# 30stomercury/whisper-char-alignment

Hardware: AMD Instinct MI355X
Metric: utterances/sec (whisper-medium, 10s audio, char align) at 1/2/4/8 MI355X (higher is better)
Workload: dtype f16x2 (hi + lo operand pairs on the f16 MFMA pipe: fp32-equivalent operands, fp32 accumulate)

## Files before the change

### include/wca.h

```cpp
#ifndef WCA_H_
#define WCA_H_

#include <stdint.h>

#ifdef __cplusplus
extern "C" {
#endif

typedef struct wca_engine wca_engine;

typedef enum {
  WCA_STATUS_PARTITIONED = 1,
  WCA_OK = 0,
  WCA_ERR_INVALID = -1,
  WCA_ERR_TOO_LONG = -2,
  WCA_ERR_HIP = -3,
  WCA_ERR_STATE = -4,
  WCA_ERR_NOMEM = -5
} wca_status;

typedef struct {
  int32_t n_mels;
  int32_t n_audio_ctx;
  int32_t n_audio_state;
// ... 28 lines not shown
void wca_engine_destroy(wca_engine* e);
int wca_engine_set_stream(wca_engine* e, void* hip_stream);
int wca_engine_synchronize(wca_engine* e);

int wca_load_weight(wca_engine* e, const char* name, const void* host_ptr, int dtype, const int64_t* shape, int ndim);
int wca_finalize_weights(wca_engine* e);
int wca_weights_inexact(wca_engine* e, long long* n_tensors_out, long long* n_values_out, char* first_name_out, int first_name_cap);
int wca_set_allow_rounded_weights(wca_engine* e, int on);


int wca_log_mel(wca_engine* e, const float* pcm_dev, int64_t pcm_stride, const int32_t* n_samples_host, int batch,
                float* mel_out_dev);

int wca_log_mel_long(wca_engine* e, const float* pcm_dev, int64_t n_samples, float* mel_out_dev, int64_t ld, int64_t* n_frames_out);

int wca_resample_plan(int sr_in, int32_t* L, int32_t* M, int32_t* W, int32_t* n_taps);
int wca_resample_table(int sr_in, double* table_out);
int wca_resample_16k(wca_engine* e, const float* in_dev, int channels, int64_t ld, int64_t n_in, int sr_in, float* out_dev, int64_t out_cap,
                     int64_t* n_out);

int wca_mel_window(wca_engine* e, const float* mel_long_dev, int64_t ld, int64_t n_frames, const int32_t* seek_host,
                   const int32_t* size_host, int batch, float* mel_out_dev);

int wca_quiet_cuts(wca_engine* e, const float* mel_long_dev, int64_t ld, int64_t content_frames, int n_pieces, int radius, int half_width,
                   int32_t* cuts_host, int32_t* level_host );

int wca_get_attentions(wca_engine* e, const float* mel_dev, const int64_t* tokens_dev, int batch, int n_tok,
                       const int32_t* n_tok_host, const int32_t* max_frames_host, int medfilt_width, float qk_scale,
                       float* weights_out_dev, float* logits_out_dev);

int wca_attention_weights(wca_engine* e, const float* qk_dev, int L, int H, int n, int ld, int max_frames,
                          int medfilt_width, float qk_scale, float* weights_out_dev);

int wca_median_filter(wca_engine* e, const float* in_dev, float* out_dev, int64_t rows, int F, int width);

int wca_filter_attention(wca_engine* e, const float* attns_dev, int L, int H, int n, int F, int topk, float w_colnorm,
                         float w_rownorm, float w_coverage, float* scores_host, int32_t* sel_idx_host,
                         float* sel_score_host);

int wca_force_align(wca_engine* e, const float* ws_dev, int L, int H, int n, int F, const wca_align_opts* opts,
                    float* matrix_host, int32_t* text_idx_host, int32_t* time_idx_host, int32_t* path_len_host,
                    int32_t* sel_idx_host, float* sel_score_host);

int wca_default_find_alignment(wca_engine* e, const float* ws_dev, int L, int H, int n, int F, const int32_t* heads_host,
                                int n_heads, int sot_len, float* weights_norm_out_dev, float* matrix_host,
                                int32_t* text_idx_host, int32_t* time_idx_host, int32_t* path_len_host);

int wca_dtw(wca_engine* e, const float* matrix_host, int N, int M, int32_t* text_idx_host, int32_t* time_idx_host,
            int32_t* path_len_host);

int wca_dtw_batch_dev(wca_engine* e, const float* matrix_dev, int P, int N, int M, int32_t* jump_frame_host);

int wca_dtw_open(wca_engine* e, const float* matrix_host, int N, int M, int32_t* text_idx_host, int32_t* time_idx_host,
                 int32_t* path_len_host, int32_t* end_row_host, float* score_host);

int wca_dtw_batch_dev_open(wca_engine* e, const float* matrix_dev, int P, int N, int M, const int32_t* n_rows_host,
                           const int32_t* n_cols_host, const int32_t* open_end_host, int32_t* jump_frame_host, int32_t* end_row_host,
                           float* score_host);

int wca_probe_heads(wca_engine* e, const float* ws_dev, int L, int H, int n, int F, int sot_len, float* scores_host,
                    int32_t* jump_frame_host);
int wca_probe_strict_tp(wca_engine* e, int n_heads, const int32_t* word_end_row_host, int n_hyp, const double* ref_times_host, int n_ref,
                        const uint8_t* same_word_host, double tolerance, int32_t* tp_host);

int wca_align_batch(wca_engine* e, const float* pcm_dev, int64_t pcm_stride, const int32_t* n_samples_host,
                    const int64_t* tokens_dev, int n_tok_max, const int32_t* n_tok_host,
                    const int32_t* max_frames_host, int batch, const wca_align_opts* opts, int32_t* jump_frame_host,
                    int32_t* sel_idx_host);

typedef struct {
  int32_t sample_len;
  int32_t eot;
  int32_t timestamp_begin;
  int32_t apply_timestamp_rules;
  int32_t max_initial_timestamp_index;
  int32_t no_speech;
} wca_decode_opts;

typedef struct {
  int32_t sample_len;
  int32_t eot;
  int32_t timestamp_begin;
  int32_t apply_timestamp_rules;
  int32_t max_initial_timestamp_index;
  int32_t no_speech;
  int32_t sot_index;
  int32_t prefill;
} wca_decode_opts_ex;

int wca_encode_batch(wca_engine* e, const float* mel_dev, const float* pcm_dev, int64_t pcm_stride,
                     const int32_t* n_samples_host, int batch);

int wca_greedy_decode(wca_engine* e, const float* mel_dev, const float* pcm_dev, int64_t pcm_stride,
                      const int32_t* n_samples_host, int batch, const int32_t* initial_tokens_host, int n_initial,
                      const uint8_t* suppress_mask_host, const uint8_t* blank_mask_host, const wca_decode_opts* opts,
                      int32_t* tokens_out_host, int32_t* n_tokens_host, float* sum_logprob_host,
                      float* no_speech_prob_host);
int wca_greedy_decode_ex(wca_engine* e, const float* mel_dev, const float* pcm_dev, int64_t pcm_stride,
                         const int32_t* n_samples_host, int batch, const int32_t* initial_tokens_host, int n_initial,
                         const uint8_t* suppress_mask_host, const uint8_t* blank_mask_host, const wca_decode_opts_ex* opts,
                         int32_t* tokens_out_host, int32_t* n_tokens_host, float* sum_logprob_host,
                         float* no_speech_prob_host);
int wca_greedy_decode_rows(wca_engine* e, const float* mel_dev, const float* pcm_dev, int64_t pcm_stride,
                           const int32_t* n_samples_host, int batch, const int32_t* initial_tokens_host,
                           const int32_t* n_initial_host, const int32_t* sot_index_host, const int32_t* sample_len_host,
                           const uint8_t* suppress_mask_host, const uint8_t* blank_mask_host, const wca_decode_opts* opts,
                           int32_t* tokens_out_host, int32_t* n_tokens_host, float* sum_logprob_host,
                           float* no_speech_prob_host);
int wca_detect_language(wca_engine* e, const float* mel_dev, const float* pcm_dev, int64_t pcm_stride, const int32_t* n_samples_host,
                        int batch, int sot, int lang_begin, int n_lang, int32_t* lang_token_host, float* probs_host);
int wca_last_decode_positions(wca_engine* e, int32_t* prefill_positions, int32_t* step_positions);

int wca_align_batch_enqueue(wca_engine* e, const float* pcm_dev, int64_t pcm_stride, const int32_t* n_samples_host,
                            const int64_t* tokens_dev, int n_tok_max, const int32_t* n_tok_host,
                            const int32_t* max_frames_host, int batch, const wca_align_opts* opts);
int wca_align_batch_fetch(wca_engine* e, int batch, int n_tok_max, int topk, int32_t* jump_frame_host,
                          int32_t* sel_idx_host);

int wca_align_batch_enqueue_ex(wca_engine* e, const float* pcm_dev, int64_t pcm_stride, const int32_t* n_samples_host,
                               const int64_t* tokens_dev, int n_tok_max, const int32_t* n_tok_host,
                               const int32_t* max_frames_host, int batch, const wca_align_opts* opts, int32_t vocab_end);
int wca_align_batch_fetch_ex(wca_engine* e, int batch, int n_tok_max, int topk, int32_t* jump_frame_host,
                             int32_t* sel_idx_host, float* token_logprob_host);
int wca_align_batch_enqueue_open(wca_engine* e, const float* pcm_dev, int64_t pcm_stride, const int32_t* n_samples_host,
                                 const int64_t* tokens_dev, int n_tok_max, const int32_t* n_tok_host,
                                 const int32_t* max_frames_host, int batch, const wca_align_opts* opts, int32_t vocab_end,
                                 const int32_t* open_end_host);
int wca_align_batch_fetch_open(wca_engine* e, int batch, int n_tok_max, int topk, int32_t* jump_frame_host,
                               int32_t* sel_idx_host, float* token_logprob_host, int32_t* end_row_host, float* score_host);
int wca_token_logprobs(wca_engine* e, const float* logits_dev, int rows, int ld, int vocab_end, const int64_t* targets_dev,
                       float* out_dev);

int wca_flac_info(const uint8_t* buf, int64_t nbytes, int32_t* sample_rate, int32_t* channels, int32_t* bits_per_sample,
                  int64_t* total_samples);
int wca_flac_decode(const uint8_t* buf, int64_t nbytes, float* out, int64_t capacity_per_channel, int64_t* n_decoded);

#define WCA_COMM_ID_BYTES 128
int wca_comm_unique_id(uint8_t* id_out );
int wca_comm_init(wca_engine* e, const uint8_t* id , int rank, int world);
int wca_comm_destroy(wca_engine* e);
int wca_allgather_results(wca_engine* e, const uint8_t* packed_host, int64_t n_bytes, uint8_t* gathered_host,
                          int64_t capacity_per_rank, int64_t* sizes_host );
int wca_allreduce_counters(wca_engine* e, int64_t* counters_host , int n);
int wca_collate_plan(const int64_t* sizes , const int64_t* capacities , int world, int64_t* pad_out);

int wca_test_gemm(wca_engine* e, const void* a_f16_dev, const void* w_f16_dev, const float* bias_dev, void* c_dev, int M,
                  int N, int K, int gelu, int out_mode);
int wca_test_gemm_pairs(wca_engine* e, const void* a2_f16_dev, const void* w_f16_dev, const float* bias_dev, void* c_dev, int M,
                        int N, int K, int gelu, int out_mode);
int wca_test_gemm_ln(wca_engine* e, const void* a_f16_dev, const void* w_f16_dev, const float* bias_dev, float* x_dev,
                     const float* gamma_dev, const float* beta_dev, void* xn_f16_dev, int M, int N, int K, int site);
int wca_test_gemm_plan(int M, int N, int K, int lda, int out_mode, int gelu, int a_lo, int force_tile, int site, int n_cu, int cu_limit, int flags,
                       int64_t sk_bytes, int32_t* out);
typedef struct wca_test_gemm_desc {
  const void* a;
  const void* w;
  const float* bias;
  void* c;
  const float* addend;
  const float* pos;
  int64_t a_batch_stride, c_batch_stride, a_lo, c_lo;
  int32_t M, N, K;
  int32_t lda, ldw, ldc;
  int32_t a_rows_per_batch, c_rows_per_batch;
  int32_t ld_addend, pos_period;
  int32_t gelu, out_mode, force_tile, site, cu_limit, supertile;
} wca_test_gemm_desc;
int wca_test_gemm_ex(wca_engine* e, const wca_test_gemm_desc* desc, int32_t* plan_out);
typedef struct wca_test_attn_desc {
  const void* q;
  const void* k;
  const void* v;
  void* o;
  float* cap;
  const int32_t* nk_rows;
  int64_t q_bs, k_bs, v_bs, o_bs;
  int64_t q_lo, k_lo, v_lo, o_lo;
  int64_t cap_bs, cap_hs;
  int32_t q_rs, k_rs, v_rs, o_rs;
  int32_t cap_ld, cap_cols;
  int32_t split, B, H, nq, nk, causal, variant;
} wca_test_attn_desc;
int wca_test_attention_ex(wca_engine* e, const wca_test_attn_desc* desc);
int wca_test_gemm_rows(wca_engine* e, const void* a_f16_dev, const float* x_f32_dev, const float* gamma_dev, const float* beta_dev,
                       const void* w_f16_dev, const float* bias_dev, void* c_dev, int M, int N, int K, int gelu, int out_mode, int splitk,
                       int groups, void* kv_k_f16_dev, void* kv_v_f16_dev, int T_max, int kv_t);
int wca_test_set_attn_split_drop(int mask);
int wca_test_set_switch(const char* name, int value);
int wca_test_last_scores(wca_engine* e, int batch, float* scores_host);
int wca_test_attention(wca_engine* e, const void* q_dev, const void* k_dev, const void* v_dev, void* o_dev,
                       float* cap_dev, int cap_ld, int cap_cols, int B, int H, int nq, int nk, int causal);
int wca_test_attention_split(wca_engine* e, const void* q2_dev, const void* k2_dev, const void* v2_dev, void* o2_dev,
                             float* cap_dev, int cap_ld, int cap_cols, int B, int H, int nq, int nk, int causal);
int wca_test_language_head(wca_engine* e, const float* x_dev, int B, int lang_begin, int n_lang, float* probs_dev, int32_t* lang_token_dev);
int wca_test_decode_select(wca_engine* e, const float* logits_dev, int batch, int n_vocab, int32_t* tokens_dev, int T_max,
                           int cur_len, int n_initial, const uint8_t* suppress_mask_dev, const uint8_t* blank_mask_dev,
                           const wca_decode_opts* opts, float* sum_logprob_dev, int32_t* n_done_dev);
int wca_test_decode_select_rows(wca_engine* e, const float* logits_dev, int batch, int n_vocab, int32_t* tokens_dev, int T_max,
                                const int32_t* cur_len_dev, const int32_t* n_initial_dev, const int32_t* cap_dev, int n_done_idx,
                                int n_done_len, const uint8_t* suppress_mask_dev, const uint8_t* blank_mask_dev,
                                const wca_decode_opts* opts, float* sum_logprob_dev, int32_t* n_done_dev);
int wca_test_attention_rows(wca_engine* e, const void* q_dev, const void* k_dev, const void* v_dev, void* o_dev, int B, int H, int nq,
                            int nk, const int32_t* nk_rows_dev, int causal);
int wca_test_layernorm(wca_engine* e, const float* x_dev, const float* g_dev, const float* b_dev, void* out_f16_dev,
                       int rows, int d);
int wca_test_layernorm_split(wca_engine* e, const float* x_dev, const float* g_dev, const float* b_dev, void* out2_f16_dev,
                             int rows, int d);
int wca_test_encoder(wca_engine* e, const float* mel_dev, int batch, float* xa_out_dev);

int wca_last_stage_ms(wca_engine* e, float* ms8);
enum {
  WCA_SITE_QKV = 0,
  WCA_SITE_ATTN = 1,
  WCA_SITE_OUT = 2,
  WCA_SITE_FC1 = 3,
  WCA_SITE_FC2 = 4,
  WCA_SITE_LN1 = 5,
  WCA_SITE_LN2 = 6,
  WCA_N_SITES = 7
};
int wca_last_kernel_ms(wca_engine* e, int site, int* n_launches, float* total_ms, double* flops_per_launch,
                       double* bytes_per_launch);
int wca_set_fuse_ln(wca_engine* e, int on);
enum { WCA_PRECISION_F16 = 0, WCA_PRECISION_SPLIT = 1, WCA_PRECISION_REFERENCE = 1 };
int wca_set_precision(wca_engine* e, int mode);
int wca_get_precision(wca_engine* e);
int wca_set_overlap(wca_engine* e, int on);
int wca_set_cu_partition(wca_engine* e, int phase2_cus);
int wca_set_decode_mode(wca_engine* e, int fused, int streams);
int wca_set_profiling(wca_engine* e, int on);

#ifdef __cplusplus
}
#endif
#endif
```

### whisper-char-alignment_amd/_lib.py

```python
import ctypes as C
import os

_HERE = os.path.dirname(os.path.abspath(__file__))
LIB_PATH = os.path.join(_HERE, "libwca.so")


class WcaError(RuntimeError):
    def __init__(self, code, msg):
        super().__init__("wca error %d: %s" % (code, msg))
        self.code = code


class TooLongError(WcaError):
    """n_tok > 448 or max_frames > 1500 (the skip condition of infer_ali.py:79)."""


class ModelDims(C.Structure):
    _fields_ = [(n, C.c_int32) for n in (
        "n_mels", "n_audio_ctx", "n_audio_state", "n_audio_head", "n_audio_layer",
        "n_vocab", "n_text_ctx", "n_text_state", "n_text_head", "n_text_layer")]


class AlignOpts(C.Structure):
    _fields_ = [("aggregation", C.c_int32), ("topk", C.c_int32), ("w_colnorm", C.c_float),
                ("w_rownorm", C.c_float), ("w_coverage", C.c_float), ("sot_len", C.c_int32),
                ("medfilt_width", C.c_int32), ("qk_scale", C.c_float)]


class DecodeOpts(C.Structure):
    _fields_ = [("sample_len", C.c_int32), ("eot", C.c_int32), ("timestamp_begin", C.c_int32),
                ("apply_timestamp_rules", C.c_int32), ("max_initial_timestamp_index", C.c_int32), ("no_speech", C.c_int32)]


class DecodeOptsEx(C.Structure):
    _fields_ = DecodeOpts._fields_ + [("sot_index", C.c_int32), ("prefill", C.c_int32)]


class GemmDesc(C.Structure):
    _fields_ = ([(n, C.c_void_p) for n in ("a", "w", "bias", "c", "addend", "pos")] +
                [(n, C.c_int64) for n in ("a_batch_stride", "c_batch_stride", "a_lo", "c_lo")] +
                [(n, C.c_int32) for n in ("M", "N", "K", "lda", "ldw", "ldc", "a_rows_per_batch", "c_rows_per_batch", "ld_addend", "pos_period",
                                          "gelu", "out_mode", "force_tile", "site", "cu_limit", "supertile")])


class AttnDesc(C.Structure):
    _fields_ = ([(n, C.c_void_p) for n in ("q", "k", "v", "o", "cap", "nk_rows")] +
                [(n, C.c_int64) for n in ("q_bs", "k_bs", "v_bs", "o_bs", "q_lo", "k_lo", "v_lo", "o_lo", "cap_bs", "cap_hs")] +
                [(n, C.c_int32) for n in ("q_rs", "k_rs", "v_rs", "o_rs", "cap_ld", "cap_cols", "split", "B", "H", "nq", "nk", "causal", "variant")])


ERR_TOO_LONG = -2
AGGR_MEAN, AGGR_TOPK = 0, 1
PRECISION_SITES = ("logmel", "conv", "enc_gemm", "enc_attn", "cross_kv", "dec", "capture")
SITES = {"qkv": 0, "attention": 1, "out_proj": 2, "fc1": 3, "fc2": 4, "ln1": 5, "ln2": 6}
DTYPE_F32, DTYPE_F16 = 0, 1

_vp, _i, _i64, _f = C.c_void_p, C.c_int, C.c_int64, C.c_float
_pi32 = C.POINTER(C.c_int32)
_pf = C.POINTER(C.c_float)

SIGNATURES = {
    "wca_last_error": (C.c_char_p, []),
    "wca_version": (_i, []),
    "wca_engine_create": (_i, [C.POINTER(ModelDims), _i, _i, C.POINTER(_vp)]),
    "wca_engine_create_ex": (_i, [C.POINTER(ModelDims), _i, _i, _i, C.POINTER(_vp)]),
    "wca_engine_destroy": (None, [_vp]),
    "wca_engine_set_stream": (_i, [_vp, _vp]),
    "wca_engine_synchronize": (_i, [_vp]),
    "wca_load_weight": (_i, [_vp, C.c_char_p, _vp, _i, C.POINTER(_i64), _i]),
    "wca_finalize_weights": (_i, [_vp]),
    "wca_weights_inexact": (_i, [_vp, C.POINTER(C.c_longlong), C.POINTER(C.c_longlong), C.c_char_p, _i]),
    "wca_set_allow_rounded_weights": (_i, [_vp, _i]),
    "wca_log_mel": (_i, [_vp, _vp, _i64, _pi32, _i, _vp]),
    "wca_log_mel_long": (_i, [_vp, _vp, _i64, _vp, _i64, C.POINTER(_i64)]),
    "wca_resample_plan": (_i, [_i, _pi32, _pi32, _pi32, _pi32]),
    "wca_resample_table": (_i, [_i, C.POINTER(C.c_double)]),
    "wca_resample_16k": (_i, [_vp, _vp, _i, _i64, _i64, _i, _vp, _i64, C.POINTER(_i64)]),
    "wca_mel_window": (_i, [_vp, _vp, _i64, _i64, _pi32, _pi32, _i, _vp]),
    "wca_quiet_cuts": (_i, [_vp, _vp, _i64, _i64, _i, _i, _i, _pi32, _pi32]),
    "wca_get_attentions": (_i, [_vp, _vp, _vp, _i, _i, _pi32, _pi32, _i, _f, _vp, _vp]),
    "wca_median_filter": (_i, [_vp, _vp, _vp, _i64, _i, _i]),
    "wca_filter_attention": (_i, [_vp, _vp, _i, _i, _i, _i, _i, _f, _f, _f, _pf, _pi32, _pf]),
    "wca_force_align": (_i, [_vp, _vp, _i, _i, _i, _i, C.POINTER(AlignOpts), _pf, _pi32, _pi32, _pi32, _pi32, _pf]),
    "wca_default_find_alignment": (_i, [_vp, _vp, _i, _i, _i, _i, _pi32, _i, _i, _vp, _pf, _pi32, _pi32, _pi32]),
    "wca_attention_weights": (_i, [_vp, _vp, _i, _i, _i, _i, _i, _i, _f, _vp]),
    "wca_flac_info": (_i, [_vp, _i64, _pi32, _pi32, _pi32, C.POINTER(_i64)]),
    "wca_flac_decode": (_i, [_vp, _i64, _vp, _i64, C.POINTER(_i64)]),
    "wca_dtw": (_i, [_vp, _pf, _i, _i, _pi32, _pi32, _pi32]),
    "wca_dtw_batch_dev": (_i, [_vp, _vp, _i, _i, _i, _pi32]),
    "wca_dtw_open": (_i, [_vp, _pf, _i, _i, _pi32, _pi32, _pi32, _pi32, _pf]),
    "wca_dtw_batch_dev_open": (_i, [_vp, _vp, _i, _i, _i, _pi32, _pi32, _pi32, _pi32, _pi32, _pf]),
    "wca_probe_heads": (_i, [_vp, _vp, _i, _i, _i, _i, _i, _pf, _pi32]),
    "wca_align_batch": (_i, [_vp, _vp, _i64, _pi32, _vp, _i, _pi32, _pi32, _i, C.POINTER(AlignOpts), _pi32, _pi32]),
    "wca_align_batch_enqueue": (_i, [_vp, _vp, _i64, _pi32, _vp, _i, _pi32, _pi32, _i, C.POINTER(AlignOpts)]),
    "wca_align_batch_fetch": (_i, [_vp, _i, _i, _i, _pi32, _pi32]),
    "wca_align_batch_enqueue_ex": (_i, [_vp, _vp, _i64, _pi32, _vp, _i, _pi32, _pi32, _i, C.POINTER(AlignOpts), C.c_int32]),
    "wca_align_batch_fetch_ex": (_i, [_vp, _i, _i, _i, _pi32, _pi32, _pf]),
    "wca_align_batch_enqueue_open": (_i, [_vp, _vp, _i64, _pi32, _vp, _i, _pi32, _pi32, _i, C.POINTER(AlignOpts), C.c_int32, _pi32]),
    "wca_align_batch_fetch_open": (_i, [_vp, _i, _i, _i, _pi32, _pi32, _pf, _pi32, _pf]),
    "wca_token_logprobs": (_i, [_vp, _vp, _i, _i, _i, _vp, _vp]),
    "wca_encode_batch": (_i, [_vp, _vp, _vp, _i64, _pi32, _i]),
    "wca_greedy_decode": (_i, [_vp, _vp, _vp, _i64, _pi32, _i, _pi32, _i, _vp, _vp, C.POINTER(DecodeOpts), _pi32, _pi32, _pf, _pf]),
    "wca_greedy_decode_ex": (_i, [_vp, _vp, _vp, _i64, _pi32, _i, _pi32, _i, _vp, _vp, C.POINTER(DecodeOptsEx), _pi32, _pi32, _pf, _pf]),
    "wca_greedy_decode_rows": (_i, [_vp, _vp, _vp, _i64, _pi32, _i, _pi32, _pi32, _pi32, _pi32, _vp, _vp, C.POINTER(DecodeOpts), _pi32, _pi32, _pf,
                                    _pf]),
    "wca_detect_language": (_i, [_vp, _vp, _vp, _i64, _pi32, _i, _i, _i, _i, _pi32, _pf]),
    "wca_test_language_head": (_i, [_vp, _vp, _i, _i, _i, _vp, _vp]),
    "wca_last_decode_positions": (_i, [_vp, _pi32, _pi32]),
    "wca_test_decode_select_rows": (_i, [_vp, _vp, _i, _i, _vp, _i, _vp, _vp, _vp, _i, _i, _vp, _vp, C.POINTER(DecodeOpts), _vp, _vp]),
    "wca_test_attention_rows": (_i, [_vp, _vp, _vp, _vp, _vp, _i, _i, _i, _i, _vp, _i]),
    "wca_test_decode_select": (_i, [_vp, _vp, _i, _i, _vp, _i, _i, _i, _vp, _vp, C.POINTER(DecodeOpts), _vp, _vp]),
    "wca_test_gemm": (_i, [_vp, _vp, _vp, _vp, _vp, _i, _i, _i, _i, _i]),
    "wca_test_gemm_plan": (_i, [_i, _i, _i, _i, _i, _i, _i, _i, _i, _i, _i, _i, _i64, _pi32]),
    "wca_test_gemm_ex": (_i, [_vp, C.POINTER(GemmDesc), _pi32]),
    "wca_test_attention_ex": (_i, [_vp, C.POINTER(AttnDesc)]),
    "wca_test_gemm_ln": (_i, [_vp, _vp, _vp, _vp, _vp, _vp, _vp, _vp, _i, _i, _i, _i]),
    "wca_test_set_attn_split_drop": (_i, [_i]),
    "wca_test_set_switch": (_i, [C.c_char_p, _i]),
    "wca_test_last_scores": (_i, [_vp, _i, _pf]),
    "wca_test_gemm_pairs": (_i, [_vp, _vp, _vp, _vp, _vp, _i, _i, _i, _i, _i]),
    "wca_test_attention": (_i, [_vp, _vp, _vp, _vp, _vp, _vp, _i, _i, _i, _i, _i, _i, _i]),
    "wca_test_attention_split": (_i, [_vp, _vp, _vp, _vp, _vp, _vp, _i, _i, _i, _i, _i, _i, _i]),
    "wca_test_layernorm": (_i, [_vp, _vp, _vp, _vp, _vp, _i, _i]),
    "wca_test_layernorm_split": (_i, [_vp, _vp, _vp, _vp, _vp, _i, _i]),
    "wca_test_encoder": (_i, [_vp, _vp, _i, _vp]),
    "wca_last_stage_ms": (_i, [_vp, _pf]),
    "wca_set_profiling": (_i, [_vp, _i]),
    "wca_last_kernel_ms": (_i, [_vp, _i, C.POINTER(C.c_int), _pf, C.POINTER(C.c_double), C.POINTER(C.c_double)]),
    "wca_set_overlap": (_i, [_vp, _i]),
    "wca_set_cu_partition": (_i, [_vp, _i]),
    "wca_set_fuse_ln": (_i, [_vp, _i]),
    "wca_set_precision": (_i, [_vp, _i]),
    "wca_get_precision": (_i, [_vp]),
    "wca_set_decode_mode": (_i, [_vp, _i, _i]),
    "wca_comm_unique_id": (_i, [_vp]),
    "wca_comm_init": (_i, [_vp, _vp, _i, _i]),
    "wca_comm_destroy": (_i, [_vp]),
    "wca_allgather_results": (_i, [_vp, _vp, _i64, _vp, _i64, C.POINTER(_i64)]),
    "wca_allreduce_counters": (_i, [_vp, C.POINTER(_i64), _i]),
    "wca_collate_plan": (_i, [C.POINTER(_i64), C.POINTER(_i64), _i, C.POINTER(_i64)]),
    "wca_probe_strict_tp": (_i, [_vp, _i, _vp, _i, _vp, _i, _vp, C.c_double, _vp]),
    "wca_test_gemm_rows": (_i, [_vp, _vp, _vp, _vp, _vp, _vp, _vp, _vp, _i, _i, _i, _i, _i, _i, _i, _vp, _vp, _i, _i]),
}

_lib = None


def load():
    global _lib
    if _lib is not None:
        return _lib
    if not os.path.exists(LIB_PATH):
        raise ImportError(
            "libwca.so not found at %s: build it with `python whisper-char-alignment_amd/build.py` "
            "(or __graft_entry__.build()). The alignment engine has no CPU fallback." % LIB_PATH)
    lib = C.CDLL(LIB_PATH)
    for name, (res, args) in SIGNATURES.items():
        fn = getattr(lib, name)
        fn.restype = res
        fn.argtypes = args
    _lib = lib
    return lib


def check(code):
    if code == 0:
        return
    msg = load().wca_last_error()
    msg = msg.decode("utf-8", "replace") if msg else ""
    if code == -2:
        raise TooLongError(code, msg)
    raise WcaError(code, msg)


def i32_array(values):
    arr = (C.c_int32 * len(values))(*[int(v) for v in values])
    return arr
```

### whisper-char-alignment_amd/csrc/attention_split.hip

```cpp
#include <cstdlib>

#include "attn_common.h"
#include "launch.h"

namespace wca {

namespace {

template <bool CAUSAL, bool CAPTURE>
__global__ __launch_bounds__(256, 2) void attn_split_kernel(AttnArgs a) {
  constexpr int NW = 4;
  extern __shared__ __attribute__((aligned(16))) char smem[];
  half_t* lds = reinterpret_cast<half_t*>(smem);
  const int tid = threadIdx.x;
  const int lane = tid & 63;
  const int wave = __builtin_amdgcn_readfirstlane(tid >> 6);
  const int fr = lane & 15, fg = lane >> 4;
  constexpr int QB = NW * 32;
  const int n_qt = (a.nq + QB - 1) / QB;
  const int lid = xcd_remap(blockIdx.x, n_qt * a.H * a.B);
  const int bh = lid / n_qt;
  const int b = bh / a.H, h = bh - b * a.H;
  const int q_blk = (lid - bh * n_qt) * QB;
  const int q_wave = q_blk + wave * 32;
// ... 237 lines not shown
  do {                                                                                       \
    R[0] = lds_read_tr_asm<VH>(A);                                                               \
    R[1] = lds_read_tr_asm<VH + B16>(A);                                                         \
    R[2] = lds_read_tr_asm<VL>(A);                                                               \
    R[3] = lds_read_tr_asm<VL + B16>(A);                                                         \
    R[4] = lds_read_tr_asm<VH + K2>(A);                                                          \
    R[5] = lds_read_tr_asm<VH + K2 + B16>(A);                                                    \
    R[6] = lds_read_tr_asm<VL + K2>(A);                                                          \
    R[7] = lds_read_tr_asm<VL + K2 + B16>(A);                                                    \
  } while (0)
      WCA_ISSUE_V(c_, vaddr[0] + sb);
#pragma unroll
      for (int dt = 0; dt < 4; ++dt) {
        if (dt < 3) {
          WCA_ISSUE_V(n_, vaddr[dt + 1] + sb);
          WCA_LGKM_WAIT8(8, c_[0], c_[1], c_[2], c_[3], c_[4], c_[5], c_[6], c_[7]);
        } else {
          WCA_LGKM_WAIT8(0, c_[0], c_[1], c_[2], c_[3], c_[4], c_[5], c_[6], c_[7]);
        }
#pragma unroll
        for (int k2 = 0; k2 < 2; ++k2) {
          const half8 vh = __builtin_shufflevector(c_[4 * k2], c_[4 * k2 + 1], 0, 1, 2, 3, 4, 5, 6, 7);
          const half8 vl = __builtin_shufflevector(c_[4 * k2 + 2], c_[4 * k2 + 3], 0, 1, 2, 3, 4, 5, 6, 7);
#pragma unroll
          for (int s = 0; s < 2; ++s) {
            ot[s][dt] = __builtin_amdgcn_mfma_f32_16x16x32_f16(vl, ph[s][k2], ot[s][dt], 0, 0, 0);
            ot[s][dt] = __builtin_amdgcn_mfma_f32_16x16x32_f16(vh, pl[s][k2], ot[s][dt], 0, 0, 0);
            ot[s][dt] = __builtin_amdgcn_mfma_f32_16x16x32_f16(vh, ph[s][k2], ot[s][dt], 0, 0, 0);
          }
        }
        if (dt < 3) {
#pragma unroll
          for (int i = 0; i < 8; ++i) c_[i] = n_[i];
        }
      }
#undef WCA_ISSUE_V
    }
  }

#pragma unroll
  for (int s = 0; s < 2; ++s) {
    const float l = xor32_sum(xor16_sum(l_part[s]));
    if (qrow[s] >= a.nq) continue;
    const float inv = 1.0f / l;
    half_t* op = a.O + (long)b * a.o_bs + (long)qrow[s] * a.o_rs + h * 64 + 4 * fg;
#pragma unroll
    for (int dt = 0; dt < 4; ++dt) {
      half4 oh, ol;
#pragma unroll
      for (int r = 0; r < 4; ++r) {
        const HalfPair pr = split_pair(ot[s][dt][r] * inv);
        oh[r] = pr.hi;
        ol[r] = pr.lo;
      }
      *reinterpret_cast<half4*>(op + dt * 16) = oh;
      *reinterpret_cast<half4*>(op + a.o_lo + dt * 16) = ol;
    }
  }
}



#define WCA_S_PIN8(A, B, C, D, E, F, G, H) asm volatile("" : "+v"(A), "+v"(B), "+v"(C), "+v"(D), "+v"(E), "+v"(F), "+v"(G), "+v"(H)::"memory")

template <int DROP>
__global__ __launch_bounds__(256, 2) void attn_split32_kernel(AttnArgs a) {
  constexpr int NW = 4;
  extern __shared__ __attribute__((aligned(16))) char smem[];
  half_t* lds = reinterpret_cast<half_t*>(smem);
  const int tid = threadIdx.x;
  const int lane = tid & 63;
  const int wave = __builtin_amdgcn_readfirstlane(tid >> 6);
  const int l31 = lane & 31, hh = lane >> 5;
  constexpr int QB = NW * 32;
  constexpr int TB = TILE * (int)sizeof(half_t);
  constexpr int SLOT_BYTES = 4 * TB;
  const int n_qt = (a.nq + QB - 1) / QB;
  const int lid = xcd_remap(blockIdx.x, n_qt * a.H * a.B);
  const int bh = lid / n_qt;
  const int b = bh / a.H, h = bh - b * a.H;
  const int q_wave = (lid - bh * n_qt) * QB + wave * 32;
  const int qrow = q_wave + l31;
  const float c_log2 = a.scale * LOG2E;
  half8 qh[4], ql[4];
  {
    const int qc = qrow < a.nq ? qrow : a.nq - 1;
    const half_t* qp = a.Q + (long)b * a.q_bs + (long)qc * a.q_rs + h * 64 + hh * 8;
#pragma unroll
    for (int ks = 0; ks < 4; ++ks) {
      const half8 rh = *reinterpret_cast<const half8*>(qp + ks * 16);
      const half8 rl = *reinterpret_cast<const half8*>(qp + a.q_lo + ks * 16);
#pragma unroll
      for (int j = 0; j < 8; ++j) {
        const HalfPair pr = split_pair(((float)rh[j] + (float)rl[j]) * c_log2);
        qh[ks][j] = pr.hi;
        ql[ks][j] = pr.lo;
      }
    }
  }
  const int nkt = (a.nk + KT - 1) / KT;
  const int kbytes = (int)(((long)(a.nk - 1) * a.k_rs + 64) * 2), vbytes = (int)(((long)(a.nk - 1) * a.v_rs + 64) * 2);
  const half_t* Kb = a.K + (long)b * a.k_bs + h * 64;
  const half_t* Vb = a.V + (long)b * a.v_bs + h * 64;
  const __amdgpu_buffer_rsrc_t rkh = __builtin_amdgcn_make_buffer_rsrc(const_cast<half_t*>(Kb), 0, kbytes, 0x00020000);
  const __amdgpu_buffer_rsrc_t rkl = __builtin_amdgcn_make_buffer_rsrc(const_cast<half_t*>(Kb + a.k_lo), 0, kbytes, 0x00020000);
  const __amdgpu_buffer_rsrc_t rvh = __builtin_amdgcn_make_buffer_rsrc(const_cast<half_t*>(Vb), 0, vbytes, 0x00020000);
  const __amdgpu_buffer_rsrc_t rvl = __builtin_amdgcn_make_buffer_rsrc(const_cast<half_t*>(Vb + a.v_lo), 0, vbytes, 0x00020000);
  unsigned dk[2], dv[2];
#pragma unroll
  for (int i = 0; i < 2; ++i) {
    const int r = (wave * 2 + i) * 8 + (lane >> 3);
    dk[i] = (unsigned)(r * a.k_rs * 2 + (((lane & 7) ^ ((r >> 1) & 7)) << 4));
    dv[i] = (unsigned)(r * a.v_rs * 2 + (((lane & 7) ^ ((r & 2) << 1)) << 4));
  }
  const unsigned k_tile_bytes = (unsigned)(KT * a.k_rs * 2), v_tile_bytes = (unsigned)(KT * a.v_rs * 2);
  auto stage = [&](int buf, int kt) {
    half_t* Kh = lds + buf * (4 * TILE);
#pragma unroll
    for (int i = 0; i < 2; ++i) {
      const int rbase = (wave * 2 + i) * 8;
      __builtin_amdgcn_raw_ptr_buffer_load_lds(rkh, (WCA_LDS void*)(Kh + rbase * 64), 16, (int)dk[i], (int)(kt * k_tile_bytes), 0, 0);
      __builtin_amdgcn_raw_ptr_buffer_load_lds(rkl, (WCA_LDS void*)(Kh + TILE + rbase * 64), 16, (int)dk[i], (int)(kt * k_tile_bytes), 0, 0);
      __builtin_amdgcn_raw_ptr_buffer_load_lds(rvh, (WCA_LDS void*)(Kh + 2 * TILE + rbase * 64), 16, (int)dv[i], (int)(kt * v_tile_bytes), 0, 0);
      __builtin_amdgcn_raw_ptr_buffer_load_lds(rvl, (WCA_LDS void*)(Kh + 3 * TILE + rbase * 64), 16, (int)dv[i], (int)(kt * v_tile_bytes), 0, 0);
    }
  };

  const int kswz = (l31 >> 1) & 7;
  const unsigned lds_base = lds_off(lds);
  unsigned ka[4];
#pragma unroll
  for (int ks = 0; ks < 4; ++ks) ka[ks] = lds_base + (unsigned)(l31 * 128 + 16 * ((hh ^ kswz) & 1) + 32 * (ks ^ (kswz >> 1)));
  const int vq = (lane & 15) >> 2, vp = lane & 3, vg1 = (lane >> 4) & 1;
  const int vkey0 = 4 * hh + vq;
  const int vdim0 = 16 * vg1 + 4 * vp;
  const int vsw = (vkey0 & 2) << 1;
  unsigned va[2];
#pragma unroll
  for (int db = 0; db < 2; ++db)
    va[db] = lds_base + (unsigned)(2 * TB + vkey0 * 128 + (((4 * db + (vdim0 >> 3)) ^ vsw) << 4) + 2 * (vdim0 & 7));

  f32x16 ot[2];
#pragma unroll
  for (int d = 0; d < 2; ++d)
#pragma unroll
    for (int r = 0; r < 16; ++r) ot[d][r] = 0.f;
  float m_run = -INFINITY;
  float l_run = 0.f;
  f32x16 cinit;
#pragma unroll
  for (int r = 0; r < 16; ++r) cinit[r] = 0.f;

  stage(0, 0);
  auto tile = [&](auto slot_c, int kt) {
    constexpr int SLOT = decltype(slot_c)::value;
    constexpr int SB = SLOT * SLOT_BYTES;
    asm volatile("s_waitcnt vmcnt(0)" ::: "memory");
    __builtin_amdgcn_s_barrier();
    asm volatile("" ::: "memory");
    if (kt + 1 < nkt) stage(SLOT ^ 1, kt + 1);

    f32x16 st[2];
    {
      half8 kl0[4], kh0[4], kl1[4], kh1[4];
      kl0[0] = lds_read_b128_asm<SB + TB>(ka[0]);
      kl0[1] = lds_read_b128_asm<SB + TB>(ka[1]);
      kl0[2] = lds_read_b128_asm<SB + TB>(ka[2]);
      kl0[3] = lds_read_b128_asm<SB + TB>(ka[3]);
      kh0[0] = lds_read_b128_asm<SB>(ka[0]);
      kh0[1] = lds_read_b128_asm<SB>(ka[1]);
      kh0[2] = lds_read_b128_asm<SB>(ka[2]);
      kh0[3] = lds_read_b128_asm<SB>(ka[3]);
      kl1[0] = lds_read_b128_asm<SB + TB + 32 * 128>(ka[0]);
      kl1[1] = lds_read_b128_asm<SB + TB + 32 * 128>(ka[1]);
      kl1[2] = lds_read_b128_asm<SB + TB + 32 * 128>(ka[2]);
      kl1[3] = lds_read_b128_asm<SB + TB + 32 * 128>(ka[3]);
      kh1[0] = lds_read_b128_asm<SB + 32 * 128>(ka[0]);
      kh1[1] = lds_read_b128_asm<SB + 32 * 128>(ka[1]);
      kh1[2] = lds_read_b128_asm<SB + 32 * 128>(ka[2]);
      kh1[3] = lds_read_b128_asm<SB + 32 * 128>(ka[3]);
      if constexpr (DROP == 0) {
      WCA_LGKM_WAIT4(12, kl0[0], kl0[1], kl0[2], kl0[3]);
      st[0] = __builtin_amdgcn_mfma_f32_32x32x16_f16(kl0[0], qh[0], cinit, 0, 0, 0);
#pragma unroll
      for (int ks = 1; ks < 4; ++ks) st[0] = __builtin_amdgcn_mfma_f32_32x32x16_f16(kl0[ks], qh[ks], st[0], 0, 0, 0);
      WCA_LGKM_WAIT4(8, kh0[0], kh0[1], kh0[2], kh0[3]);
#pragma unroll
      for (int ks = 0; ks < 4; ++ks) st[0] = __builtin_amdgcn_mfma_f32_32x32x16_f16(kh0[ks], ql[ks], st[0], 0, 0, 0);
#pragma unroll
      for (int ks = 0; ks < 4; ++ks) st[0] = __builtin_amdgcn_mfma_f32_32x32x16_f16(kh0[ks], qh[ks], st[0], 0, 0, 0);
      WCA_LGKM_WAIT4(4, kl1[0], kl1[1], kl1[2], kl1[3]);
      st[1] = __builtin_amdgcn_mfma_f32_32x32x16_f16(kl1[0], qh[0], cinit, 0, 0, 0);
#pragma unroll
      for (int ks = 1; ks < 4; ++ks) st[1] = __builtin_amdgcn_mfma_f32_32x32x16_f16(kl1[ks], qh[ks], st[1], 0, 0, 0);
      WCA_LGKM_WAIT4(0, kh1[0], kh1[1], kh1[2], kh1[3]);
#pragma unroll
      for (int ks = 0; ks < 4; ++ks) st[1] = __builtin_amdgcn_mfma_f32_32x32x16_f16(kh1[ks], ql[ks], st[1], 0, 0, 0);
#pragma unroll
      for (int ks = 0; ks < 4; ++ks) st[1] = __builtin_amdgcn_mfma_f32_32x32x16_f16(kh1[ks], qh[ks], st[1], 0, 0, 0);
      } else {
        WCA_LGKM_WAIT4(0, kh1[0], kh1[1], kh1[2], kh1[3]);
        WCA_S_PIN8(kl0[0], kl0[1], kl0[2], kl0[3], kh0[0], kh0[1], kh0[2], kh0[3]);
        WCA_S_PIN8(kl1[0], kl1[1], kl1[2], kl1[3], kh1[0], kh1[1], kh1[2], kh1[3]);
        st[0] = cinit;
        st[1] = cinit;
#pragma unroll
        for (int ks = 0; ks < 4; ++ks) {
          if (!(DROP & 1)) st[0] = __builtin_amdgcn_mfma_f32_32x32x16_f16(kl0[ks], qh[ks], st[0], 0, 0, 0);
          if (!(DROP & 1)) st[1] = __builtin_amdgcn_mfma_f32_32x32x16_f16(kl1[ks], qh[ks], st[1], 0, 0, 0);
        }
#pragma unroll
        for (int ks = 0; ks < 4; ++ks) {
          if (!(DROP & 2)) st[0] = __builtin_amdgcn_mfma_f32_32x32x16_f16(kh0[ks], ql[ks], st[0], 0, 0, 0);
          if (!(DROP & 2)) st[1] = __builtin_amdgcn_mfma_f32_32x32x16_f16(kh1[ks], ql[ks], st[1], 0, 0, 0);
        }
#pragma unroll
        for (int ks = 0; ks < 4; ++ks) {
          st[0] = __builtin_amdgcn_mfma_f32_32x32x16_f16(kh0[ks], qh[ks], st[0], 0, 0, 0);
          st[1] = __builtin_amdgcn_mfma_f32_32x32x16_f16(kh1[ks], qh[ks], st[1], 0, 0, 0);
        }
      }
    }
    half4 v0ha[4], v0hb[4], v0la[4], v0lb[4], v1ha[4], v1hb[4], v1la[4], v1lb[4];
#define WCA_ISSUE_V32(P, DB)                                           \
  do {                                                                 \
    P##ha[0] = lds_read_tr_asm<SB + 0 * 2048>(va[DB]);                     \
    P##hb[0] = lds_read_tr_asm<SB + 0 * 2048 + 1024>(va[DB]);              \
    P##ha[1] = lds_read_tr_asm<SB + 1 * 2048>(va[DB]);                     \
    P##hb[1] = lds_read_tr_asm<SB + 1 * 2048 + 1024>(va[DB]);              \
    P##ha[2] = lds_read_tr_asm<SB + 2 * 2048>(va[DB]);                     \
    P##hb[2] = lds_read_tr_asm<SB + 2 * 2048 + 1024>(va[DB]);              \
    P##ha[3] = lds_read_tr_asm<SB + 3 * 2048>(va[DB]);                     \
    P##hb[3] = lds_read_tr_asm<SB + 3 * 2048 + 1024>(va[DB]);              \
    P##la[0] = lds_read_tr_asm<SB + TB + 0 * 2048>(va[DB]);                \
    P##lb[0] = lds_read_tr_asm<SB + TB + 0 * 2048 + 1024>(va[DB]);         \
    P##la[1] = lds_read_tr_asm<SB + TB + 1 * 2048>(va[DB]);                \
    P##lb[1] = lds_read_tr_asm<SB + TB + 1 * 2048 + 1024>(va[DB]);         \
    P##la[2] = lds_read_tr_asm<SB + TB + 2 * 2048>(va[DB]);                \
    P##lb[2] = lds_read_tr_asm<SB + TB + 2 * 2048 + 1024>(va[DB]);         \
    P##la[3] = lds_read_tr_asm<SB + TB + 3 * 2048>(va[DB]);                \
    P##lb[3] = lds_read_tr_asm<SB + TB + 3 * 2048 + 1024>(va[DB]);         \
  } while (0)
    WCA_ISSUE_V32(v0, 0);
    if (kt * KT + KT > a.nk) {
#pragma unroll
      for (int kb = 0; kb < 2; ++kb)
#pragma unroll
        for (int r = 0; r < 16; ++r) {
          const int key = kt * KT + kb * 32 + (r & 3) + 8 * (r >> 2) + 4 * hh;
          st[kb][r] = key >= a.nk ? -INFINITY : st[kb][r];
        }
    }
    float mx;
    {
      float m0 = max3f(st[0][0], st[0][1], st[0][2]), m1 = max3f(st[0][3], st[0][4], st[0][5]);
      float m2 = max3f(st[0][6], st[0][7], st[0][8]), m3 = max3f(st[0][9], st[0][10], st[0][11]);
      m0 = max3f(m0, st[0][12], st[0][13]);
      m1 = max3f(m1, st[0][14], st[0][15]);
      m2 = max3f(m2, st[1][0], st[1][1]);
      m3 = max3f(m3, st[1][2], st[1][3]);
      m0 = max3f(m0, st[1][4], st[1][5]);
      m1 = max3f(m1, st[1][6], st[1][7]);
      m2 = max3f(m2, st[1][8], st[1][9]);
      m3 = max3f(m3, st[1][10], st[1][11]);
      m0 = max3f(m0, st[1][12], st[1][13]);
      m1 = max3f(m1, st[1][14], st[1][15]);
      mx = fmaxf(max3f(m0, m1, m2), m3);
      mx = xor32_max(mx);
    }
    if (__any((mx > RESCALE_THR) || (m_run == -INFINITY && mx != -INFINITY))) {
      const float m_eff = (m_run == -INFINITY) ? 0.f : m_run;
      const float m_new = fmaxf(m_run, mx + m_eff);
      const float delta = (m_new == -INFINITY) ? 0.f : m_new - m_eff;
      const float alpha = (m_run == -INFINITY) ? 1.0f : __builtin_amdgcn_exp2f(m_run - m_new);
      l_run *= alpha;
#pragma unroll
      for (int d = 0; d < 2; ++d)
#pragma unroll
        for (int r = 0; r < 16; ++r) ot[d][r] *= alpha;
#pragma unroll
      for (int kb = 0; kb < 2; ++kb)
#pragma unroll
        for (int r = 0; r < 16; ++r) st[kb][r] -= delta;
      m_run = m_new;
      const float c0 = (m_new != -INFINITY) ? -m_new : 0.f;
#pragma unroll
      for (int r = 0; r < 16; ++r) cinit[r] = c0;
    }
    half8 ph[4], pl[4];
    {
      f32x2 psum = f32x2{0.f, 0.f};
#pragma unroll
      for (int s4 = 0; s4 < 4; ++s4) {
        half2_ hq[4], lq[4];
#pragma unroll
        for (int u = 0; u < 4; ++u) {
          const int r0 = 8 * (s4 & 1) + 2 * u;
          const f32x2 p = f32x2{__builtin_amdgcn_exp2f(st[s4 >> 1][r0]), __builtin_amdgcn_exp2f(st[s4 >> 1][r0 + 1])};
          psum += p;
          hq[u] = __builtin_convertvector(p, half2_);
          const unsigned hu = __builtin_bit_cast(unsigned, hq[u]);
          unsigned lu;
          asm("v_fma_mixlo_f16 %0, %1, 1.0, -%2 op_sel:[0,0,0] op_sel_hi:[0,0,1]" : "=v"(lu) : "v"(p[0]), "v"(hu));
          asm("v_fma_mixhi_f16 %0, %1, 1.0, -%2 op_sel:[0,0,1] op_sel_hi:[0,0,1]" : "+v"(lu) : "v"(p[1]), "v"(hu));
          lq[u] = __builtin_bit_cast(half2_, lu);
        }
        ph[s4] = half8{hq[0][0], hq[0][1], hq[1][0], hq[1][1], hq[2][0], hq[2][1], hq[3][0], hq[3][1]};
        pl[s4] = half8{lq[0][0], lq[0][1], lq[1][0], lq[1][1], lq[2][0], lq[2][1], lq[3][0], lq[3][1]};
      }
      l_run += psum[0] + psum[1];
    }
    WCA_LGKM_WAIT8(0, v0ha[0], v0hb[0], v0ha[1], v0hb[1], v0ha[2], v0hb[2], v0ha[3], v0hb[3]);
    WCA_S_PIN8(v0la[0], v0lb[0], v0la[1], v0lb[1], v0la[2], v0lb[2], v0la[3], v0lb[3]);
    WCA_ISSUE_V32(v1, 1);
#pragma unroll
    for (int s4 = 0; s4 < 4; ++s4) {
      const half8 wh = __builtin_shufflevector(v0ha[s4], v0hb[s4], 0, 1, 2, 3, 4, 5, 6, 7);
      const half8 wl = __builtin_shufflevector(v0la[s4], v0lb[s4], 0, 1, 2, 3, 4, 5, 6, 7);
      if (!(DROP & 4)) ot[0] = __builtin_amdgcn_mfma_f32_32x32x16_f16(wl, ph[s4], ot[0], 0, 0, 0);
      if (!(DROP & 8)) ot[0] = __builtin_amdgcn_mfma_f32_32x32x16_f16(wh, pl[s4], ot[0], 0, 0, 0);
      ot[0] = __builtin_amdgcn_mfma_f32_32x32x16_f16(wh, ph[s4], ot[0], 0, 0, 0);
    }
    WCA_LGKM_WAIT8(0, v1ha[0], v1hb[0], v1ha[1], v1hb[1], v1ha[2], v1hb[2], v1ha[3], v1hb[3]);
    WCA_S_PIN8(v1la[0], v1lb[0], v1la[1], v1lb[1], v1la[2], v1lb[2], v1la[3], v1lb[3]);
#pragma unroll
    for (int s4 = 0; s4 < 4; ++s4) {
      const half8 wh = __builtin_shufflevector(v1ha[s4], v1hb[s4], 0, 1, 2, 3, 4, 5, 6, 7);
      const half8 wl = __builtin_shufflevector(v1la[s4], v1lb[s4], 0, 1, 2, 3, 4, 5, 6, 7);
      if (!(DROP & 4)) ot[1] = __builtin_amdgcn_mfma_f32_32x32x16_f16(wl, ph[s4], ot[1], 0, 0, 0);
      if (!(DROP & 8)) ot[1] = __builtin_amdgcn_mfma_f32_32x32x16_f16(wh, pl[s4], ot[1], 0, 0, 0);
      ot[1] = __builtin_amdgcn_mfma_f32_32x32x16_f16(wh, ph[s4], ot[1], 0, 0, 0);
    }
#undef WCA_ISSUE_V32
  };
  for (int kt = 0; kt < nkt; kt += 2) {
    tile(IntC<0>{}, kt);
    if (kt + 1 < nkt) tile(IntC<1>{}, kt + 1);
  }

  const float inv = 1.0f / xor32_sum(l_run);
  half_t* op = a.O + (long)b * a.o_bs + (long)qrow * a.o_rs + h * 64;
#pragma unroll
  for (int db = 0; db < 2; ++db)
#pragma unroll
    for (int g2 = 0; g2 < 2; ++g2) {
      unsigned wh[2][2], wl[2][2];
#pragma unroll
      for (int e = 0; e < 2; ++e)
#pragma unroll
        for (int k2 = 0; k2 < 2; ++k2) {
          const Half2Pair pr = split_pair2(ot[db][4 * (2 * g2 + e) + 2 * k2] * inv, ot[db][4 * (2 * g2 + e) + 2 * k2 + 1] * inv);
          wh[e][k2] = __builtin_bit_cast(unsigned, pr.hi);
          wl[e][k2] = __builtin_bit_cast(unsigned, pr.lo);
        }
      typedef unsigned u32x4 __attribute__((ext_vector_type(4)));
      u32x4 oh, ol;
      {
        auto r0 = __builtin_amdgcn_permlane32_swap(wh[0][0], wh[1][0], false, false);
        auto r1 = __builtin_amdgcn_permlane32_swap(wh[0][1], wh[1][1], false, false);
        oh = u32x4{r0[0], r1[0], r0[1], r1[1]};
        auto s0 = __builtin_amdgcn_permlane32_swap(wl[0][0], wl[1][0], false, false);
        auto s1 = __builtin_amdgcn_permlane32_swap(wl[0][1], wl[1][1], false, false);
        ol = u32x4{s0[0], s1[0], s0[1], s1[1]};
      }
      if (qrow < a.nq) {
        *reinterpret_cast<u32x4*>(op + 32 * db + 16 * g2 + 8 * hh) = oh;
        *reinterpret_cast<u32x4*>(op + a.o_lo + 32 * db + 16 * g2 + 8 * hh) = ol;
      }
    }
}

}

hipError_t launch_attention_split(const AttnArgs& a, hipStream_t s) {
  if (a.nq <= 0 || a.B <= 0) return hipSuccess;
  if (!attn_args_ok(a)) return hipErrorInvalidValue;
  if ((a.q_lo % 8) || (a.k_lo % 8) || (a.v_lo % 8) || (a.o_lo % 4) || a.q_lo <= 0 || a.k_lo <= 0 || a.v_lo <= 0 || a.o_lo <= 0) return hipErrorInvalidValue;
  const bool cap = a.cap != nullptr && a.cap_cols > 0;
  constexpr int LDS = 2 * 4 * TILE * (int)sizeof(half_t);
  const dim3 grid(((a.nq + 127) / 128) * a.H * a.B), block(256);
  const int variant = a.variant ? a.variant : debug_switch(DBG_ATTN_SPLIT_VARIANT);
  if (!a.causal && !cap && a.nq >= 64 && variant != 1 && (a.o_rs % 8) == 0 && (a.o_lo % 8) == 0) {
    auto launch32 = [&](auto drop_c) { return launch_lds<attn_split32_kernel<decltype(drop_c)::value>, LDS>(grid, block, LDS, s, a); };
    switch (debug_switch(DBG_ATTN_SPLIT_DROP)) {
      case 0: return launch32(IntC<0>{});
      case 1: return launch32(IntC<1>{});
      case 2: return launch32(IntC<2>{});
      case 3: return launch32(IntC<3>{});
      case 4: return launch32(IntC<4>{});
      case 8: return launch32(IntC<8>{});
      case 9: return launch32(IntC<9>{});
      case 12: return launch32(IntC<12>{});
      case 15: return launch32(IntC<15>{});
      default: return hipErrorInvalidValue;
    }
  }
  if (a.causal) {
    if (cap) return launch_lds<attn_split_kernel<true, true>, LDS>(grid, block, LDS, s, a);
    return launch_lds<attn_split_kernel<true, false>, LDS>(grid, block, LDS, s, a);
  }
  if (cap) return launch_lds<attn_split_kernel<false, true>, LDS>(grid, block, LDS, s, a);
  return launch_lds<attn_split_kernel<false, false>, LDS>(grid, block, LDS, s, a);
}

}
```

### whisper-char-alignment_amd/csrc/debug_switch.cpp

```cpp
#include <atomic>
#include <cstring>

#include "kernels.h"

namespace wca {

namespace {
struct Sw {
  const char* name;
  std::atomic<int> value;
};
Sw g_sw[DBG_SWITCH_COUNT] = {
    {"attn_split_variant", {0}},
    {"head_stats_general", {0}},
    {"fail_precision_alloc", {0}},
    {"attn_split_drop", {0}},
    {"gemm_ring", {0}},
};
}

int debug_switch(int id) {
  if (id < 0 || id >= DBG_SWITCH_COUNT) return 0;
  return g_sw[id].value.load(std::memory_order_relaxed);
}

int set_debug_switch(const char* name, int value) {
  for (int i = 0; i < DBG_SWITCH_COUNT; ++i)
    if (std::strcmp(g_sw[i].name, name) == 0) {
      g_sw[i].value.store(value, std::memory_order_relaxed);
      return 0;
    }
  return -1;
}

}
```

### whisper-char-alignment_amd/csrc/elementwise.hip

```cpp
#include <cstdlib>

#include "kernels.h"
#include "wca_common.h"

namespace wca {

namespace {

template <int NV, bool SPLIT = false>
__global__ __launch_bounds__(256) void layernorm_f16_v4_kernel(const float* __restrict__ x, const float* __restrict__ gamma,
                                                               const float* __restrict__ beta, half_t* __restrict__ out,
                                                               int rows, float eps, int ld_out, long lo_off) {
  constexpr int d = 256 * NV;
  const int lane = threadIdx.x & 63;
  const int row = blockIdx.x * 4 + (threadIdx.x >> 6);
  if (row >= rows) return;
  const f32x4* xr = reinterpret_cast<const f32x4*>(x + (long)row * d);
  f32x4 v[NV];
  float s = 0.f;
#pragma unroll
  for (int i = 0; i < NV; ++i) {
    v[i] = xr[i * 64 + lane];
    s += (v[i][0] + v[i][1]) + (v[i][2] + v[i][3]);
  }
// ... 26 lines not shown
      } else {
        o[j] = (half_t)y;
      }
    }
    o4[i * 64 + lane] = o;
    if (SPLIT) l4[i * 64 + lane] = ol;
  }
}

template <int NV>
__global__ __launch_bounds__(256) void layernorm_pair_v8_kernel(const float* __restrict__ x, const float* __restrict__ gamma,
                                                                const float* __restrict__ beta, half_t* __restrict__ out, int rows, float eps,
                                                                int ld_out, long lo_off) {
  constexpr int d = 256 * NV, NC = NV / 2;
  const int lane = threadIdx.x & 63;
  const int row = blockIdx.x * 4 + (threadIdx.x >> 6);
  if (row >= rows) return;
  const float* xr = x + (long)row * d;
  f32x4 v[NV];
  float s = 0.f;
#pragma unroll
  for (int c = 0; c < NC; ++c) {
    v[2 * c] = *reinterpret_cast<const f32x4*>(xr + c * 512 + lane * 8);
    v[2 * c + 1] = *reinterpret_cast<const f32x4*>(xr + c * 512 + lane * 8 + 4);
  }
  if (NV & 1) v[NV - 1] = *reinterpret_cast<const f32x4*>(xr + NC * 512 + lane * 4);
#pragma unroll
  for (int i = 0; i < NV; ++i) s += (v[i][0] + v[i][1]) + (v[i][2] + v[i][3]);
  const float mean = wave_sum(s) * (1.0f / d);
  float q = 0.f;
#pragma unroll
  for (int i = 0; i < NV; ++i) {
#pragma unroll
    for (int j = 0; j < 4; ++j) {
      const float t = v[i][j] - mean;
      q += t * t;
    }
  }
  const float rstd = rsqrtf(wave_sum(q) * (1.0f / d) + eps);
  half_t* orow = out + (long)row * ld_out;
#pragma unroll
  for (int c = 0; c < NC; ++c) {
    const int e0 = c * 512 + lane * 8;
    half8 o, ol;
#pragma unroll
    for (int h = 0; h < 2; ++h) {
      const f32x4 g = *reinterpret_cast<const f32x4*>(gamma + e0 + 4 * h), bb = *reinterpret_cast<const f32x4*>(beta + e0 + 4 * h);
#pragma unroll
      for (int j = 0; j < 4; ++j) {
        const HalfPair pr = split_pair((v[2 * c + h][j] - mean) * rstd * g[j] + bb[j]);
        o[4 * h + j] = pr.hi;
        ol[4 * h + j] = pr.lo;
      }
    }
    *reinterpret_cast<half8*>(orow + e0) = o;
    *reinterpret_cast<half8*>(orow + lo_off + e0) = ol;
  }
  if (NV & 1) {
    const int e0 = NC * 512 + lane * 4;
    const f32x4 g = *reinterpret_cast<const f32x4*>(gamma + e0), bb = *reinterpret_cast<const f32x4*>(beta + e0);
    half4 o, ol;
#pragma unroll
    for (int j = 0; j < 4; ++j) {
      const HalfPair pr = split_pair((v[NV - 1][j] - mean) * rstd * g[j] + bb[j]);
      o[j] = pr.hi;
      ol[j] = pr.lo;
    }
    *reinterpret_cast<half4*>(orow + e0) = o;
    *reinterpret_cast<half4*>(orow + lo_off + e0) = ol;
  }
}

template <int NV2, bool SPLIT = false>
__global__ __launch_bounds__(256) void layernorm_f16_v2_kernel(const float* __restrict__ x, const float* __restrict__ gamma,
                                                               const float* __restrict__ beta, half_t* __restrict__ out,
                                                               int rows, float eps, int ld_out, long lo_off) {
  constexpr int d = 128 * NV2;
  const int lane = threadIdx.x & 63;
  const int row = blockIdx.x * 4 + (threadIdx.x >> 6);
  if (row >= rows) return;
  const f32x2* xr = reinterpret_cast<const f32x2*>(x + (long)row * d);
  f32x2 v[NV2];
  float s = 0.f;
#pragma unroll
  for (int i = 0; i < NV2; ++i) {
    v[i] = xr[i * 64 + lane];
    s += v[i][0] + v[i][1];
  }
  const float mean = wave_sum(s) * (1.0f / d);
  float q = 0.f;
#pragma unroll
  for (int i = 0; i < NV2; ++i) {
    const float a = v[i][0] - mean, b = v[i][1] - mean;
    q += a * a + b * b;
  }
  const float rstd = rsqrtf(wave_sum(q) * (1.0f / d) + eps);
  const f32x2* g2 = reinterpret_cast<const f32x2*>(gamma);
  const f32x2* b2 = reinterpret_cast<const f32x2*>(beta);
  half2_* o2 = reinterpret_cast<half2_*>(out + (long)row * ld_out);
  half2_* l2 = reinterpret_cast<half2_*>(out + (long)row * ld_out + lo_off);
#pragma unroll
  for (int i = 0; i < NV2; ++i) {
    const f32x2 g = g2[i * 64 + lane], bb = b2[i * 64 + lane];
    const float y0 = (v[i][0] - mean) * rstd * g[0] + bb[0], y1 = (v[i][1] - mean) * rstd * g[1] + bb[1];
    half2_ o;
    if (SPLIT) {
      const HalfPair p0 = split_pair(y0), p1 = split_pair(y1);
      half2_ ol;
      o[0] = p0.hi;
      o[1] = p1.hi;
      ol[0] = p0.lo;
      ol[1] = p1.lo;
      l2[i * 64 + lane] = ol;
    } else {
      o[0] = (half_t)y0;
      o[1] = (half_t)y1;
    }
    o2[i * 64 + lane] = o;
  }
}

__global__ __launch_bounds__(256) void embed_kernel(const int64_t* __restrict__ tokens, const half_t* __restrict__ tok_emb,
                                                    const float* __restrict__ pos_emb, float* __restrict__ x, int B, int n,
                                                    int d, int n_vocab, int* __restrict__ err, const half_t* __restrict__ tok_emb_lo) {
  const int row = blockIdx.x;
  const int i = row % n;
  long tok = tokens[row];
  if (tok < 0 || tok >= n_vocab) {
    if (threadIdx.x == 0 && err) atomicOr(err, 1);
    tok = 0;
  }
  const half_t* e = tok_emb + tok * d;
  const float* p = pos_emb + (long)i * d;
  float* o = x + (long)row * d;
  if (tok_emb_lo != nullptr) {
    const half_t* el = tok_emb_lo + tok * d;
    for (int c = threadIdx.x; c < d; c += blockDim.x) o[c] = ((float)e[c] + (float)el[c]) + p[c];
    return;
  }
  for (int c = threadIdx.x; c < d; c += blockDim.x) o[c] = (float)e[c] + p[c];
}

__global__ void fill_f16_kernel(half_t* p, size_t n, float v) {
  size_t i = (size_t)blockIdx.x * blockDim.x + threadIdx.x;
  const size_t st = (size_t)gridDim.x * blockDim.x;
  const half_t h = (half_t)v;
  for (; i < n; i += st) p[i] = h;
}

__global__ void f32_to_f16_kernel(const float* __restrict__ in, half_t* __restrict__ out, size_t n) {
  size_t i = (size_t)blockIdx.x * blockDim.x + threadIdx.x;
  const size_t st = (size_t)gridDim.x * blockDim.x;
  for (; i < n; i += st) out[i] = (half_t)in[i];
}

}

hipError_t launch_layernorm_f16(const float* x, const float* gamma, const float* beta, half_t* out, int rows, int d,
                                float eps, hipStream_t s, int ld_out, long lo_off) {
  if (rows <= 0) return hipSuccess;
  if (ld_out <= 0) ld_out = d;
  if ((ld_out & 3) || (lo_off & 3) || lo_off < 0) return hipErrorInvalidValue;
  dim3 grid((rows + 3) / 4), block(256);
#define WCA_LN(KERN, NV)                                                                                                           \
  do {                                                                                                                             \
    if (lo_off) hipLaunchKernelGGL((KERN<NV, true>), grid, block, 0, s, x, gamma, beta, out, rows, eps, ld_out, lo_off);           \
    else hipLaunchKernelGGL((KERN<NV, false>), grid, block, 0, s, x, gamma, beta, out, rows, eps, ld_out, lo_off);                 \
  } while (0)
  if (lo_off && d >= 512 && (d % 256) == 0 && (ld_out & 7) == 0 && (lo_off & 7) == 0 && (reinterpret_cast<uintptr_t>(out) & 15) == 0) {
    switch (d) {
      case 512: hipLaunchKernelGGL((layernorm_pair_v8_kernel<2>), grid, block, 0, s, x, gamma, beta, out, rows, eps, ld_out, lo_off); return hipGetLastError();
      case 768: hipLaunchKernelGGL((layernorm_pair_v8_kernel<3>), grid, block, 0, s, x, gamma, beta, out, rows, eps, ld_out, lo_off); return hipGetLastError();
      case 1024: hipLaunchKernelGGL((layernorm_pair_v8_kernel<4>), grid, block, 0, s, x, gamma, beta, out, rows, eps, ld_out, lo_off); return hipGetLastError();
      case 1280: hipLaunchKernelGGL((layernorm_pair_v8_kernel<5>), grid, block, 0, s, x, gamma, beta, out, rows, eps, ld_out, lo_off); return hipGetLastError();
      default: break;
    }
  }
  switch (d) {
    case 128: WCA_LN(layernorm_f16_v2_kernel, 1); break;
    case 256: WCA_LN(layernorm_f16_v4_kernel, 1); break;
    case 384: WCA_LN(layernorm_f16_v2_kernel, 3); break;
    case 512: WCA_LN(layernorm_f16_v4_kernel, 2); break;
    case 768: WCA_LN(layernorm_f16_v4_kernel, 3); break;
    case 1024: WCA_LN(layernorm_f16_v4_kernel, 4); break;
    case 1280: WCA_LN(layernorm_f16_v4_kernel, 5); break;
    default: return hipErrorInvalidValue;
  }
#undef WCA_LN
  return hipGetLastError();
}

hipError_t launch_embed(const int64_t* tokens, const half_t* tok_emb, const float* pos_emb, float* x, int B, int n,
                        int d, int n_vocab, int* err, hipStream_t s, const half_t* tok_emb_lo) {
  if (B * n <= 0) return hipSuccess;
  hipLaunchKernelGGL(embed_kernel, dim3(B * n), dim3(256), 0, s, tokens, tok_emb, pos_emb, x, B, n, d, n_vocab, err, tok_emb_lo);
  return hipGetLastError();
}

hipError_t launch_fill_f16(half_t* p, size_t n, float v, hipStream_t s) {
  if (n == 0) return hipSuccess;
  const int blocks = (int)((n + 255) / 256 < 2048 ? (n + 255) / 256 : 2048);
  hipLaunchKernelGGL(fill_f16_kernel, dim3(blocks), dim3(256), 0, s, p, n, v);
  return hipGetLastError();
}

hipError_t launch_f32_to_f16(const float* in, half_t* out, size_t n, hipStream_t s) {
  if (n == 0) return hipSuccess;
  const int blocks = (int)((n + 255) / 256 < 2048 ? (n + 255) / 256 : 2048);
  hipLaunchKernelGGL(f32_to_f16_kernel, dim3(blocks), dim3(256), 0, s, in, out, n);
  return hipGetLastError();
}

}
```

### whisper-char-alignment_amd/csrc/engine.hip

```cpp
#include <cstdarg>

#include "engine_internal.h"

using namespace wca;

namespace {
thread_local std::string g_err;
}

namespace wca {

int fail(int code, const char* fmt, ...) {
  char buf[512];
  va_list ap;
  va_start(ap, fmt);
  vsnprintf(buf, sizeof(buf), fmt, ap);
  va_end(ap);
  g_err = buf;
  return code;
}

static size_t layout_arena(wca_engine* e, char* base) {
  const wca_model_dims& D = e->dims;
  const size_t B = e->max_batch, d = D.n_audio_state, dt = D.n_text_state, L = D.n_text_layer;
// ... 31 lines not shown
    for (int i = 0; i < 2; ++i) {
      e->sk_part[i] = carve<float>(cur, e->sk_floats);
      e->sk_cnt[i] = carve<unsigned>(cur, e->sk_tiles + 16, 256);
    }
    e->sk_big_bytes = (size_t)4 * 128 * 128 * 128 * sizeof(float);
    for (int i = 0; i < 3; ++i) e->sk_big[i] = carve<float>(cur, e->sk_big_bytes / sizeof(float));
  }
  return (size_t)(cur - base) + 4096;
}

void record(wca_engine* e, int i, hipStream_t s) {
  if (e->profiling && e->ev_valid) (void)hipEventRecord(e->ev[i], s ? s : e->stream);
}

int join_phase2(wca_engine* e) {
  if (e->enq_count > e->fetch_count) HIPCHK(hipStreamWaitEvent(e->stream, e->res_ev[(e->enq_count - 1) & 1], 0));
  return WCA_OK;
}

int enter(wca_engine* e) {
  if (!e) return fail(WCA_ERR_INVALID, "null engine");
  HIPCHK(hipSetDevice(e->device));
  return join_phase2(e);
}

int check_ready(wca_engine* e) {
  if (!e) return fail(WCA_ERR_INVALID, "null engine");
  if (!e->finalized) return fail(WCA_ERR_STATE, "weights not finalized (call wca_finalize_weights)");
  HIPCHK(hipSetDevice(e->device));
  return ensure_split_weights(e);
}

int stage_meta(wca_engine* e, int B, const int32_t* a0, const int32_t* a1, const int32_t* a2, const int32_t* a3, int** dev_rows, hipStream_t s) {
  const int slot = e->meta_slot;
  e->meta_slot = (e->meta_slot + 1) % META_SLOTS;
  int* h = e->meta_host + (size_t)slot * 4 * e->max_batch;
  int* dv = e->meta_dev + (size_t)slot * 4 * e->max_batch;
  const int32_t* src[4] = {a0, a1, a2, a3};
  for (int r = 0; r < 4; ++r)
    for (int b = 0; b < B; ++b) h[r * e->max_batch + b] = src[r] ? src[r][b] : 0;
  HIPCHK(hipMemcpyAsync(dv, h, sizeof(int) * 4 * e->max_batch, hipMemcpyHostToDevice, s ? s : e->stream));
  for (int r = 0; r < 4; ++r) dev_rows[r] = dv + r * e->max_batch;
  return WCA_OK;
}

int take_kv_slot(wca_engine* e) {
  for (int sl = 0; sl < 2; ++sl)
    if (!e->slot_busy[sl]) return sl;
  for (auto it = e->enc_q.begin(); it != e->enc_q.end(); ++it)
    if (it->decoded) {
      const int sl = it->slot;
      e->enc_q.erase(it);
      return sl;
    }
  return -1;
}

}

extern "C" {

const char* wca_last_error(void) { return g_err.c_str(); }
int wca_version(void) { return 15; }

int wca_engine_create(const wca_model_dims* dims, int device_ordinal, int max_batch, wca_engine** out) {
  return wca_engine_create_ex(dims, device_ordinal, max_batch, WCA_PRECISION_REFERENCE, out);
}

int wca_engine_create_ex(const wca_model_dims* dims, int device_ordinal, int max_batch, int precision_mode, wca_engine** out) {
  if (!dims || !out) return fail(WCA_ERR_INVALID, "null argument");
  if (precision_mode != WCA_PRECISION_F16 && precision_mode != WCA_PRECISION_REFERENCE) return fail(WCA_ERR_INVALID, "precision mode %d", precision_mode);
  if (max_batch < 1 || max_batch > 256) return fail(WCA_ERR_INVALID, "max_batch %d outside [1,256]", max_batch);
  const wca_model_dims& D = *dims;
  if (D.n_audio_ctx != N_CTX || D.n_text_ctx != MAX_TOK) return fail(WCA_ERR_INVALID, "n_audio_ctx must be 1500 and n_text_ctx 448");
  if (D.n_audio_state % 128 || D.n_text_state % 128 || D.n_audio_state / D.n_audio_head != 64 || D.n_text_state / D.n_text_head != 64 ||
      D.n_audio_state > 1280 || D.n_text_state > 1280)
    return fail(WCA_ERR_INVALID, "unsupported widths: need n_state %% 128 == 0, n_state <= 1280, head_dim == 64");
  if (D.n_audio_state != D.n_text_state) return fail(WCA_ERR_INVALID, "n_audio_state != n_text_state");
  if (D.n_mels % 8 || D.n_mels > 256) return fail(WCA_ERR_INVALID, "n_mels must be a multiple of 8 and <= 256");
  int ndev = 0;
  HIPCHK(hipGetDeviceCount(&ndev));
  if (device_ordinal < 0 || device_ordinal >= ndev) return fail(WCA_ERR_INVALID, "device %d not present (%d devices)", device_ordinal, ndev);
  HIPCHK(hipSetDevice(device_ordinal));
  wca_engine* e = new wca_engine();
  e->dims = D;
  e->device = device_ordinal;
  e->max_batch = max_batch;
  HIPCHK(hipDeviceGetAttribute(&e->n_cu, hipDeviceAttributeMultiprocessorCount, device_ordinal));
  HIPCHK(hipStreamCreateWithFlags(&e->own_stream, hipStreamNonBlocking));
  HIPCHK(hipStreamCreateWithFlags(&e->stream2, hipStreamNonBlocking));
  HIPCHK(hipStreamCreateWithFlags(&e->stream3, hipStreamNonBlocking));
  HIPCHK(hipEventCreateWithFlags(&e->ev_fork, hipEventDisableTiming));
  HIPCHK(hipEventCreateWithFlags(&e->ev_join, hipEventDisableTiming));
  e->stream = e->own_stream;
  for (auto& ev : e->ev_kv) HIPCHK(hipEventCreateWithFlags(&ev, hipEventDisableTiming));
  e->wslab_bytes = layout_weights(e, nullptr);
  HIPCHK(hipMalloc((void**)&e->wslab, e->wslab_bytes));
  HIPCHK(hipMemset(e->wslab, 0, e->wslab_bytes));
  layout_weights(e, e->wslab);
  if (precision_mode == WCA_PRECISION_REFERENCE) {
    e->split = true;
    const size_t wbytes = layout_split_weights(e, nullptr);
    HIPCHK(hipMalloc((void**)&e->wslab2, wbytes));
    HIPCHK(hipMemset(e->wslab2, 0, wbytes));
    layout_split_weights(e, e->wslab2);
    e->sw_dirty = true;
  }
  const size_t abytes = layout_arena(e, nullptr);
  HIPCHK(hipMalloc((void**)&e->aslab, abytes));
  HIPCHK(hipMemset(e->aslab, 0, abytes));
  layout_arena(e, e->aslab);
  HIPCHK(hipHostMalloc((void**)&e->meta_host, sizeof(int) * META_SLOTS * 4 * max_batch, hipHostMallocDefault));
  HIPCHK(hipHostMalloc((void**)&e->err_host, sizeof(int) * 4, hipHostMallocDefault));
  e->err_host[0] = 0;
  for (auto& ev : e->ev) HIPCHK(hipEventCreate(&ev));
  for (auto& site : e->kev)
    for (auto& layer : site)
      for (auto& ev : layer) HIPCHK(hipEventCreate(&ev));
  for (auto& ev : e->res_ev) HIPCHK(hipEventCreateWithFlags(&ev, hipEventDisableTiming));
  e->ev_valid = true;
  {
    std::vector<float> win(N_FFT), tw(2 * N_FFT);
    const double PI = 3.14159265358979323846;
    for (int n = 0; n < N_FFT; ++n) {
      win[n] = (float)(0.5 - 0.5 * std::cos(2.0 * PI * n / N_FFT));
      tw[2 * n] = (float)std::cos(2.0 * PI * n / N_FFT);
      tw[2 * n + 1] = (float)std::sin(2.0 * PI * n / N_FFT);
    }
    HIPCHK(hipMemcpy(e->window, win.data(), sizeof(float) * N_FFT, hipMemcpyHostToDevice));
    HIPCHK(hipMemcpy(e->twiddle, tw.data(), sizeof(float) * 2 * N_FFT, hipMemcpyHostToDevice));
  }
  *out = e;
  return WCA_OK;
}

void wca_engine_destroy(wca_engine* e) {
  if (!e) return;
  (void)hipSetDevice(e->device);
  (void)hipDeviceSynchronize();
  if (e->part_s1) {
    e->enq_count = e->fetch_count;
    e->enc_q.clear();
    (void)wca_set_cu_partition(e, 0);
  }
  for (GrowBuf* g : {&e->cap, &e->wws, &e->colnorm, &e->scores, &e->sel, &e->selsc, &e->matrix, &e->trace, &e->path, &e->pathlen,
                     &e->jump, &e->tmp0, &e->tmp1})
    g->release();
  (void)wca_comm_destroy(e);
  e->coll_send.release();
  e->coll_recv.release();
  if (e->wslab) (void)hipFree(e->wslab);
  if (e->wslab2) (void)hipFree(e->wslab2);
  if (e->wslab_lo) (void)hipFree(e->wslab_lo);
  e->wlo_tmp[0].release();
  e->wlo_tmp[1].release();
  if (e->aslab) (void)hipFree(e->aslab);
  if (e->meta_host) (void)hipHostFree(e->meta_host);
  if (e->err_host) (void)hipHostFree(e->err_host);
  if (e->dec_done_host) (void)hipHostFree(e->dec_done_host);
  e->dec_cache.release();
  e->dec_tokens.release();
  e->dec_masks.release();
  e->dec_logits.release();
  e->dec_state.release();
  e->dec_gather.release();
  e->dec_rows.release();
  e->probe_jump.release();
  e->dtw_out.release();
  e->dtw_meta.release();
  e->quiet_out.release();
  for (auto& t : e->rs_tables) (void)hipFree(t.dev);
  for (int i = 0; i < 2; ++i) {
    if (e->res_host[i]) (void)hipHostFree(e->res_host[i]);
    if (e->res_ev[i]) (void)hipEventDestroy(e->res_ev[i]);
  }
  if (e->ev_valid)
  {
    for (auto& ev : e->ev) (void)hipEventDestroy(ev);
    for (auto& site : e->kev)
      for (auto& layer : site)
        for (auto& ev : layer) (void)hipEventDestroy(ev);
  }
  for (auto& ev : e->ev_kv)
    if (ev) (void)hipEventDestroy(ev);
  if (e->ev_fork) (void)hipEventDestroy(e->ev_fork);
  if (e->ev_join) (void)hipEventDestroy(e->ev_join);
  if (e->stream3) (void)hipStreamDestroy(e->stream3);
  if (e->stream2) (void)hipStreamDestroy(e->stream2);
  if (e->own_stream) (void)hipStreamDestroy(e->own_stream);
  delete e;
}

int wca_engine_set_stream(wca_engine* e, void* hip_stream) {
  if (!e) return fail(WCA_ERR_INVALID, "null engine");
  e->user_stream = (hipStream_t)hip_stream;
  e->user_stream_set = true;
  if (e->part_cus > 0) return WCA_STATUS_PARTITIONED;
  e->stream = e->user_stream;
  return WCA_OK;
}

int wca_engine_synchronize(wca_engine* e) {
  if (!e) return fail(WCA_ERR_INVALID, "null engine");
  HIPCHK(hipSetDevice(e->device));
  HIPCHK(hipStreamSynchronize(e->stream));
  HIPCHK(hipStreamSynchronize(e->stream2));
  HIPCHK(hipStreamSynchronize(e->stream3));
  return WCA_OK;
}

int wca_set_decode_mode(wca_engine* e, int fused, int streams) {
  if (!e) return fail(WCA_ERR_INVALID, "null engine");
  if (streams != 1 && streams != 2) return fail(WCA_ERR_INVALID, "streams must be 1 or 2");
  e->dec_fused = fused != 0;
  e->dec_streams = streams;
  return WCA_OK;
}

int wca_set_profiling(wca_engine* e, int on) {
  if (!e) return fail(WCA_ERR_INVALID, "null engine");
  e->profiling = on != 0;
  return WCA_OK;
}

int wca_last_stage_ms(wca_engine* e, float* ms8) {
  if (!e || !ms8) return fail(WCA_ERR_INVALID, "null argument");
  if (!e->profiling) return fail(WCA_ERR_STATE, "profiling disabled");
  HIPCHK(hipEventSynchronize(e->ev[8]));
  for (int i = 0; i < 7; ++i) HIPCHK(hipEventElapsedTime(&ms8[i], e->ev[i], e->ev[i + 1]));
  HIPCHK(hipEventElapsedTime(&ms8[7], e->ev[0], e->ev[8]));
  return WCA_OK;
}

int wca_last_kernel_ms(wca_engine* e, int site, int* n_launches, float* total_ms, double* flops_per_launch, double* bytes_per_launch) {
  if (!e || !n_launches || !total_ms || !flops_per_launch || !bytes_per_launch) return fail(WCA_ERR_INVALID, "null argument");
  if (site < 0 || site >= WCA_N_SITES) return fail(WCA_ERR_INVALID, "site %d outside [0,%d)", site, WCA_N_SITES);
  if (!e->profiling) return fail(WCA_ERR_STATE, "profiling disabled");
  HIPCHK(hipEventSynchronize(e->ev[8]));
  int nl = 0;
  float tot = 0.f;
  for (int i = 0; i < 33; ++i) {
    if (!e->kev_set[site][i]) continue;
    float ms = 0.f;
    HIPCHK(hipEventElapsedTime(&ms, e->kev[site][i][0], e->kev[site][i][1]));
    tot += ms;
    ++nl;
  }
  *n_launches = nl;
  *total_ms = tot;
  const double d = e->dims.n_audio_state, M = (double)e->last_batch * N_CTX, H = e->dims.n_audio_head;
  const double p = e->split ? 2.0 : 1.0;
  const double fused_ln = e->fuse_ln && !e->split ? 2 : 0;
  double fl = 0, by = 0;
  switch (site) {
    case WCA_SITE_QKV: fl = 2 * M * 3 * d * d; by = 2 * (p * M * d + 3 * d * d + p * M * 3 * d); break;
    case WCA_SITE_ATTN: fl = 4.0 * e->last_batch * H * (double)N_CTX * N_CTX * 64; by = 2 * p * (M * 3 * d + M * d); break;
    case WCA_SITE_OUT: fl = 2 * M * d * d; by = 2 * (p * M * d + d * d) + 8 * M * d + fused_ln * M * d; break;
    case WCA_SITE_FC1: fl = 2 * M * 4 * d * d; by = 2 * (p * M * d + 4 * d * d + p * M * 4 * d); break;
    case WCA_SITE_FC2: fl = 2 * M * 4 * d * d; by = 2 * (p * M * 4 * d + 4 * d * d) + 8 * M * d + fused_ln * M * d; break;
    case WCA_SITE_LN1:
    case WCA_SITE_LN2: fl = 8 * M * d; by = (4 + 2 * p) * M * d; break;
  }
  *flops_per_launch = fl;
  *bytes_per_launch = by;
  return WCA_OK;
}

int wca_set_precision(wca_engine* e, int mode) {
  if (!e) return fail(WCA_ERR_INVALID, "null engine");
  if (mode != WCA_PRECISION_F16 && mode != WCA_PRECISION_SPLIT) return fail(WCA_ERR_INVALID, "precision mode %d", mode);
  const bool want = mode == WCA_PRECISION_SPLIT, was = e->split;
  if (want == was) return WCA_OK;
  if (e->enq_count != e->fetch_count) return fail(WCA_ERR_STATE, "fetch the batches in flight before changing the precision mode");
  for (auto& st : e->enc_q)
    if (!st.decoded) return fail(WCA_ERR_STATE, "an encoded batch is waiting: consume it before changing the precision mode");
  HIPCHK(hipSetDevice(e->device));
  HIPCHK(hipStreamSynchronize(e->stream));
  HIPCHK(hipStreamSynchronize(e->stream2));
  HIPCHK(hipStreamSynchronize(e->stream3));
  e->split = want;
  const size_t abytes = layout_arena(e, nullptr);
  e->split = was;
  char* na = nullptr;
  char* nw = nullptr;
  size_t wbytes = 0;
  hipError_t he = hipMalloc((void**)&na, abytes);
  if (he == hipSuccess && want) {
    wbytes = layout_split_weights(e, nullptr);
    he = hipMalloc((void**)&nw, wbytes);
  }
  if (he == hipSuccess) he = hipMemset(na, 0, abytes);
  if (he == hipSuccess && nw) he = hipMemset(nw, 0, wbytes);
  if (he == hipSuccess && debug_switch(DBG_FAIL_PRECISION_ALLOC)) he = hipErrorOutOfMemory;
  if (he != hipSuccess) {
    if (na) (void)hipFree(na);
    if (nw) (void)hipFree(nw);
    (void)hipGetLastError();
    layout_arena(e, e->aslab);
    if (was) layout_split_weights(e, e->wslab2);
    return fail(WCA_ERR_HIP, "precision switch: allocating the %s arena (%zu + %zu bytes) failed: %s; the engine keeps its previous mode",
                want ? "wide" : "narrow", abytes, wbytes, hipGetErrorString(he));
  }
  (void)hipFree(e->aslab);
  if (e->wslab2) (void)hipFree(e->wslab2);
  e->aslab = na;
  e->wslab2 = nw;
// ... 77 lines not shown
```

### whisper-char-alignment_amd/csrc/engine_align.hip

```cpp
#include "engine_internal.h"

using namespace wca;

namespace {

int check_medfilt(int width) {
  if (width < 1 || !(width & 1) || width > 33) return fail(WCA_ERR_INVALID, "median filter width %d must be odd and in [1, 33]", width);
  return WCA_OK;
}

int check_maps(int L, int H, int n, int F) {
  if (L < 1 || H < 1 || n < 1 || n > MAX_TOK) return fail(WCA_ERR_INVALID, "bad shape L=%d H=%d n=%d", L, H, n);
  if (F < 1 || F > N_CTX) return fail(WCA_ERR_TOO_LONG, "F=%d outside [1,%d]", F, N_CTX);
  return WCA_OK;
}

int check_aggregation(const wca_align_opts* o) {
  if (o->aggregation != WCA_AGGR_MEAN && o->aggregation != WCA_AGGR_TOPK) return fail(WCA_ERR_INVALID, "aggregation %d", o->aggregation);
  if (o->aggregation == WCA_AGGR_TOPK && o->topk < 1) return fail(WCA_ERR_INVALID, "topk must be > 0 (timing.py:92)");
  return WCA_OK;
}

int validate_lengths(int B, int n_tok_max, const int32_t* n_tok, const int32_t* max_frames, int* Fmax_out) {
  if (n_tok_max > MAX_TOK) return fail(WCA_ERR_TOO_LONG, "n_tok %d > %d", n_tok_max, MAX_TOK);
// ... 427 lines not shown
int wca_probe_strict_tp(wca_engine* e, int n_heads, const int32_t* word_end_row_host, int n_hyp, const double* ref_times_host, int n_ref,
                        const uint8_t* same_word_host, double tolerance, int32_t* tp_host) {
  if (!e || !tp_host || (n_hyp > 0 && !word_end_row_host) || (n_ref > 0 && !ref_times_host) || (n_hyp > 0 && n_ref > 0 && !same_word_host))
    return fail(WCA_ERR_INVALID, "null argument");
  if (e->probe_LH <= 0) return fail(WCA_ERR_STATE, "wca_probe_strict_tp needs a preceding wca_probe_heads");
  if (n_heads != e->probe_LH) return fail(WCA_ERR_INVALID, "n_heads %d != the %d heads of the preceding wca_probe_heads", n_heads, e->probe_LH);
  if (n_hyp < 0 || n_ref < 0 || n_ref > 512) return fail(WCA_ERR_INVALID, "n_hyp=%d n_ref=%d outside [0, 512]", n_hyp, n_ref);
  for (int i = 0; i < n_hyp; ++i)
    if (word_end_row_host[i] < 0 || word_end_row_host[i] >= e->probe_N)
      return fail(WCA_ERR_INVALID, "word end row %d = %d outside the %d aligned token rows", i, word_end_row_host[i], e->probe_N);
  HIPCHK(hipSetDevice(e->device));
  const int LH = e->probe_LH;
  const size_t b_wb = align_up(sizeof(int) * (size_t)std::max(n_hyp, 1), 256), b_y = align_up(sizeof(double) * (size_t)std::max(n_ref, 1), 256),
               b_eq = align_up((size_t)std::max(n_hyp * n_ref, 1), 256), b_tp = sizeof(int) * (size_t)LH;
  HIPCHK(e->tmp0.ensure(b_wb + b_y + b_eq + b_tp));
  char* base = (char*)e->tmp0.p;
  if (n_hyp) HIPCHK(hipMemcpyAsync(base, word_end_row_host, sizeof(int) * (size_t)n_hyp, hipMemcpyHostToDevice, e->stream));
  if (n_ref) HIPCHK(hipMemcpyAsync(base + b_wb, ref_times_host, sizeof(double) * (size_t)n_ref, hipMemcpyHostToDevice, e->stream));
  if (n_hyp && n_ref) HIPCHK(hipMemcpyAsync(base + b_wb + b_y, same_word_host, (size_t)n_hyp * n_ref, hipMemcpyHostToDevice, e->stream));
  HIPCHK(launch_probe_strict((const int*)e->probe_jump.p, e->probe_N, LH, (const int*)base, n_hyp, (const double*)(base + b_wb), n_ref,
                             (const unsigned char*)(base + b_wb + b_y), tolerance, (int*)(base + b_wb + b_y + b_eq), e->stream));
  HIPCHK(hipMemcpyAsync(tp_host, base + b_wb + b_y + b_eq, b_tp, hipMemcpyDeviceToHost, e->stream));
  HIPCHK(hipStreamSynchronize(e->stream));
  return WCA_OK;
}

int wca_attention_weights(wca_engine* e, const float* qk_dev, int L, int H, int n, int ld, int max_frames, int medfilt_width,
                          float qk_scale, float* weights_out_dev) {
  if (!e || !qk_dev || !weights_out_dev) return fail(WCA_ERR_INVALID, "null argument");
  if (L < 1 || H < 1 || n < 1) return fail(WCA_ERR_INVALID, "bad shape L=%d H=%d n=%d", L, H, n);
  if (n > MAX_TOK) return fail(WCA_ERR_TOO_LONG, "n=%d > %d", n, MAX_TOK);
  if (max_frames < 1 || ld < max_frames) return fail(WCA_ERR_INVALID, "max_frames=%d must be in [1, ld=%d]", max_frames, ld);
  if (max_frames > N_CTX) return fail(WCA_ERR_TOO_LONG, "max_frames=%d > %d", max_frames, N_CTX);
  WCA_TRY(check_medfilt(medfilt_width));
  WCA_TRY(enter(e));
  int32_t nt = n, nf = max_frames;
  int* rows[4];
  WCA_TRY(stage_meta(e, 1, nullptr, &nt, &nf, nullptr, rows));
  HeadStatsArgs h;
  return run_head_stats(e, e->stream, &h, qk_dev, ld, false, weights_out_dev, false, rows[1], rows[2], n, max_frames, L * H, 1, medfilt_width,
                        qk_scale, 1.f, 1.f, 0.f);
}

int wca_default_find_alignment(wca_engine* e, const float* ws_dev, int L, int H, int n, int F, const int32_t* heads_host, int n_heads,
                                int sot_len, float* weights_norm_out_dev, float* matrix_host, int32_t* text_idx_host,
                                int32_t* time_idx_host, int32_t* path_len_host) {
  if (!e || !ws_dev || !heads_host || !path_len_host) return fail(WCA_ERR_INVALID, "null argument");
  const int LH = L * H, N = n - sot_len - 1;
  if (n_heads < 1) return fail(WCA_ERR_INVALID, "empty alignment head list");
  WCA_TRY(check_maps(L, H, n, F));
  if (sot_len < 0 || N < 1) return fail(WCA_ERR_INVALID, "n=%d leaves no rows after the [sot_len:-1] slice", n);
  for (int i = 0; i < n_heads; ++i)
    if (heads_host[i] < 0 || heads_host[i] >= LH) return fail(WCA_ERR_INVALID, "alignment head %d out of range", heads_host[i]);
  WCA_TRY(enter(e));
  const size_t norm_elems = (size_t)n_heads * n * F;
  HIPCHK(e->tmp1.ensure(sizeof(int) * (size_t)n_heads + (weights_norm_out_dev ? 0 : sizeof(float) * norm_elems) + 256));
  int* sel_dev = reinterpret_cast<int*>(e->tmp1.p);
  float* norm = weights_norm_out_dev ? weights_norm_out_dev
                                     : reinterpret_cast<float*>(reinterpret_cast<char*>(e->tmp1.p) + align_up(sizeof(int) * (size_t)n_heads, 256));
  HIPCHK(hipMemcpyAsync(sel_dev, heads_host, sizeof(int) * n_heads, hipMemcpyHostToDevice, e->stream));
  HIPCHK(hipStreamSynchronize(e->stream));
  HIPCHK(launch_stdmean_normalize(ws_dev, sel_dev, n_heads, n, F, norm, e->stream));
  HIPCHK(e->matrix.ensure(sizeof(float) * (size_t)n * F));
  HIPCHK(launch_mean_heads(norm, n_heads, n, F, sot_len, 1, (float*)e->matrix.p, e->stream));
  WCA_TRY(dtw_dev_common(e, (const float*)e->matrix.p, 1, N, F, false));
  return read_path(e, N, F, text_idx_host, time_idx_host, path_len_host, matrix_host);
}

int wca_align_batch_enqueue(wca_engine* e, const float* pcm_dev, int64_t pcm_stride, const int32_t* n_samples_host,
                            const int64_t* tokens_dev, int n_tok_max, const int32_t* n_tok_host, const int32_t* max_frames_host,
                            int batch, const wca_align_opts* o) {
  return wca_align_batch_enqueue_ex(e, pcm_dev, pcm_stride, n_samples_host, tokens_dev, n_tok_max, n_tok_host, max_frames_host, batch, o, 0);
}

int wca_align_batch_enqueue_ex(wca_engine* e, const float* pcm_dev, int64_t pcm_stride, const int32_t* n_samples_host,
                               const int64_t* tokens_dev, int n_tok_max, const int32_t* n_tok_host, const int32_t* max_frames_host,
                               int batch, const wca_align_opts* o, int32_t vocab_end) {
  return align_enqueue(e, pcm_dev, pcm_stride, n_samples_host, tokens_dev, n_tok_max, n_tok_host, max_frames_host, batch, o, vocab_end, nullptr);
}

int wca_align_batch_enqueue_open(wca_engine* e, const float* pcm_dev, int64_t pcm_stride, const int32_t* n_samples_host,
                                 const int64_t* tokens_dev, int n_tok_max, const int32_t* n_tok_host, const int32_t* max_frames_host,
                                 int batch, const wca_align_opts* o, int32_t vocab_end, const int32_t* open_end_host) {
  if (!e || !open_end_host) return fail(WCA_ERR_INVALID, "null argument");
  return align_enqueue(e, pcm_dev, pcm_stride, n_samples_host, tokens_dev, n_tok_max, n_tok_host, max_frames_host, batch, o, vocab_end,
                       open_end_host);
}

static int align_enqueue(wca_engine* e, const float* pcm_dev, int64_t pcm_stride, const int32_t* n_samples_host, const int64_t* tokens_dev,
                         int n_tok_max, const int32_t* n_tok_host, const int32_t* max_frames_host, int batch, const wca_align_opts* o,
                         int32_t vocab_end, const int32_t* open_end_host) {
  if (!e || !tokens_dev || !n_tok_host || !max_frames_host || !o) return fail(WCA_ERR_INVALID, "null argument");
  const bool want_open = open_end_host != nullptr;
  if (vocab_end < 0 || vocab_end > e->dims.n_vocab) return fail(WCA_ERR_INVALID, "vocab_end %d outside (0, %d] (0 = no token log-probs)", vocab_end, e->dims.n_vocab);
  const bool want_lp = vocab_end > 0;
  const bool reuse_enc = (pcm_dev == nullptr);
  if (reuse_enc && (e->enc_q.empty() || e->enc_q.front().batch != batch))
    return fail(WCA_ERR_STATE, "pcm_dev == NULL re-uses the oldest state left by wca_encode_batch / wca_greedy_decode for the same batch; there is none");
  if (!reuse_enc && !n_samples_host) return fail(WCA_ERR_INVALID, "null argument");
  if (!reuse_enc && !e->enc_q.empty()) {
    for (auto& st : e->enc_q)
      if (!st.decoded && !st.detected) return fail(WCA_ERR_STATE, "an encoded batch is waiting for wca_greedy_decode / wca_align_batch_enqueue(pcm_dev = NULL)");
    for (auto& st : e->enc_q) e->slot_busy[st.slot] = false;
    e->enc_q.clear();
  }
  if (e->enq_count - e->fetch_count >= 2) return fail(WCA_ERR_STATE, "two batches already in flight: call wca_align_batch_fetch first");
  if (batch < 1 || batch > e->max_batch) return fail(WCA_ERR_INVALID, "batch %d outside [1,%d]", batch, e->max_batch);
  WCA_TRY(check_aggregation(o));
  WCA_TRY(check_medfilt(o->medfilt_width));
  int Fmax = 0;
  WCA_TRY(validate_lengths(batch, n_tok_max, n_tok_host, max_frames_host, &Fmax));
  if (!reuse_enc) WCA_TRY(check_pcm_lengths(n_samples_host, batch, pcm_stride));
  WCA_TRY(check_ready(e));
  const wca_model_dims& D = e->dims;
  const int LH = D.n_text_layer * D.n_text_head;
  const int Fpad = (Fmax + 3) & ~3;
  std::vector<int32_t> dn(batch);
  for (int b = 0; b < batch; ++b) {
    dn[b] = n_tok_host[b] - o->sot_len - 1;
    if (dn[b] < 0) dn[b] = 0;
  }
  int* rows[4];
  hipStream_t s2 = e->overlap ? e->stream2 : e->stream;
  WCA_TRY(stage_meta(e, batch, reuse_enc ? nullptr : n_samples_host, n_tok_host, max_frames_host, dn.data(), rows, reuse_enc ? s2 : nullptr));
  int* lp_rows[4] = {nullptr, nullptr, nullptr, nullptr};
  int lp_R = 0, lp_nmax = 0;
  if (want_lp) {
    std::vector<int32_t> off(batch);
    for (int b = 0; b < batch; ++b) {
      const int nt = std::max(0, n_tok_host[b] - o->sot_len - 2);
      off[b] = lp_R;
      lp_R += nt;
      lp_nmax = std::max(lp_nmax, nt);
    }
    WCA_TRY(stage_meta(e, batch, off.data(), nullptr, nullptr, nullptr, lp_rows, reuse_enc ? s2 : nullptr));
  }
  int* open_rows[4] = {nullptr, nullptr, nullptr, nullptr};
  if (want_open) {
    std::vector<int32_t> flags(batch);
    for (int b = 0; b < batch; ++b) flags[b] = open_end_host[b] ? 1 : 0;
    WCA_TRY(stage_meta(e, batch, flags.data(), nullptr, nullptr, nullptr, open_rows, reuse_enc ? s2 : nullptr));
  }
  int bs;
  if (reuse_enc) {
    bs = e->enc_q.front().slot;
    e->enc_q.pop_front();
    record(e, 0);
    record(e, 1);
    record(e, 2);
    record(e, 3);
  } else {
    WCA_TRY(kv_slot_or_fail(e, &bs));
    e->slot_busy[bs] = true;
    if (int rc = run_phase1(e, nullptr, pcm_dev, pcm_stride, rows[0], batch, bs, !want_lp)) {
      e->slot_busy[bs] = false;
      return rc;
    }
  }
  half_t* kvbuf = bs ? e->kv_alt : e->kv;
  HIPCHK(hipStreamWaitEvent(s2, e->ev_kv[bs], 0));
  HIPCHK(hipMemsetAsync(e->err_dev, 0, sizeof(int), s2));
  HIPCHK(e->cap.ensure(sizeof(float) * (size_t)batch * LH * n_tok_max * Fpad));
  WCA_TRY(run_decoder(e, tokens_dev, batch, n_tok_max, (float*)e->cap.p, Fpad, Fmax, nullptr, s2, kvbuf, want_lp));
  record(e, 4, s2);
  HeadStatsArgs h;
  WCA_TRY(run_head_stats(e, s2, &h, (const float*)e->cap.p, Fpad, false, nullptr, true, rows[1], rows[2], n_tok_max, Fmax, LH, batch, o->medfilt_width,
                         o->qk_scale, o->w_colnorm, o->w_rownorm, o->w_coverage));
  record(e, 5, s2);
  WCA_TRY(run_select_aggregate_dtw(e, s2, h, rows[3], o, D.n_text_layer, open_rows[0]));
  if (want_lp) {
    HIPCHK(e->lp_out.ensure(sizeof(float) * (size_t)batch * n_tok_max));
    WCA_TRY(run_token_logprobs(e, s2, tokens_dev, batch, n_tok_max, o->sot_len, vocab_end, rows[1], lp_rows[0], lp_R, lp_nmax, (float*)e->lp_out.p));
  }
  record(e, 7, s2);
  const int k = o->aggregation == WCA_AGGR_TOPK ? o->topk : 0;
  const int rs = (int)(e->enq_count & 1);
  const ResLayout at = res_layout(batch, n_tok_max, k, want_lp, want_open);
  WCA_TRY(ensure_res_host(e, rs, at.ints));
  int* res = e->res_host[rs];
  if (want_lp) HIPCHK(hipMemcpyAsync(res + at.lp, e->lp_out.p, sizeof(float) * (size_t)batch * n_tok_max, hipMemcpyDeviceToHost, s2));
  HIPCHK(hipMemcpyAsync(res + at.flags, e->err_dev, sizeof(int), hipMemcpyDeviceToHost, s2));
  HIPCHK(hipMemcpyAsync(res + at.flags + 1, e->err_dev + 1 + bs, sizeof(int), hipMemcpyDeviceToHost, s2));
  if (n_tok_max - o->sot_len - 1 >= 1) HIPCHK(hipMemcpyAsync(res + at.jump, e->jump.p, sizeof(int) * (size_t)batch * n_tok_max, hipMemcpyDeviceToHost, s2));
  if (k > 0) HIPCHK(hipMemcpyAsync(res + at.sel, e->sel.p, sizeof(int) * (size_t)batch * k, hipMemcpyDeviceToHost, s2));
  if (want_open) HIPCHK(hipMemcpyAsync(res + at.open, e->dtw_out.p, 2 * sizeof(int) * (size_t)batch, hipMemcpyDeviceToHost, s2));
  record(e, 8, s2);
  HIPCHK(hipEventRecord(e->res_ev[rs], s2));
  e->res_batch[rs] = batch;
  e->res_ntok[rs] = n_tok_max;
  e->res_topk[rs] = k;
  e->res_lp[rs] = want_lp;
  e->res_open[rs] = want_open;
  e->res_kvslot[rs] = bs;
  e->last_batch = batch;
  e->enq_count++;
  return WCA_OK;
}

int wca_encode_batch(wca_engine* e, const float* mel_dev, const float* pcm_dev, int64_t pcm_stride, const int32_t* n_samples_host, int batch) {
  if (!e) return fail(WCA_ERR_INVALID, "null engine");
  if ((mel_dev == nullptr) == (pcm_dev == nullptr)) return fail(WCA_ERR_INVALID, "pass exactly one of mel_dev / pcm_dev");
  if (pcm_dev && !n_samples_host) return fail(WCA_ERR_INVALID, "null argument");
  if (batch < 1 || batch > e->max_batch) return fail(WCA_ERR_INVALID, "batch %d outside [1,%d]", batch, e->max_batch);
  if (pcm_dev) WCA_TRY(check_pcm_lengths(n_samples_host, batch, pcm_stride));
  WCA_TRY(check_ready(e));
  int slot;
  WCA_TRY(kv_slot_or_fail(e, &slot));
  int* rows[4] = {nullptr, nullptr, nullptr, nullptr};
  if (pcm_dev) WCA_TRY(stage_meta(e, batch, n_samples_host, nullptr, nullptr, nullptr, rows));
  e->slot_busy[slot] = true;
  if (int rc = run_phase1(e, mel_dev, pcm_dev, pcm_stride, rows[0], batch, slot)) {
    e->slot_busy[slot] = false;
    return rc;
  }
  e->enc_q.push_back({slot, batch, false});
  return WCA_OK;
}

int wca_align_batch_fetch(wca_engine* e, int batch, int n_tok_max, int topk, int32_t* jump_frame_host, int32_t* sel_idx_host) {
  return wca_align_batch_fetch_ex(e, batch, n_tok_max, topk, jump_frame_host, sel_idx_host, nullptr);
}

int wca_align_batch_fetch_ex(wca_engine* e, int batch, int n_tok_max, int topk, int32_t* jump_frame_host, int32_t* sel_idx_host,
                             float* token_logprob_host) {
  return align_fetch(e, batch, n_tok_max, topk, jump_frame_host, sel_idx_host, token_logprob_host, nullptr, nullptr);
}

int wca_align_batch_fetch_open(wca_engine* e, int batch, int n_tok_max, int topk, int32_t* jump_frame_host, int32_t* sel_idx_host,
                               float* token_logprob_host, int32_t* end_row_host, float* score_host) {
  return align_fetch(e, batch, n_tok_max, topk, jump_frame_host, sel_idx_host, token_logprob_host, end_row_host, score_host);
}

static int align_fetch(wca_engine* e, int batch, int n_tok_max, int topk, int32_t* jump_frame_host, int32_t* sel_idx_host,
                       float* token_logprob_host, int32_t* end_row_host, float* score_host) {
  if (!e) return fail(WCA_ERR_INVALID, "null engine");
  if (e->fetch_count >= e->enq_count) return fail(WCA_ERR_STATE, "nothing to fetch");
  const int rs = (int)(e->fetch_count & 1);
  if (batch != e->res_batch[rs] || n_tok_max != e->res_ntok[rs]) return fail(WCA_ERR_STATE, "fetch does not match the oldest pending enqueue");
  if (sel_idx_host && e->res_topk[rs] > 0 && topk != e->res_topk[rs]) return fail(WCA_ERR_STATE, "topk does not match the pending enqueue");
  if (token_logprob_host && !e->res_lp[rs]) return fail(WCA_ERR_STATE, "token log-probs requested, but the pending batch was enqueued without them (vocab_end = 0)");
  if ((end_row_host || score_host) && !e->res_open[rs])
    return fail(WCA_ERR_STATE, "end rows requested, but the pending batch was not enqueued with wca_align_batch_enqueue_open");
  HIPCHK(hipSetDevice(e->device));
  HIPCHK(hipEventSynchronize(e->res_ev[rs]));
  const ResLayout at = res_layout(batch, n_tok_max, e->res_topk[rs], e->res_lp[rs], e->res_open[rs]);
  const int* res = e->res_host[rs];
  if (jump_frame_host) memcpy(jump_frame_host, res + at.jump, sizeof(int) * (size_t)batch * n_tok_max);
  if (sel_idx_host && e->res_topk[rs] > 0) memcpy(sel_idx_host, res + at.sel, sizeof(int) * (size_t)batch * topk);
  if (e->res_kvslot[rs] >= 0) e->slot_busy[e->res_kvslot[rs]] = false;
  e->res_kvslot[rs] = -1;
  e->fetch_count++;
  if (token_logprob_host) memcpy(token_logprob_host, res + at.lp, sizeof(float) * (size_t)batch * n_tok_max);
  if (end_row_host) memcpy(end_row_host, res + at.open, sizeof(int) * (size_t)batch);
  if (score_host) memcpy(score_host, res + at.open + batch, sizeof(float) * (size_t)batch);
  const int flag = res[at.flags] | (res[at.flags + 1] & 2);
  if (flag & 2) return fail(WCA_ERR_HIP, "LayerNorm statistics hand-off timed out inside a GEMM epilogue (a workgroup of a row panel never arrived)");
  if (flag == ERR_TARGET_VOCAB)
    return fail(WCA_ERR_INVALID, "a teacher token is outside the scored vocabulary [0, vocab_end) (its log-prob is NaN)");
  if (flag)
    return fail(WCA_ERR_INVALID, "a token id is outside the model's vocabulary [0, %d) (tokenizer / checkpoint mismatch?)", e->dims.n_vocab);
  return WCA_OK;
}

int wca_align_batch(wca_engine* e, const float* pcm_dev, int64_t pcm_stride, const int32_t* n_samples_host, const int64_t* tokens_dev,
                    int n_tok_max, const int32_t* n_tok_host, const int32_t* max_frames_host, int batch, const wca_align_opts* o,
                    int32_t* jump_frame_host, int32_t* sel_idx_host) {
  WCA_TRY(wca_align_batch_enqueue(e, pcm_dev, pcm_stride, n_samples_host, tokens_dev, n_tok_max, n_tok_host, max_frames_host, batch, o));
  return wca_align_batch_fetch(e, batch, n_tok_max, o->aggregation == WCA_AGGR_TOPK ? o->topk : 0, jump_frame_host, sel_idx_host);
}

int wca_token_logprobs(wca_engine* e, const float* logits_dev, int rows, int ld, int vocab_end, const int64_t* targets_dev, float* out_dev) {
  if (!e || !logits_dev || !targets_dev || !out_dev) return fail(WCA_ERR_INVALID, "null argument");
  if (vocab_end < 1 || vocab_end > e->dims.n_vocab) return fail(WCA_ERR_INVALID, "vocab_end %d outside (0, %d]", vocab_end, e->dims.n_vocab);
  if (rows < 0 || ld < vocab_end) return fail(WCA_ERR_INVALID, "rows %d / ld %d (need rows >= 0, ld >= vocab_end = %d)", rows, ld, vocab_end);
  WCA_TRY(enter(e));
  if (rows == 0) return WCA_OK;
  int* err = e->err_dev + 3;
  HIPCHK(hipMemsetAsync(err, 0, sizeof(int), e->stream));
  HIPCHK(launch_token_logprob(logits_dev, ld, vocab_end, rows, targets_dev, nullptr, 0, out_dev, err, ERR_TARGET_VOCAB, e->stream));
  HIPCHK(hipMemcpyAsync(e->err_host + 3, err, sizeof(int), hipMemcpyDeviceToHost, e->stream));
  HIPCHK(hipStreamSynchronize(e->stream));
  if (e->err_host[3]) return fail(WCA_ERR_INVALID, "a target token is outside [0, vocab_end = %d) (its log-prob is NaN)", vocab_end);
  return WCA_OK;
}

}
```

### whisper-char-alignment_amd/csrc/engine_audio.hip

```cpp
#include "engine_internal.h"

using namespace wca;

namespace {

int logmel_tables(const wca_engine* e, LogMelTables* t) {
  if (!e->have_filters) return fail(WCA_ERR_STATE, "mel_filters not loaded (wca_load_weight(\"mel_filters\"))");
  t->filters = e->mel_filters;
  t->filt_lo = e->filt_lo;
  t->filt_hi = e->filt_hi;
  t->window = e->window;
  t->twiddle = e->twiddle;
  t->precise = e->split ? 1 : 0;
  t->n_mels = e->dims.n_mels;
  return WCA_OK;
}

int resample_table_dev(wca_engine* e, int sr_in, const ResamplePlan& pl, const wca_engine::ResampleTable** out) {
  constexpr size_t RS_TABLES_MAX = 8;
  auto it = std::find_if(e->rs_tables.begin(), e->rs_tables.end(), [&](const wca_engine::ResampleTable& t) { return t.sr_in == sr_in; });
  if (it == e->rs_tables.end()) {
    const size_t count = (size_t)pl.L * pl.n_taps;
    std::vector<double> h(count);
    resample_table(pl, h.data());
    std::vector<float> hf(count);
    for (int p = 0; p < pl.L; ++p)
      for (int i = 0; i < pl.n_taps; ++i)
        hf[pl.home == RESAMPLE_HOME_LDS ? (size_t)i * pl.L + p : (size_t)p * pl.n_taps + i] = (float)h[(size_t)p * pl.n_taps + i];
    if (e->rs_tables.size() >= RS_TABLES_MAX) {
      HIPCHK(hipFree(e->rs_tables.front().dev));
      e->rs_tables.erase(e->rs_tables.begin());
    }
    float* dev = nullptr;
    HIPCHK(hipMalloc(&dev, sizeof(float) * count));
    hipError_t ce = hipMemcpy(dev, hf.data(), sizeof(float) * count, hipMemcpyHostToDevice);
    if (ce != hipSuccess) {
      (void)hipFree(dev);
      HIPCHK(ce);
    }
    e->rs_tables.push_back({sr_in, pl, dev});
    it = e->rs_tables.end() - 1;
  }
  *out = &*it;
  return WCA_OK;
}

}

namespace wca {

int check_pcm_lengths(const int32_t* n_samples_host, int batch, int64_t pcm_stride) {
  for (int b = 0; b < batch; ++b)
    if (n_samples_host[b] < 0 || n_samples_host[b] > 480000 || n_samples_host[b] > pcm_stride)
      return fail(WCA_ERR_INVALID, "n_samples[%d]=%d invalid (pad_or_trim to <= 480000 first)", b, n_samples_host[b]);
  return WCA_OK;
}

int run_logmel(wca_engine* e, const float* pcm_dev, int64_t pcm_stride, const int* n_samples_dev, int B, float* mel_out, bool want_tm) {
  LogMelArgs a{};
  WCA_TRY(logmel_tables(e, &a));
  a.pcm = pcm_dev;
  a.pcm_stride = pcm_stride;
  a.n_samples = n_samples_dev;
  a.mel_out = mel_out;
  a.mel_tm = want_tm ? e->mel_tm : nullptr;
  a.n_mels_pad = (e->split ? 2 : 1) * e->dims.n_mels;
  a.tm_lo = e->split ? e->dims.n_mels : 0;
  a.scratch = e->mel_scratch;
  a.gmax = e->gmax;
  a.B = B;
  HIPCHK(launch_logmel(a, e->stream));
  return WCA_OK;
}

}

extern "C" {

int wca_log_mel(wca_engine* e, const float* pcm_dev, int64_t pcm_stride, const int32_t* n_samples_host, int batch, float* mel_out_dev) {
  if (!e || !pcm_dev || !n_samples_host || !mel_out_dev) return fail(WCA_ERR_INVALID, "null argument");
  if (batch < 1 || batch > e->max_batch) return fail(WCA_ERR_INVALID, "batch %d outside [1,%d]", batch, e->max_batch);
  WCA_TRY(check_pcm_lengths(n_samples_host, batch, pcm_stride));
  WCA_TRY(enter(e));
  int* rows[4];
  WCA_TRY(stage_meta(e, batch, n_samples_host, nullptr, nullptr, nullptr, rows));
  return run_logmel(e, pcm_dev, pcm_stride, rows[0], batch, mel_out_dev, false);
}

int wca_log_mel_long(wca_engine* e, const float* pcm_dev, int64_t n_samples, float* mel_out_dev, int64_t ld, int64_t* n_frames_out) {
  if (!e || !mel_out_dev || (!pcm_dev && n_samples > 0)) return fail(WCA_ERR_INVALID, "null argument");
  if (n_samples < 0 || n_samples > INT32_MAX - 480000) return fail(WCA_ERR_INVALID, "n_samples %lld outside [0, 2^31 - 480001]", (long long)n_samples);
  const int64_t T = (n_samples + 480000) / 160;
  if (n_frames_out) *n_frames_out = T;
  if (ld < T) return fail(WCA_ERR_INVALID, "ld %lld < %lld frames of %lld samples + 30 s", (long long)ld, (long long)T, (long long)n_samples);
  LogMelLongArgs a{};
  WCA_TRY(logmel_tables(e, &a));
  WCA_TRY(enter(e));
  a.pcm = pcm_dev;
  a.n_samples = n_samples;
  a.mel_out = mel_out_dev;
  a.ld = ld;
  a.n_frames = T;
  a.gmax = e->gmax;
  HIPCHK(launch_logmel_long(a, e->stream));
  return WCA_OK;
}

int wca_mel_window(wca_engine* e, const float* mel_long_dev, int64_t ld, int64_t n_frames, const int32_t* seek_host, const int32_t* size_host,
                   int batch, float* mel_out_dev) {
  if (!e || !mel_long_dev || !seek_host || !size_host || !mel_out_dev) return fail(WCA_ERR_INVALID, "null argument");
  if (batch < 1 || batch > e->max_batch) return fail(WCA_ERR_INVALID, "batch %d outside [1,%d]", batch, e->max_batch);
  if (n_frames < 1 || ld < n_frames) return fail(WCA_ERR_INVALID, "n_frames %lld / ld %lld invalid", (long long)n_frames, (long long)ld);
  for (int b = 0; b < batch; ++b) {
    if (size_host[b] < 1 || size_host[b] > N_FRAMES) return fail(WCA_ERR_INVALID, "size[%d]=%d outside [1,%d]", b, size_host[b], N_FRAMES);
    if (seek_host[b] < 0 || (int64_t)seek_host[b] + size_host[b] > n_frames)
      return fail(WCA_ERR_INVALID, "window %d: seek %d + size %d outside the %lld frames", b, seek_host[b], size_host[b], (long long)n_frames);
  }
  WCA_TRY(enter(e));
  int* rows[4];
  WCA_TRY(stage_meta(e, batch, seek_host, size_host, nullptr, nullptr, rows));
  HIPCHK(launch_mel_window(mel_long_dev, ld, e->dims.n_mels, rows[0], rows[1], batch, mel_out_dev, e->stream));
  return WCA_OK;
}

int wca_quiet_cuts(wca_engine* e, const float* mel_long_dev, int64_t ld, int64_t content_frames, int n_pieces, int radius, int half_width,
                   int32_t* cuts_host, int32_t* level_host) {
  if (!e || !mel_long_dev || !cuts_host) return fail(WCA_ERR_INVALID, "null argument");
  if (n_pieces < 2 || n_pieces > QUIET_PIECES_MAX) return fail(WCA_ERR_INVALID, "n_pieces %d outside [2,%d]", n_pieces, QUIET_PIECES_MAX);
  if (radius < 1 || radius > QUIET_RADIUS_MAX) return fail(WCA_ERR_INVALID, "radius %d outside [1,%d]", radius, QUIET_RADIUS_MAX);
  if (half_width < 0 || half_width > QUIET_HALF_WIDTH_MAX) return fail(WCA_ERR_INVALID, "half_width %d outside [0,%d]", half_width, QUIET_HALF_WIDTH_MAX);
  if (content_frames > ld || content_frames > INT32_MAX)
    return fail(WCA_ERR_INVALID, "content_frames %lld beyond ld %lld or 2^31 - 1", (long long)content_frames, (long long)ld);
  if (content_frames / n_pieces < 2 * radius + 2)
    return fail(WCA_ERR_INVALID, "%lld frames in %d pieces leave %lld per piece: fewer than 2 radius + 2 = %d", (long long)content_frames, n_pieces,
                (long long)(content_frames / n_pieces), 2 * radius + 2);
  if (e->dims.n_mels > 128) return fail(WCA_ERR_INVALID, "n_mels %d > 128: the smoothed level would leave int32", e->dims.n_mels);
  WCA_TRY(enter(e));
  const int n = n_pieces - 1;
  HIPCHK(e->quiet_out.ensure(2 * sizeof(int) * (size_t)n));
  int* out_dev = (int*)e->quiet_out.p;
  HIPCHK(launch_quiet_cuts(mel_long_dev, ld, e->dims.n_mels, content_frames, n_pieces, radius, half_width, out_dev, out_dev + n, e->stream));
  std::vector<int32_t> out(2 * (size_t)n);
  HIPCHK(hipMemcpyAsync(out.data(), out_dev, sizeof(int32_t) * out.size(), hipMemcpyDeviceToHost, e->stream));
  HIPCHK(hipStreamSynchronize(e->stream));
  cuts_host[0] = 0;
  memcpy(cuts_host + 1, out.data(), sizeof(int32_t) * (size_t)n);
  cuts_host[n_pieces] = (int32_t)content_frames;
  if (level_host) memcpy(level_host, out.data() + n, sizeof(int32_t) * (size_t)n);
  return WCA_OK;
}

int wca_resample_plan(int sr_in, int32_t* L, int32_t* M, int32_t* W, int32_t* n_taps) {
  ResamplePlan pl;
  if (resample_plan(sr_in, &pl)) return fail(WCA_ERR_INVALID, "sr_in %d outside [%d, %d]", sr_in, RESAMPLE_SR_MIN, RESAMPLE_SR_MAX);
  if (L) *L = pl.L;
  if (M) *M = pl.M;
  if (W) *W = pl.W;
  if (n_taps) *n_taps = pl.n_taps;
  return WCA_OK;
}

int wca_resample_table(int sr_in, double* table_out) {
  if (!table_out) return fail(WCA_ERR_INVALID, "null argument");
  ResamplePlan pl;
  if (resample_plan(sr_in, &pl)) return fail(WCA_ERR_INVALID, "sr_in %d outside [%d, %d]", sr_in, RESAMPLE_SR_MIN, RESAMPLE_SR_MAX);
  resample_table(pl, table_out);
  return WCA_OK;
}

int wca_resample_16k(wca_engine* e, const float* in_dev, int channels, int64_t ld, int64_t n_in, int sr_in, float* out_dev, int64_t out_cap,
                     int64_t* n_out) {
  if (!e || !n_out || (n_in > 0 && (!in_dev || !out_dev))) return fail(WCA_ERR_INVALID, "null argument");
  if (channels < 1 || channels > 8) return fail(WCA_ERR_INVALID, "channels %d outside [1, 8]", channels);
  ResamplePlan pl;
  if (resample_plan(sr_in, &pl)) return fail(WCA_ERR_INVALID, "sr_in %d outside [%d, %d]", sr_in, RESAMPLE_SR_MIN, RESAMPLE_SR_MAX);
  const int64_t n_max = INT32_MAX - 480000;
  if (n_in < 0 || n_in > ld || n_in > n_max * 24) return fail(WCA_ERR_INVALID, "n_in %lld outside [0, ld = %lld]", (long long)n_in, (long long)ld);
  const int64_t n = (n_in * pl.L + pl.M - 1) / pl.M;
  if (n > n_max) return fail(WCA_ERR_INVALID, "%lld samples at %d Hz give %lld at 16 kHz: more than 2^31 - 480001", (long long)n_in, sr_in, (long long)n);
  *n_out = n;
  if (out_cap < n) return fail(WCA_ERR_INVALID, "out_cap %lld < %lld output samples", (long long)out_cap, (long long)n);
  if (n == 0) return WCA_OK;
  WCA_TRY(enter(e));
  ResampleArgs a{};
  a.in = in_dev;
  a.channels = channels;
  a.ld = ld;
  a.n_in = n_in;
  a.out = out_dev;
  a.n_out = n;
  a.max_blocks = 3 * (e->n_cu > 0 ? e->n_cu : 256);
  if (sr_in != RESAMPLE_SR_OUT) {
    const wca_engine::ResampleTable* t = nullptr;
    WCA_TRY(resample_table_dev(e, sr_in, pl, &t));
    a.plan = &t->plan;
    a.table = t->dev;
  }
  HIPCHK(launch_resample(a, e->stream));
  return WCA_OK;
}

}
```

### whisper-char-alignment_amd/csrc/engine_forward.hip

```cpp
#include "engine_internal.h"

using namespace wca;

namespace {

thread_local int g_gemm_cu_limit = 0;

}

namespace wca {

hipError_t gemm(wca_engine* e, hipStream_t s, Gemm g) {
  g.cu_limit = g_gemm_cu_limit;
  if (g.c_lo > 0 && g.out_mode == 0) g.out_mode = 4;
  if (g.w_plain != nullptr && use_wlo(e) && e->wlo_bases.count(g.w_plain)) {
    GemmArgs x = flat(g.A, g.lda, g.w_lo ? g.w_lo : wlo_of(e, g.w_plain), g.k_plain, g.C, g.ldc, g.M, g.N, g.k_plain);
    x.a_rows_per_batch = g.a_rows_per_batch;
    x.a_batch_stride = g.a_batch_stride;
    x.cu_limit = g_gemm_cu_limit;
    x.site = g.site;
    x.out_mode = 2;
    if (g.out_mode != 2) {
      GrowBuf& tmp = e->wlo_tmp[s == e->stream ? 0 : 1];
      if (hipError_t he = tmp.ensure((size_t)g.M * g.N * sizeof(float)); he != hipSuccess) return he;
      x.C = tmp.p;
      x.ldc = g.N;
      x.out_mode = 1;
      g.addend = (const float*)tmp.p;
      g.ld_addend = g.N;
    }
    if (hipError_t he = launch_gemm(x, s); he != hipSuccess) return he;
  }
  if (g.a_lo > 0 && !plan_gemm(g, e->n_cu).pair()) {
    g.W = g.w_pair;
    g.K = g.ldw = 2 * g.k_plain;
    g.a_lo = 0;
  }
  return launch_gemm(g, s);
}

namespace {

void mark_site(wca_engine* e, hipStream_t s, int site, int li, int which) {
  if (e->profiling && site >= 0 && li >= 0 && li < 33) {
    (void)hipEventRecord(e->kev[site][li][which], s);
    e->kev_set[site][li] = true;
  }
}

int dec_gemm(wca_engine* e, hipStream_t s, int ws, Gemm g, half_t* xn_scratch = nullptr) {
  const bool ln = g.A32 != nullptr;
  const int M = g.M, N = g.N, K = g.K, T_max = g.kv_tmax;
  const int sk = gemm_rows_pick_splitk(K);
  const bool fits = sk <= 1 || (g.kv_k == nullptr && (size_t)((M + 63) / 64) * ((N + 15) / 16) <= e->sk_tiles &&
                                gemm_rows_workspace_bytes(M, N, sk) <= e->sk_floats * sizeof(float));
  if (e->dec_fused && M <= DEC_ROWS_MAX && gemm_rows_supported(M, N, K, ln) && fits) {
    g.lda32 = K;
    g.ln_eps = 1e-5f;
    g.splitk = sk;
    g.sk_part = e->sk_part[ws];
    g.sk_cnt = e->sk_cnt[ws];
    g.kv_bs = (long)T_max * K;
    g.kv_d = g.kv_k ? N / 3 : 0;
    if (!g.kv_k) g.kv_t_rows = nullptr;
    HIPCHK(launch_gemm_rows(g, s));
    return WCA_OK;
  }
  Gemm t = flat(g.A, g.lda, g.W, g.ldw, g.C, g.ldc, M, N, K);
  if (ln) {
    HIPCHK(launch_layernorm_f16(g.A32, g.ln_gamma, g.ln_beta, xn_scratch, M, K, 1e-5f, s));
    t.A = xn_scratch;
    t.lda = K;
  }
  t.bias = g.bias;
  t.gelu = g.gelu;
  t.out_mode = g.out_mode;
  t.site = g.site;
  t.sk_part = e->sk_big[1 + ws];
  t.sk_bytes = e->sk_big_bytes;
  HIPCHK(gemm(e, s, t));
  if (g.kv_k) HIPCHK(launch_kv_append(reinterpret_cast<const half_t*>(g.C), g.kv_k, g.kv_v, M, T_max, StepPos{g.kv_t, g.kv_t_rows}, N / 3, s));
  return WCA_OK;
}

struct EvSlots {
  int gemm_site, gemm_li, ln_site, ln_li;
};
int gemm_residual_ln(wca_engine* e, hipStream_t s, Gemm g, const float* gamma, const float* beta, half_t* xn, bool allow_fused, const EvSlots& slots) {
  mark_site(e, s, slots.gemm_site, slots.gemm_li, 0);
  GemmArgs f = g;
  f.out_mode = 3;
  f.ln_gamma = gamma;
  f.ln_beta = beta;
  f.ln_out = xn;
  f.ln_ld = g.N;
  f.ln_eps = 1e-5f;
  f.ln_stats = e->ln_stats;
  f.ln_cnt = e->ln_cnt;
  f.ln_err = e->ln_err ? e->ln_err : e->err_dev;
  if (allow_fused && !e->split && plan_gemm(f, e->n_cu).kernel == GemmKernel::Persist256LN) {
    HIPCHK(launch_gemm(f, s));
    mark_site(e, s, slots.gemm_site, slots.gemm_li, 1);
    return WCA_OK;
  }
  g.out_mode = 2;
  g.sk_part = e->sk_big[0];
  g.sk_bytes = e->sk_big_bytes;
  HIPCHK(gemm(e, s, g));
  mark_site(e, s, slots.gemm_site, slots.gemm_li, 1);
  mark_site(e, s, slots.ln_site, slots.ln_li, 0);
  HIPCHK(launch_layernorm_f16(reinterpret_cast<const float*>(g.C), gamma, beta, xn, g.M, g.N, 1e-5f, s, (e->split ? 2 : 1) * g.N, e->split ? g.N : 0));
  mark_site(e, s, slots.ln_site, slots.ln_li, 1);
  return WCA_OK;
}

}

int run_encoder(wca_engine* e, int B) {
  const wca_model_dims& D = e->dims;
  const int d = D.n_audio_state, H = D.n_audio_head;
  const bool sp = e->split;
  const int om = sp ? 2 : 1;
  hipStream_t s = e->stream;
  {
    const int k1 = sp ? e->sw.k1pad : e->k1pad;
    Gemm g = flat(e->mel_tm, om * D.n_mels, sp ? e->sw.conv1_w : e->conv1_w, k1, e->h1pad + om * d, om * d, B * N_FRAMES, d, k1);
    g.a_rows_per_batch = N_FRAMES;
    g.a_batch_stride = (long)(N_FRAMES + 2) * om * D.n_mels;
    g.bias = e->conv1_b;
    g.c_rows_per_batch = N_FRAMES;
    g.c_batch_stride = (long)(N_FRAMES + 2) * om * d;
    g.c_lo = sp ? d : 0;
    g.gelu = 1;
    g.site = 3;
    if (sp) {
      g.w_plain = e->conv1_w;
      g.k_plain = k1;
      g.w_lo = e->sw.conv1_wlo;
    }
    HIPCHK(gemm(e, s, g));
  }
  {
    Gemm g = flat(e->h1pad, 2 * om * d, sp ? e->sw.conv2_w : e->conv2_w, 3 * om * d, e->x, d, B * N_CTX, d, 3 * om * d);
    g.a_rows_per_batch = N_CTX;
    g.a_batch_stride = (long)(N_FRAMES + 2) * om * d;
    g.bias = e->conv2_b;
    g.pos = e->enc_pos;
    g.pos_period = N_CTX;
    g.gelu = 1;
    g.out_mode = 1;
    g.site = 3;
    if (sp) {
      g.w_plain = e->conv2_w;
      g.k_plain = 3 * om * d;
      g.w_lo = e->sw.conv2_wlo;
    }
    HIPCHK(gemm(e, s, g));
  }
  const int M = B * N_CTX;
  const float scale = 1.0f / std::sqrt((float)(d / H));
  memset(e->kev_set, 0, sizeof(e->kev_set));
  auto mark = [&](int site, int li, int which) { mark_site(e, s, site, li, which); };
  mark(WCA_SITE_LN1, 0, 0);
  HIPCHK(launch_layernorm_f16(e->x, e->enc[0].ln1_g, e->enc[0].ln1_b, e->xn, M, d, 1e-5f, s, om * d, sp ? d : 0));
  mark(WCA_SITE_LN1, 0, 1);
  for (int li = 0; li < D.n_audio_layer; ++li) {
    const LayerW& l = e->enc[li];
    const LayerW& w2 = sp ? e->sw.enc[li] : l;
    mark(WCA_SITE_QKV, li, 0);
    Gemm gq = flat(e->xn, sp, l.qkv_w, w2.qkv_w, d, e->qkv, om * 3 * d, M, 3 * d);
    gq.bias = l.qkv_b;
    gq.c_lo = sp ? 3 * d : 0;
    gq.site = 1;
    HIPCHK(gemm(e, s, gq));
    mark(WCA_SITE_QKV, li, 1);
    AttnArgs a{};
    a.Q = e->qkv;
    a.K = e->qkv + d;
    a.V = e->qkv + 2 * d;
    a.q_bs = a.k_bs = a.v_bs = (long)N_CTX * om * 3 * d;
    a.q_rs = a.k_rs = a.v_rs = om * 3 * d;
    a.O = e->att;
    a.o_bs = (long)N_CTX * om * d;
    a.o_rs = om * d;
    a.split = sp ? 1 : 0;
    a.q_lo = a.k_lo = a.v_lo = 3 * d;
    a.o_lo = d;
    a.nq = N_CTX;
    a.nk = N_CTX;
    a.H = H;
    a.B = B;
    a.scale = scale;
    a.causal = 0;
    mark(WCA_SITE_ATTN, li, 0);
    HIPCHK(launch_attention(a, s));
    mark(WCA_SITE_ATTN, li, 1);
    Gemm go = flat(e->att, sp, l.out_w, w2.out_w, d, e->x, d, M, d);
    go.bias = l.out_b;
    go.site = 1;
    WCA_TRY(gemm_residual_ln(e, s, go, l.ln2_g, l.ln2_b, e->xn, e->fuse_ln, {WCA_SITE_OUT, li, WCA_SITE_LN2, li}));
    mark(WCA_SITE_FC1, li, 0);
    Gemm g1 = flat(e->xn, sp, l.fc1_w, w2.fc1_w, d, e->hid, om * 4 * d, M, 4 * d);
    g1.bias = l.fc1_b;
    g1.gelu = 1;
    g1.c_lo = sp ? 4 * d : 0;
    g1.site = 1;
    HIPCHK(gemm(e, s, g1));
    mark(WCA_SITE_FC1, li, 1);
    const bool last = li + 1 == D.n_audio_layer;
    Gemm g2 = flat(e->hid, sp, l.fc2_w, w2.fc2_w, 4 * d, e->x, d, M, d);
    g2.bias = l.fc2_b;
    g2.site = 4;
    WCA_TRY(gemm_residual_ln(e, s, g2, last ? e->lnpost_g : e->enc[li + 1].ln1_g, last ? e->lnpost_b : e->enc[li + 1].ln1_b, e->xn, e->fuse_ln,
                             {WCA_SITE_FC2, li, WCA_SITE_LN1, li + 1}));
  }
  return WCA_OK;
}

int run_cross_kv(wca_engine* e, int B, half_t* kvbuf, bool skip_last_v) {
  if (!kvbuf) kvbuf = e->kv;
  const wca_model_dims& D = e->dims;
  const int d = D.n_audio_state, dt = D.n_text_state, L = D.n_text_layer;
  const int n_cols = L * 2 * dt - (skip_last_v ? dt : 0);
  const bool sp = e->split;
  Gemm g = flat(e->xn, sp, e->kv_w, e->sw.kv_w, d, kvbuf, (sp ? 2 : 1) * L * 2 * dt, B * N_CTX, n_cols);
  g.bias = e->kv_b;
  g.c_lo = sp ? (long)L * 2 * dt : 0;
  g.site = 3;
  HIPCHK(gemm(e, e->stream, g));
  return WCA_OK;
}

struct DecPass {
  hipStream_t s;
  int ws;
  int B, nq, b0;
  bool pair;
  const half_t* kv;
  half_t* cache;
  int B_all, T_max;
  StepPos pos;
  const int* nk_rows() const { return pos.rows ? pos.rows + B_all : nullptr; }
  half_t* scatter;
  float* cap;
  int Fpad, Fcap;
  int l0, l1;
  bool stop_at_capture;
};

namespace {

int dec_linear(wca_engine* e, const DecPass& p, Gemm g, const half_t* W2, half_t* xn) {
  if (!p.pair) return dec_gemm(e, p.s, p.ws, g, xn);
  const bool f16_out = g.out_mode == 0;
  if (g.A32) {
    HIPCHK(launch_layernorm_f16(g.A32, g.ln_gamma, g.ln_beta, xn, g.M, g.K, 1e-5f, p.s, 2 * g.K, g.K));
    g.A = xn;
  }
  Gemm m = flat(g.A, true, g.W, W2, g.K, g.C, (f16_out ? 2 : 1) * g.ldc, g.M, g.N);
  m.bias = g.bias;
  m.gelu = g.gelu;
  m.out_mode = g.out_mode;
  m.site = g.site;
  m.c_lo = f16_out ? g.N : 0;
  m.sk_part = e->sk_big[1 + p.ws];
  m.sk_bytes = e->sk_big_bytes;
  HIPCHK(gemm(e, p.s, m));
  return WCA_OK;
}

Gemm dec_flat(const half_t* A, const half_t* W, const float* bias, void* C, int M, int N, int K) {
  Gemm g = flat(A, K, W, K, C, N, M, N, K);
  g.bias = bias;
  g.site = 2;
  return g;
}
Gemm dec_flat_ln(const float* x, const float* gamma, const float* beta, const half_t* W, const float* bias, void* C, int M, int N, int K) {
  Gemm g = flat(nullptr, 0, W, K, C, N, M, N, K);
  g.A32 = x;
  g.ln_gamma = gamma;
  g.ln_beta = beta;
  g.bias = bias;
  g.site = 2;
  return g;
}

AttnArgs attn_common(const wca_engine* e, const DecPass& p, const half_t* q, int q_rs, half_t* o) {
  const int dt = e->dims.n_text_state, H = e->dims.n_text_head, om = p.pair ? 2 : 1;
  AttnArgs a{};
  a.Q = q;
  a.q_bs = (long)p.nq * q_rs;
  a.q_rs = q_rs;
  a.O = o;
  a.o_bs = (long)p.nq * om * dt;
  a.o_rs = om * dt;
  if (p.pair) {
    a.split = 1;
    a.o_lo = dt;
  }
  a.nq = p.nq;
  a.H = H;
  a.B = p.B;
  a.scale = 1.0f / std::sqrt((float)(dt / H));
  return a;
}

AttnArgs self_attn_args(const wca_engine* e, const DecPass& p, const half_t* qkv, half_t* o, const half_t* kc, const half_t* vc) {
  const int dt = e->dims.n_text_state, om = p.pair ? 2 : 1;
  AttnArgs a = attn_common(e, p, qkv, om * 3 * dt, o);
  if (p.cache) {
// ... 38 lines not shown

int run_decoder_layers(wca_engine* e, const DecPass& p) {
  const int dt = e->dims.n_text_state, L = e->dims.n_text_layer;
  const int M = p.B * p.nq, om = p.pair ? 2 : 1;
  const size_t r0 = (size_t)p.b0 * p.nq;
  float* xd = e->xd + r0 * dt;
  half_t* xdn = e->xdn + r0 * om * dt;
  half_t* qkv_d = e->qkv_d + r0 * om * 3 * dt;
  half_t* att_d = e->att_d + r0 * om * dt;
  half_t* q_d = e->q_d + r0 * om * dt;
  half_t* hid_d = e->hid_d + r0 * om * 4 * dt;
  half_t* planes = p.cache ? p.cache : p.scatter;
  const size_t plane = (size_t)p.B_all * p.T_max * dt;
  for (int li = p.l0; li < p.l1; ++li) {
    const LayerW& l = e->dec[li];
    const LayerW& w2 = p.pair ? e->sw.dec[li] : l;
    half_t* kc = planes ? planes + (size_t)(2 * li) * plane + (size_t)p.b0 * p.T_max * dt : nullptr;
    half_t* vc = planes ? kc + plane : nullptr;
    Gemm g = dec_flat_ln(xd, l.ln1_g, l.ln1_b, l.qkv_w, l.qkv_b, qkv_d, M, 3 * dt, dt);
    if (p.cache) {
      g.kv_k = kc;
      g.kv_v = vc;
      g.kv_tmax = p.T_max;
      g.kv_t = p.pos.t;
      g.kv_t_rows = p.pos.rows;
    }
    WCA_TRY(dec_linear(e, p, g, w2.qkv_w, xdn));
    if (p.scatter) HIPCHK(launch_kv_scatter(qkv_d, kc, vc, p.B, p.nq, p.T_max, dt, p.s));
    HIPCHK(launch_attention(self_attn_args(e, p, qkv_d, att_d, kc, vc), p.s));
    g = dec_flat(att_d, l.out_w, l.out_b, xd, M, dt, dt);
    g.out_mode = 2;
    WCA_TRY(dec_linear(e, p, g, w2.out_w, xdn));
    WCA_TRY(dec_linear(e, p, dec_flat_ln(xd, l.lnc_g, l.lnc_b, l.cq_w, l.cq_b, q_d, M, dt, dt), w2.cq_w, xdn));
    HIPCHK(launch_attention(cross_attn_args(e, p, li, q_d, att_d), p.s));
    if (li == L - 1 && p.stop_at_capture) break;
    g = dec_flat(att_d, l.co_w, l.co_b, xd, M, dt, dt);
    g.out_mode = 2;
    WCA_TRY(dec_linear(e, p, g, w2.co_w, xdn));
    g = dec_flat_ln(xd, l.ln2_g, l.ln2_b, l.fc1_w, l.fc1_b, hid_d, M, 4 * dt, dt);
    g.gelu = 1;
    WCA_TRY(dec_linear(e, p, g, w2.fc1_w, xdn));
    g = dec_flat(hid_d, l.fc2_w, l.fc2_b, xd, M, dt, 4 * dt);
    g.out_mode = 2;
    WCA_TRY(dec_linear(e, p, g, w2.fc2_w, xdn));
  }
  return WCA_OK;
}

int dec_logits(wca_engine* e, const DecPass& p, const float* x, half_t* xn, int M, float* logits) {
  const wca_model_dims& D = e->dims;
  Gemm g = dec_flat_ln(x, e->lnf_g, e->lnf_b, e->tok_emb, nullptr, logits, M, D.n_vocab, D.n_text_state);
  g.out_mode = 1;
  g.site = 3;
  return dec_linear(e, p, g, e->sw.tok_emb, xn);
}

}

int run_decoder(wca_engine* e, const int64_t* tokens_dev, int B, int n, float* cap, int Fpad, int Fcap, float* logits_out, hipStream_t s,
                const half_t* kvbuf, bool finish_last) {
  const wca_model_dims& D = e->dims;
  DecPass p{};
  p.s = s ? s : e->stream;
  p.B = B;
  p.nq = n;
  p.pair = e->split;
  p.kv = kvbuf ? kvbuf : e->kv;
  p.cap = cap;
  p.Fpad = Fpad;
  p.Fcap = Fcap;
  p.l1 = D.n_text_layer;
  p.stop_at_capture = !logits_out && !finish_last;
  HIPCHK(launch_embed(tokens_dev, e->tok_emb, e->dec_pos, e->xd, B, n, D.n_text_state, D.n_vocab, e->err_dev, p.s,
                      (e->split && use_wlo(e) && e->wlo_bases.count(e->tok_emb)) ? wlo_of(e, e->tok_emb) : nullptr));
  WCA_TRY(run_decoder_layers(e, p));
  if (logits_out) WCA_TRY(dec_logits(e, p, e->xd, e->xdn, B * n, logits_out));
  return WCA_OK;
}

int run_decode_step(wca_engine* e, hipStream_t s, int ws, const half_t* kvbuf, const int* tokens, int b0, int B, int B_all, StepPos pos,
                    int T_max, bool want_logits, int phase) {
  const wca_model_dims& D = e->dims;
  const int dt = D.n_text_state, L = D.n_text_layer;
  DecPass p{};
  p.s = s;
  p.ws = ws;
  p.B = B;
  p.nq = 1;
  p.b0 = b0;
  p.kv = kvbuf + (size_t)b0 * N_CTX * (e->split ? 2 : 1) * L * 2 * dt;
  p.cache = (half_t*)e->dec_cache.p;
  p.B_all = B_all;
  p.T_max = T_max;
  p.pos = pos;
  p.l0 = phase == -2 ? 0 : phase;
  p.l1 = phase == -2 ? L : (phase >= 0 && phase < L ? phase + 1 : phase);
  float* xd = e->xd + (size_t)b0 * dt;
  if (phase == -2 || phase == -1)
    HIPCHK(launch_embed_step(tokens + (size_t)b0 * T_max, T_max, pos, e->tok_emb, e->dec_pos, xd, B, dt, D.n_vocab, s));
  WCA_TRY(run_decoder_layers(e, p));
  if (want_logits && (phase == -2 || phase == L))
    WCA_TRY(dec_logits(e, p, xd, e->xdn + (size_t)b0 * dt, B, (float*)e->dec_logits.p + (size_t)b0 * D.n_vocab));
  return WCA_OK;
}

int run_decode_prefill(wca_engine* e, hipStream_t s, const half_t* kvbuf, const int* tokens, int B, int n, int T_max, StepPos last, StepPos sot) {
  const int dt = e->dims.n_text_state;
  DecPass p{};
  p.s = s;
  p.B = B;
  p.nq = n;
  p.kv = kvbuf;
  p.scatter = (half_t*)e->dec_cache.p;
  p.B_all = B;
  p.T_max = T_max;
  p.l1 = e->dims.n_text_layer;
  HIPCHK(launch_embed_prefix(tokens, T_max, n, e->tok_emb, e->dec_pos, e->xd, B, dt, e->dims.n_vocab, s));
  WCA_TRY(run_decoder_layers(e, p));
  const int R = ((last.rows ? sot.rows != nullptr : sot.t >= 0) ? 2 : 1) * B;
  float* xg = (float*)e->dec_gather.p;
  HIPCHK(launch_gather_rows(e->xd, xg, B, n, last, sot, dt, s));
  return dec_logits(e, p, xg, e->xdn, R, (float*)e->dec_logits.p);
}

}

namespace {

__global__ void mel_to_tm_kernel(const float* __restrict__ mel, half_t* __restrict__ tm, int n_mels, int B, int row, int lo_off) {
  const int b = blockIdx.y;
  const long e0 = (long)blockIdx.x * blockDim.x + threadIdx.x;
  if (e0 >= (long)n_mels * N_FRAMES) return;
  const int t = (int)(e0 / n_mels), m = (int)(e0 - (long)t * n_mels);
  const float v = mel[((long)b * n_mels + m) * N_FRAMES + t];
  const half_t hv = (half_t)v;
  half_t* o = tm + ((long)b * (N_FRAMES + 2) + t + 1) * row + m;
  o[0] = hv;
  if (lo_off) o[lo_off] = (half_t)(v - (float)hv);
}

}

namespace wca {

int mel_to_tm(wca_engine* e, const float* mel_dev, int batch) {
  const wca_model_dims& D = e->dims;
  const size_t nel = (size_t)D.n_mels * N_FRAMES;
  dim3 grid((unsigned)((nel + 255) / 256), batch);
  hipLaunchKernelGGL(mel_to_tm_kernel, grid, dim3(256), 0, e->stream, mel_dev, e->mel_tm, D.n_mels, batch, (e->split ? 2 : 1) * D.n_mels, e->split ? D.n_mels : 0);
  HIPCHK(hipGetLastError());
  return WCA_OK;
}

int run_phase1(wca_engine* e, const float* mel_dev, const float* pcm_dev, int64_t pcm_stride, const int* n_samples_dev, int batch, int slot,
               bool skip_last_v) {
  half_t* kvbuf = slot ? e->kv_alt : e->kv;
  record(e, 0);
  if (pcm_dev) {
    int rc = run_logmel(e, pcm_dev, pcm_stride, n_samples_dev, batch, nullptr, true);
    if (rc) return rc;
  } else {
    if (int mr = mel_to_tm(e, mel_dev, batch)) return mr;
  }
  record(e, 1);
  e->ln_err = e->err_dev + 1 + slot;
  HIPCHK(hipMemsetAsync(e->ln_err, 0, sizeof(int), e->stream));
  g_gemm_cu_limit = e->part_cus > 0 ? e->n_cu - e->part_cus : 0;
  int rc = run_encoder(e, batch);
  e->ln_err = e->err_dev;
  if (!rc) {
    record(e, 2);
    rc = run_cross_kv(e, batch, kvbuf, skip_last_v);
  }
  g_gemm_cu_limit = 0;
  if (rc) return rc;
  record(e, 3);
  HIPCHK(hipEventRecord(e->ev_kv[slot], e->stream));
  return WCA_OK;
}

}
```

### whisper-char-alignment_amd/csrc/engine_internal.h

```cpp
#pragma once
#include <hip/hip_runtime.h>
#include <rccl/rccl.h>

#include <algorithm>
#include <cmath>
#include <cstdio>
#include <cstdlib>
#include <cstring>
#include <deque>
#include <map>
#include <set>
#include <string>
#include <vector>

#include "../../include/wca.h"
#include "kernels.h"

namespace wca {

int fail(int code, const char* fmt, ...);

#define HIPCHK(expr)                                                                              \
  do {                                                                                            \
    hipError_t _e = (expr);                                                                       \
    if (_e != hipSuccess) return fail(WCA_ERR_HIP, "%s failed: %s (%s:%d)", #expr, hipGetErrorString(_e), __FILE__, __LINE__); \
  } while (0)

constexpr int N_FRAMES = 3000, N_CTX = 1500, MAX_TOK = 448, N_BIN = 201, N_FFT = 400;
constexpr int META_SLOTS = 16;
constexpr int DEC_ROWS_MAX = 128;

#define WCA_TRY(expr)          \
  do {                         \
    const int _rc = (expr);    \
    if (_rc != WCA_OK) return _rc; \
  } while (0)

inline size_t align_up(size_t v, size_t a) { return (v + a - 1) / a * a; }

struct GrowBuf {
  void* p = nullptr;
  size_t bytes = 0;
  hipError_t ensure(size_t need) {
    if (need <= bytes) return hipSuccess;
    if (p) {
      hipError_t e = hipFree(p);
      if (e != hipSuccess) return e;
      p = nullptr;
      bytes = 0;
    }
    need = align_up(need, 1 << 20);
    hipError_t e = hipMalloc(&p, need);
    if (e != hipSuccess) return e;
    bytes = need;
    static const bool poison = std::getenv("WCA_POISON_ALLOC") != nullptr;
    if (poison) {
      e = hipMemset(p, 0xFF, need);
      if (e != hipSuccess) return e;
    }
    return hipSuccess;
  }
  void release() {
    if (p) (void)hipFree(p);
    p = nullptr;
    bytes = 0;
  }
};

struct LayerW {
  float *ln1_g, *ln1_b;
  half_t* qkv_w;
  float* qkv_b;
  half_t* out_w;
  float* out_b;
  float *ln2_g, *ln2_b;
  half_t* fc1_w;
  float* fc1_b;
  half_t* fc2_w;
  float* fc2_b;
  float *lnc_g, *lnc_b;
  half_t* cq_w;
  float* cq_b;
  half_t* co_w;
  float* co_b;
};

}

struct wca_engine {
  wca_model_dims dims;
  int device = 0;
  int max_batch = 1;
  hipStream_t stream = nullptr;
  hipStream_t own_stream = nullptr;
  hipStream_t stream2 = nullptr;
  hipStream_t stream3 = nullptr;
  hipEvent_t ev_kv[2] = {};
  hipEvent_t ev_fork = nullptr, ev_join = nullptr;
  bool finalized = false;
  bool have_filters = false;
  bool profiling = false;
  std::set<std::string> loaded;
  std::map<std::string, size_t> inexact;
  bool allow_rounded = false;
  char* wslab_lo = nullptr;
  std::set<const void*> wlo_bases;
  wca::GrowBuf wlo_tmp[2];

  char* wslab = nullptr;
  size_t wslab_bytes = 0, wslab_used = 0;
  int k1pad = 0;
  wca::half_t *conv1_w = nullptr, *conv2_w = nullptr;
  float *conv1_b = nullptr, *conv2_b = nullptr, *enc_pos = nullptr, *lnpost_g = nullptr, *lnpost_b = nullptr;
  std::vector<wca::LayerW> enc, dec;
  wca::half_t* tok_emb = nullptr;
  float *dec_pos = nullptr, *lnf_g = nullptr, *lnf_b = nullptr;
  wca::half_t* kv_w = nullptr;
  float* kv_b = nullptr;
  float *mel_filters = nullptr, *window = nullptr, *twiddle = nullptr;
  int *filt_lo = nullptr, *filt_hi = nullptr;

  char* aslab = nullptr;
  float* mel_scratch = nullptr;
  unsigned* gmax = nullptr;
  float* mel_f32 = nullptr;
  wca::half_t* mel_tm = nullptr;
  wca::half_t* h1pad = nullptr;
  float* x = nullptr;
  wca::half_t* xn = nullptr;
  wca::half_t* qkv = nullptr;
  wca::half_t* att = nullptr;
  wca::half_t* hid = nullptr;
  wca::half_t* kv = nullptr;
  wca::half_t* kv_alt = nullptr;
  float* xd = nullptr;
  wca::half_t* xdn = nullptr;
  wca::half_t* qkv_d = nullptr;
  wca::half_t* att_d = nullptr;
  wca::half_t* q_d = nullptr;
  wca::half_t* hid_d = nullptr;
  int* meta_dev = nullptr;
  int* meta_host = nullptr;
  int meta_slot = 0;
  unsigned long long* ln_stats = nullptr;
  unsigned* ln_cnt = nullptr;
  float* sk_part[2] = {nullptr, nullptr};
  unsigned* sk_cnt[2] = {nullptr, nullptr};
  size_t sk_floats = 0, sk_tiles = 0;
  float* sk_big[3] = {nullptr, nullptr, nullptr};
  size_t sk_big_bytes = 0;
  int n_cu = 0;
  int* err_dev = nullptr;
  int* ln_err = nullptr;
  int* err_host = nullptr;

  wca::GrowBuf cap, wws, colnorm, scores, sel, selsc, matrix, trace, path, pathlen, jump, tmp0, tmp1;
  wca::GrowBuf dtw_out, dtw_meta;
  wca::GrowBuf quiet_out;
  wca::GrowBuf probe_jump;
  int probe_LH = 0, probe_N = 0;
  wca::GrowBuf dec_cache, dec_tokens, dec_masks, dec_logits, dec_state;
  wca::GrowBuf dec_rows;
  wca::GrowBuf dec_gather;
  int* dec_done_host = nullptr;
  struct ResampleTable { int sr_in; wca::ResamplePlan plan; float* dev; };
  std::vector<ResampleTable> rs_tables;
  int dec_prefill_positions = 0, dec_step_positions = 0;
  struct EncState { int slot; int batch; bool decoded; bool detected = false; };
  std::deque<EncState> enc_q;
  bool slot_busy[2] = {false, false};
  int res_kvslot[2] = {-1, -1};
  int* res_host[2] = {nullptr, nullptr};
  size_t res_host_ints[2] = {0, 0};
  hipEvent_t res_ev[2] = {};
  int res_topk[2] = {0, 0}, res_ntok[2] = {0, 0}, res_batch[2] = {0, 0};
  bool res_open[2] = {false, false};
  bool res_lp[2] = {false, false};
  wca::GrowBuf lp_x, lp_xn, lp_map, lp_logits, lp_out;
  unsigned long enq_count = 0, fetch_count = 0;
  int last_batch = 0;

  hipEvent_t ev[9] = {};
  hipEvent_t kev[WCA_N_SITES][33][2] = {};
  bool kev_set[WCA_N_SITES][33] = {};
  bool split = false;
  char* wslab2 = nullptr;
  bool sw_dirty = true;
  struct SplitW {
    wca::half_t *conv1_w = nullptr, *conv2_w = nullptr, *kv_w = nullptr, *tok_emb = nullptr;
    wca::half_t *conv1_wlo = nullptr, *conv2_wlo = nullptr;
    int k1pad = 0;
    std::vector<wca::LayerW> enc, dec;
  } sw;
  ncclComm_t comm = nullptr;
  int comm_rank = 0, comm_world = 0;
  wca::GrowBuf coll_send, coll_recv;
  bool fuse_ln = false;
  bool overlap = true;
  int part_cus = 0;
  hipStream_t part_s1 = nullptr, part_s2 = nullptr, part_s3 = nullptr;
  hipStream_t saved_s2 = nullptr, saved_s3 = nullptr;
  hipStream_t user_stream = nullptr;
  bool user_stream_set = false;
  bool dec_fused = true;
  int dec_streams = 1;
  bool ev_valid = false;
  float stage_ms[8] = {};
};

namespace wca {

template <typename T>
T* carve(char*& cur, size_t count, size_t align = 256) {
  uintptr_t p = reinterpret_cast<uintptr_t>(cur);
  p = (p + align - 1) / align * align;
  T* r = reinterpret_cast<T*>(p);
  cur = reinterpret_cast<char*>(p + count * sizeof(T));
  return r;
}

inline bool use_wlo(const wca_engine* e) { return e->wslab_lo != nullptr && !e->wlo_bases.empty() && !e->allow_rounded; }
inline const half_t* wlo_of(const wca_engine* e, const half_t* w) {
  return reinterpret_cast<const half_t*>(e->wslab_lo + (reinterpret_cast<const char*>(w) - e->wslab));
}

int check_ready(wca_engine* e);
int stage_meta(wca_engine* e, int B, const int32_t* a0, const int32_t* a1, const int32_t* a2, const int32_t* a3, int** dev_rows, hipStream_t s = nullptr);
int join_phase2(wca_engine* e);
int enter(wca_engine* e);
void record(wca_engine* e, int i, hipStream_t s = nullptr);
int take_kv_slot(wca_engine* e);

size_t layout_weights(wca_engine* e, char* base);
size_t layout_split_weights(wca_engine* e, char* base);
int ensure_split_weights(wca_engine* e);

struct Gemm : GemmArgs {
  const half_t* w_plain = nullptr;
  int k_plain = 0;
  const half_t* w_pair = nullptr;
  const half_t* w_lo = nullptr;
};
inline Gemm flat(const half_t* A, int lda, const half_t* W, int ldw, void* C, int ldc, int M, int N, int K) {
  Gemm g{};
  g.A = A;
  g.lda = lda;
  g.W = W;
  g.ldw = ldw;
  g.C = C;
  g.ldc = ldc;
  g.M = M;
  g.N = N;
  g.K = K;
  return g;
}
inline Gemm flat(const half_t* A, bool pair, const half_t* W1, const half_t* W2, int K, void* C, int ldc, int M, int N) {
  Gemm g = flat(A, (pair ? 2 : 1) * K, W1, K, C, ldc, M, N, K);
  if (pair) {
    g.a_lo = K;
    g.w_plain = W1;
    g.k_plain = K;
    g.w_pair = W2;
  }
  return g;
}
hipError_t gemm(wca_engine* e, hipStream_t s, Gemm g);
int run_encoder(wca_engine* e, int B);
int run_cross_kv(wca_engine* e, int B, half_t* kvbuf = nullptr, bool skip_last_v = false);
int run_decoder(wca_engine* e, const int64_t* tokens_dev, int B, int n, float* cap, int Fpad, int Fcap, float* logits_out, hipStream_t s = nullptr,
                const half_t* kvbuf = nullptr, bool finish_last = false);
int run_decode_step(wca_engine* e, hipStream_t s, int ws, const half_t* kvbuf, const int* tokens, int b0, int B, int B_all, StepPos pos,
                    int T_max, bool want_logits, int phase = -2);
int run_decode_prefill(wca_engine* e, hipStream_t s, const half_t* kvbuf, const int* tokens, int B, int n, int T_max, StepPos last, StepPos sot);
int mel_to_tm(wca_engine* e, const float* mel_dev, int batch);
int run_phase1(wca_engine* e, const float* mel_dev, const float* pcm_dev, int64_t pcm_stride, const int* n_samples_dev, int batch, int slot,
               bool skip_last_v = false);

int check_pcm_lengths(const int32_t* n_samples_host, int batch, int64_t pcm_stride);
int run_logmel(wca_engine* e, const float* pcm_dev, int64_t pcm_stride, const int* n_samples_dev, int B, float* mel_out, bool want_tm);

}
```

### whisper-char-alignment_amd/csrc/kernels.h

```cpp
#pragma once
#include <hip/hip_runtime.h>
#include <stdint.h>

namespace wca {

typedef _Float16 half_t;

enum { DBG_ATTN_SPLIT_VARIANT = 0, DBG_HEAD_STATS_GENERAL, DBG_FAIL_PRECISION_ALLOC, DBG_ATTN_SPLIT_DROP, DBG_GEMM_RING, DBG_SWITCH_COUNT };
int debug_switch(int id);
int set_debug_switch(const char* name, int value);

struct GemmArgs {
  const half_t* A;
  long a_lo;
  int lda;
  int a_rows_per_batch;
  long a_batch_stride;
  const half_t* W;
  int ldw;
  const float* bias;
  void* C;
  int ldc;
  int c_rows_per_batch;
  long c_batch_stride;
  long c_lo;
  const float* addend;
  int ld_addend;
  const float* pos;
  int pos_period;
  int M, N, K;
  int gelu;
  int out_mode;
  unsigned a_bytes, w_bytes;
  int force_tile;
  const float* ln_gamma;
  const float* ln_beta;
  half_t* ln_out;
  int ln_ld;
  float ln_eps;
  unsigned long long* ln_stats;
  unsigned* ln_cnt;
  int* ln_err;
  int site;
  int supertile;
  int cu_limit;
  const float* A32;
  int lda32;
  half_t* kv_k;
  half_t* kv_v;
  long kv_bs;
  int kv_t, kv_d;
  size_t sk_bytes;
  float* sk_part;
  unsigned* sk_cnt;
  int splitk;
  int groups;
  const int* kv_t_rows;
  int kv_tmax;
};
enum GemmForceTile {
  GEMM_TILE_AUTO = 0,
  GEMM_TILE_SKINNY = 64,
  GEMM_TILE_128 = 128,
  GEMM_TILE_256 = 256,
  GEMM_TILE_PERSIST = 257,
  GEMM_TILE_PERSIST_ONE = 258,
};
constexpr int GEMM_LDS_128 = 2 * 2 * 128 * 64 * (int)sizeof(half_t);
constexpr int GEMM_LDS_256 = 2 * 2 * 256 * 64 * (int)sizeof(half_t);
constexpr int GEMM_LDS_256P = GEMM_LDS_256 + 2 * 256 * (int)sizeof(float);
constexpr int GEMM_LDS_256P_LN = GEMM_LDS_256P + (2 * 512 + 2560) * (int)sizeof(float);
constexpr long GEMM_MIN_TILES_256 = 192;

enum class GemmKernel { None , Skinny, Tile128, Tile256, Persist256, Persist256Pair2, Persist256Pair3, Persist256LN };
struct GemmPlan {
  GemmKernel kernel;
  unsigned grid_x, grid_y, block;
  unsigned lds;
  int splitk;
  int supertile;
  unsigned a_bytes, w_bytes;
  int site_used;
  const char* refused;
  bool pair() const { return kernel == GemmKernel::Persist256Pair2 || kernel == GemmKernel::Persist256Pair3; }
};
GemmPlan plan_gemm(const GemmArgs& a, int n_cu);
hipError_t launch_gemm(const GemmArgs& a, hipStream_t s);
hipError_t launch_gemm_rows(const GemmArgs& a, hipStream_t s);
bool gemm_rows_supported(int M, int N, int K, bool layernorm_a);
int gemm_rows_pick_splitk(int K);
size_t gemm_rows_workspace_bytes(int M, int N, int splitk);

struct AttnArgs {
  const half_t* Q; long q_bs; int q_rs;
  const half_t* K; long k_bs; int k_rs;
  const half_t* V; long v_bs; int v_rs;
  half_t* O; long o_bs; int o_rs;
  float* cap;
  long cap_bs; long cap_hs; int cap_ld;
  int cap_cols;
  int nq, nk, H, B;
  float scale;
  int causal;
  int variant;
  int split;
  long q_lo, k_lo, v_lo, o_lo;
  const int* nk_rows;
};
hipError_t launch_attention(const AttnArgs& a, hipStream_t s);
hipError_t launch_attention_split(const AttnArgs& a, hipStream_t s);

hipError_t launch_layernorm_f16(const float* x, const float* gamma, const float* beta, half_t* out,
                                int rows, int d, float eps, hipStream_t s, int ld_out = 0, long lo_off = 0);
hipError_t launch_embed(const int64_t* tokens, const half_t* tok_emb, const float* pos_emb, float* x,
                        int B, int n, int d, int n_vocab, int* err, hipStream_t s, const half_t* tok_emb_lo = nullptr);
hipError_t launch_fill_f16(half_t* p, size_t n, float v, hipStream_t s);

struct StepPos {
  int t;
  const int* rows;
};
hipError_t launch_embed_step(const int* tokens, int T_max, StepPos pos, const half_t* tok_emb, const float* pos_emb, float* x, int B, int d,
                             int n_vocab, hipStream_t s);
hipError_t launch_kv_append(const half_t* qkv, half_t* kc, half_t* vc, int B, int T_max, StepPos pos, int d, hipStream_t s);
hipError_t launch_embed_prefix(const int* tokens, int T_max, int n, const half_t* tok_emb, const float* pos_emb, float* x, int B, int d,
                               int n_vocab, hipStream_t s);
hipError_t launch_kv_scatter(const half_t* qkv, half_t* kc, half_t* vc, int B, int n, int T_max, int d, hipStream_t s);
hipError_t launch_gather_rows(const float* x, float* out, int B, int n, StepPos p0, StepPos p1, int d, hipStream_t s);
struct DecodeSelectArgs {
  const float* logits;
  int ld, n_vocab;
  int* tokens;
  int T_max, cur_len, n_initial;
  const unsigned char* suppress_mask;
  const unsigned char* blank_mask;
  int eot, timestamp_begin;
  int apply_timestamp_rules, max_initial_timestamp_index;
  float* sum_logprob;
  int* n_done;
  const int* cur_len_rows;
  const int* n_initial_rows;
  const int* cap_rows;
  int n_done_idx;
};
hipError_t launch_decode_select(const DecodeSelectArgs& a, int B, hipStream_t s);
hipError_t launch_token_prob(const float* logits, int ld, int n_vocab, int token, float* out, int B, hipStream_t s);
hipError_t launch_f32_to_f16(const float* in, half_t* out, size_t n, hipStream_t s);
hipError_t launch_language_head(const float* x, const float* gamma, const float* beta, const half_t* tok_emb, int B, int d, int n_vocab,
                                int lang_begin, int n_lang, float* probs, int* lang_token, hipStream_t s);
hipError_t launch_gather_text_rows(const float* x, int n_tok_max, int d, int sot_len, const int* n_tok, const int* row_off, int B, int n_text_max,
                                   float* out, int* row_map, hipStream_t s);
hipError_t launch_token_logprob(const float* logits, long ld, int vocab_end, int rows, const int64_t* targets, const int* row_map, int tgt_off,
                                float* out, int* err, int err_bit, hipStream_t s);

struct LogMelTables {
  const float* filters;
  const int* filt_lo;
  const int* filt_hi;
  const float* window;
  const float* twiddle;
  int precise;
  int n_mels;
};
struct LogMelArgs : LogMelTables {
  const float* pcm;
  long pcm_stride;
  const int* n_samples;
  float* mel_out;
  half_t* mel_tm;
  int n_mels_pad;
  int tm_lo;
  float* scratch;
  unsigned* gmax;
  int B;
};
hipError_t launch_logmel(const LogMelArgs& a, hipStream_t s);

struct LogMelLongArgs : LogMelTables {
  const float* pcm;
  long n_samples;
  float* mel_out;
  long ld;
  long n_frames;
  unsigned* gmax;
};
hipError_t launch_logmel_long(const LogMelLongArgs& a, hipStream_t s);

hipError_t launch_mel_window(const float* mel_long, long ld, int n_mels, const int* seek, const int* size, int B, float* out, hipStream_t s);

constexpr int QUIET_PIECES_MAX = 4096, QUIET_RADIUS_MAX = 1500, QUIET_HALF_WIDTH_MAX = 100;
hipError_t launch_quiet_cuts(const float* mel_long, long ld, int n_mels, long content_frames, int n_pieces, int radius, int half_width,
                             int* cuts, int* level, hipStream_t s);

constexpr int RESAMPLE_SR_OUT = 16000, RESAMPLE_SR_MIN = 2000, RESAMPLE_SR_MAX = 384000;
enum { RESAMPLE_HOME_UNIFORM = 0, RESAMPLE_HOME_LDS = 1, RESAMPLE_HOME_GLOBAL = 2 };
struct ResamplePlan {
  int L, M, W, n_taps;
  int home;
  int tile, span_max;
};
int resample_plan(int sr_in, ResamplePlan* pl);
void resample_table(const ResamplePlan& pl, double* h);
struct ResampleArgs {
  const float* in;
  int channels;
  long ld, n_in;
  float* out;
  long n_out;
  const ResamplePlan* plan;
  const float* table;
  int max_blocks;
};
hipError_t launch_resample(const ResampleArgs& a, hipStream_t s);

struct HeadStatsArgs {
  const float* qk;
  long qk_bs; long qk_hs; int qk_ld;
  float* weights;
  long w_bs;
  const int* n_tok;
  const int* n_frames;
  int n_tok_max, n_frames_max;
  float* colnorm;
  float* scores;
  float* rowstats;
  int LH, B, medfilt_width;
  float qk_scale, w_col, w_row, w_cov;
  int input_is_weights;
};
hipError_t launch_head_stats(const HeadStatsArgs& a, hipStream_t s);

hipError_t launch_topk(const float* scores, int LH, int B, int k, int* sel_idx ,
                       float* sel_score , hipStream_t s);

struct AggregateArgs {
  const float* weights; long w_bs; int n_tok_max, n_frames_max;
  const float* colnorm;
  const int* sel_idx;
  int n_sel, head_lo, LH, B;
  const int* n_tok; const int* n_frames;
  int row_lo, row_hi_trim;
  float* matrix;
  const float* qk; long qk_bs; long qk_hs; int qk_ld;
  const float* rowstats;
  int medfilt_width; float qk_scale;
};
hipError_t launch_aggregate(const AggregateArgs& a, hipStream_t s);

hipError_t launch_stdmean_normalize(const float* ws, const int* sel_dev, int n_sel, int n, int F, float* out, hipStream_t s);
hipError_t launch_mean_heads(const float* x, int n_sel, int n, int F, int row_lo, int row_hi_trim, float* matrix, hipStream_t s);

hipError_t launch_probe_strict(const int* jump, int jump_ld, int LH, const int* wb_end, int n_hyp, const double* y, int n_ref,
                               const unsigned char* eq, double tol, int* tp_out, hipStream_t s);

hipError_t launch_median_filter(const float* in, float* out, long rows, int F, int width, hipStream_t s);

struct DtwArgs {
  const float* matrix;
  long m_bs; int ld;
  const int* N;
  const int* M;
  int N_all, M_all;
  int N_max, M_max;
  uint32_t* trace;
  int* path;
  int* path_len;
  int* jump_frame;
  int jump_ld;
  int P;
  const int* open_end;
  int open_all;
  int* end_row;
  float* score;
};
hipError_t launch_dtw(const DtwArgs& a, hipStream_t s);

}
```

### whisper-char-alignment_amd/csrc/logmel.hip

```cpp
#include "kernels.h"
#include "wca_common.h"

namespace wca {

namespace {

constexpr int NFFT = 400, HOP = 160, NBIN = 201, NFRAMES = 3000, NSAMP = 480000;

__device__ __forceinline__ unsigned f2ord(float f) {
  const unsigned u = __float_as_uint(f);
  return (u & 0x80000000u) ? ~u : (u | 0x80000000u);
}
__device__ __forceinline__ float ord2f(unsigned o) {
  const unsigned u = (o & 0x80000000u) ? (o & 0x7fffffffu) : ~o;
  return __uint_as_float(u);
}

__device__ __forceinline__ int active_frames(int n_samples) {
  int na = (n_samples + 200 + HOP - 1) / HOP;
  return na < NFRAMES ? na : NFRAMES;
}

__global__ void logmel_init_kernel(unsigned* gmax, int B) {
  const int i = blockIdx.x * blockDim.x + threadIdx.x;
// ... 16 lines not shown
    long idx = t * HOP - NFFT / 2 + n;
    if (idx < 0) idx = -idx;
    if (idx >= total) idx = 2 * (total - 1) - idx;
    const float x = (idx < ns) ? pcm[idx] : 0.f;
    s.raw[n] = x * a.window[n];
    s.tw[n] = reinterpret_cast<const f32x2*>(a.twiddle)[n];
  }
  __syncthreads();
  for (int n = tid; n <= NFFT / 2; n += 256) {
    if (n == 0 || n == NFFT / 2) {
      s.e[n] = s.raw[n];
      s.o[n] = 0.f;
    } else {
      s.e[n] = s.raw[n] + s.raw[NFFT - n];
      s.o[n] = s.raw[n] - s.raw[NFFT - n];
    }
  }
  __syncthreads();
  if (tid < NBIN) {
    const int k = tid;
    if (a.precise) {
      double re = (double)s.e[0] + ((k & 1) ? -(double)s.e[NFFT / 2] : (double)s.e[NFFT / 2]);
      double im = 0.0;
      int idx = 0;
      for (int n = 1; n < NFFT / 2; ++n) {
        idx += k;
        if (idx >= NFFT) idx -= NFFT;
        const f32x2 tw = s.tw[idx];
        re = fma((double)s.e[n], (double)tw[0], re);
        im = fma((double)s.o[n], (double)tw[1], im);
      }
      const float ref = (float)re, imf = (float)im;
      s.pow[k] = ref * ref + imf * imf;
    } else {
      float re = s.e[0] + ((k & 1) ? -s.e[NFFT / 2] : s.e[NFFT / 2]);
      float im = 0.f;
      int idx = 0;
      for (int n = 1; n < NFFT / 2; ++n) {
        idx += k;
        if (idx >= NFFT) idx -= NFFT;
        const f32x2 tw = s.tw[idx];
        re = fmaf(s.e[n], tw[0], re);
        im = fmaf(s.o[n], tw[1], im);
      }
      s.pow[k] = re * re + im * im;
    }
  }
  __syncthreads();
  float lv = -INFINITY;
  if (tid < a.n_mels) {
    const int m = tid;
    const int lo = a.filt_lo[m], hi = a.filt_hi[m];
    const float* fr = a.filters + (long)m * NBIN;
    float acc = 0.f;
    if (a.precise) {
      double acc64 = 0.0;
      for (int k = lo; k < hi; ++k) acc64 = fma((double)fr[k], (double)s.pow[k], acc64);
      acc = (float)acc64;
    } else {
      for (int k = lo; k < hi; ++k) acc = fmaf(fr[k], s.pow[k], acc);
    }
    lv = log10f(fmaxf(acc, 1e-10f));
    out[(long)m * ld] = lv;
  }
  lv = wave_max(lv);
  if ((tid & 63) == 0) s.max[tid >> 6] = lv;
  __syncthreads();
  if (tid == 0) {
    const float mx = fmaxf(fmaxf(s.max[0], s.max[1]), fmaxf(s.max[2], s.max[3]));
    atomicMax(gmax, f2ord(mx));
  }
}

__global__ __launch_bounds__(256) void logmel_power_kernel(LogMelArgs a) {
  __shared__ FrameLds s;
  const int t = blockIdx.x, b = blockIdx.y;
  const int ns = a.n_samples[b];
  if (t >= active_frames(ns)) return;
  frame_log_mel(a, s, a.pcm + (long)b * a.pcm_stride, ns, NSAMP, t, a.scratch + (long)b * a.n_mels * NFRAMES + t, NFRAMES, a.gmax + b);
}

__global__ __launch_bounds__(256) void logmel_finalize_kernel(LogMelArgs a) {
  const int b = blockIdx.y;
  const int t0 = blockIdx.x * 64;
  const int na = active_frames(a.n_samples[b]);
  const float floorv = ord2f(a.gmax[b]) - 8.0f;
  const float* sc = a.scratch + (long)b * a.n_mels * NFRAMES;
  if (a.mel_out) {
    float* mo = a.mel_out + (long)b * a.n_mels * NFRAMES;
    for (int e = threadIdx.x; e < a.n_mels * 64; e += 256) {
      const int m = e >> 6, t = t0 + (e & 63);
      if (t < NFRAMES) {
        const float v = (t < na) ? sc[(long)m * NFRAMES + t] : -10.0f;
        mo[(long)m * NFRAMES + t] = (fmaxf(v, floorv) + 4.0f) * 0.25f;
      }
    }
  }
  if (a.mel_tm) {
    half_t* mt = a.mel_tm + (long)b * (NFRAMES + 2) * a.n_mels_pad;
    for (int e = threadIdx.x; e < a.n_mels * 64; e += 256) {
      const int tt = e / a.n_mels, m = e - tt * a.n_mels;
      const int t = t0 + tt;
      if (t < NFRAMES) {
        const float v = (t < na) ? sc[(long)m * NFRAMES + t] : -10.0f;
        const float y = (fmaxf(v, floorv) + 4.0f) * 0.25f;
        if (a.tm_lo) {
          const HalfPair pr = split_pair(y);
          mt[(long)(t + 1) * a.n_mels_pad + m] = pr.hi;
          mt[(long)(t + 1) * a.n_mels_pad + a.tm_lo + m] = pr.lo;
        } else {
          mt[(long)(t + 1) * a.n_mels_pad + m] = (half_t)y;
        }
      }
    }
  }
}

__device__ __forceinline__ long active_frames_long(long n_samples, long n_frames) {
  const long na = (n_samples + 200 + HOP - 1) / HOP;
  return na < n_frames ? na : n_frames;
}

__global__ void logmel_long_init_kernel(unsigned* gmax) { *gmax = f2ord(-10.0f); }

__global__ __launch_bounds__(256) void logmel_long_power_kernel(LogMelLongArgs a) {
  __shared__ FrameLds s;
  const long t = blockIdx.x;
  frame_log_mel(a, s, a.pcm, a.n_samples, a.n_samples + NSAMP, t, a.mel_out + t, a.ld, a.gmax);
}

__global__ __launch_bounds__(256) void logmel_long_finalize_kernel(LogMelLongArgs a) {
  const long t = (long)blockIdx.x * 256 + threadIdx.x;
  if (t >= a.n_frames) return;
  const float floorv = ord2f(*a.gmax) - 8.0f;
  float* p = a.mel_out + (long)blockIdx.y * a.ld + t;
  const float v = (t < active_frames_long(a.n_samples, a.n_frames)) ? *p : -10.0f;
  *p = (fmaxf(v, floorv) + 4.0f) * 0.25f;
}

__global__ __launch_bounds__(256) void mel_window_kernel(const float* __restrict__ mel_long, long ld, const int* __restrict__ seek,
                                                         const int* __restrict__ size, float* __restrict__ out) {
  const int t = blockIdx.x * 256 + threadIdx.x, m = blockIdx.y, b = blockIdx.z;
  if (t >= NFRAMES) return;
  const float v = (t < size[b]) ? mel_long[(long)m * ld + seek[b] + t] : 0.f;
  out[((long)b * gridDim.y + m) * NFRAMES + t] = v;
}

}

hipError_t launch_logmel(const LogMelArgs& a, hipStream_t s) {
  if (a.B <= 0) return hipSuccess;
  if (a.n_mels > 256) return hipErrorInvalidValue;
  hipLaunchKernelGGL(logmel_init_kernel, dim3((a.B + 63) / 64), dim3(64), 0, s, a.gmax, a.B);
  hipLaunchKernelGGL(logmel_power_kernel, dim3(NFRAMES, a.B), dim3(256), 0, s, a);
  hipLaunchKernelGGL(logmel_finalize_kernel, dim3((NFRAMES + 63) / 64, a.B), dim3(256), 0, s, a);
  return hipGetLastError();
}

hipError_t launch_logmel_long(const LogMelLongArgs& a, hipStream_t s) {
  if (a.n_mels > 256 || a.n_samples < 0 || a.n_frames != (a.n_samples + NSAMP) / HOP || a.ld < a.n_frames) return hipErrorInvalidValue;
  const long na = (a.n_samples + 200 + HOP - 1) / HOP < a.n_frames ? (a.n_samples + 200 + HOP - 1) / HOP : a.n_frames;
  hipLaunchKernelGGL(logmel_long_init_kernel, dim3(1), dim3(1), 0, s, a.gmax);
  if (na > 0) hipLaunchKernelGGL(logmel_long_power_kernel, dim3((unsigned)na), dim3(256), 0, s, a);
  hipLaunchKernelGGL(logmel_long_finalize_kernel, dim3((unsigned)((a.n_frames + 255) / 256), a.n_mels), dim3(256), 0, s, a);
  return hipGetLastError();
}

hipError_t launch_mel_window(const float* mel_long, long ld, int n_mels, const int* seek, const int* size, int B, float* out, hipStream_t s) {
  if (B <= 0) return hipSuccess;
  hipLaunchKernelGGL(mel_window_kernel, dim3((NFRAMES + 255) / 256, n_mels, B), dim3(256), 0, s, mel_long, ld, seek, size, out);
  return hipGetLastError();
}

}
```

Measured before the change: 351.0.

## Skip padded-silence work in logmel, conv stem and attention tail

Uses host-known sample counts to limit logmel power frames to active audio, and runs the conv1/conv2 GEMMs only over content rows plus boundary rows. The constant padded region is filled by copy kernels that replicate a computed padding row plus positional embeddings. The split attention kernel also processes only half of the last key tile when the tail fits. This cuts encoder front-end work for 10s clips padded to 30s, but it relies on padded rows being identical and adds extra launches plus complex edge handling.

```diff
diff --git a/include/wca.h b/include/wca.h
--- a/include/wca.h
+++ b/include/wca.h
@@ -204,6 +204,7 @@
                      const float* gamma_dev, const float* beta_dev, void* xn_f16_dev, int M, int N, int K, int site);
 int wca_test_gemm_plan(int M, int N, int K, int lda, int out_mode, int gelu, int a_lo, int force_tile, int site, int n_cu, int cu_limit, int flags,
                        int64_t sk_bytes, int32_t* out);
+int wca_test_pad_bounds(int n_samples, int32_t* out);
 typedef struct wca_test_gemm_desc {
   const void* a;
   const void* w;
@@ -259,6 +260,7 @@
 int wca_test_layernorm_split(wca_engine* e, const float* x_dev, const float* g_dev, const float* b_dev, void* out2_f16_dev,
                              int rows, int d);
 int wca_test_encoder(wca_engine* e, const float* mel_dev, int batch, float* xa_out_dev);
+int wca_test_encoded_output(wca_engine* e, int batch, float* xa_out_dev);
 
 int wca_last_stage_ms(wca_engine* e, float* ms8);
 enum {
diff --git a/whisper-char-alignment_amd/_lib.py b/whisper-char-alignment_amd/_lib.py
--- a/whisper-char-alignment_amd/_lib.py
+++ b/whisper-char-alignment_amd/_lib.py
@@ -112,6 +112,8 @@
     "wca_test_decode_select": (_i, [_vp, _vp, _i, _i, _vp, _i, _i, _i, _vp, _vp, C.POINTER(DecodeOpts), _vp, _vp]),
     "wca_test_gemm": (_i, [_vp, _vp, _vp, _vp, _vp, _i, _i, _i, _i, _i]),
     "wca_test_gemm_plan": (_i, [_i, _i, _i, _i, _i, _i, _i, _i, _i, _i, _i, _i, _i64, _pi32]),
+    "wca_test_pad_bounds": (_i, [_i, _pi32]),
+    "wca_test_encoded_output": (_i, [_vp, _i, _vp]),
     "wca_test_gemm_ex": (_i, [_vp, C.POINTER(GemmDesc), _pi32]),
     "wca_test_attention_ex": (_i, [_vp, C.POINTER(AttnDesc)]),
     "wca_test_gemm_ln": (_i, [_vp, _vp, _vp, _vp, _vp, _vp, _vp, _vp, _i, _i, _i, _i]),
diff --git a/whisper-char-alignment_amd/csrc/attention_split.hip b/whisper-char-alignment_amd/csrc/attention_split.hip
--- a/whisper-char-alignment_amd/csrc/attention_split.hip
+++ b/whisper-char-alignment_amd/csrc/attention_split.hip
@@ -413,8 +413,11 @@
   for (int r = 0; r < 16; ++r) cinit[r] = 0.f;
 
   stage(0, 0);
-  auto tile = [&](auto slot_c, int kt) {
+  auto tile = [&](auto slot_c, auto half_c, int kt) {
     constexpr int SLOT = decltype(slot_c)::value;
+    constexpr bool HALF = decltype(half_c)::value != 0;
+    static_assert(!HALF || DROP == 0, "the ablation forms keep the whole tile");
+    constexpr int NKB = HALF ? 1 : 2;
     constexpr int SB = SLOT * SLOT_BYTES;
     asm volatile("s_waitcnt vmcnt(0)" ::: "memory");
     __builtin_amdgcn_s_barrier();
@@ -432,15 +435,27 @@
       kh0[1] = lds_read_b128_asm<SB>(ka[1]);
       kh0[2] = lds_read_b128_asm<SB>(ka[2]);
       kh0[3] = lds_read_b128_asm<SB>(ka[3]);
-      kl1[0] = lds_read_b128_asm<SB + TB + 32 * 128>(ka[0]);
-      kl1[1] = lds_read_b128_asm<SB + TB + 32 * 128>(ka[1]);
-      kl1[2] = lds_read_b128_asm<SB + TB + 32 * 128>(ka[2]);
-      kl1[3] = lds_read_b128_asm<SB + TB + 32 * 128>(ka[3]);
-      kh1[0] = lds_read_b128_asm<SB + 32 * 128>(ka[0]);
-      kh1[1] = lds_read_b128_asm<SB + 32 * 128>(ka[1]);
-      kh1[2] = lds_read_b128_asm<SB + 32 * 128>(ka[2]);
-      kh1[3] = lds_read_b128_asm<SB + 32 * 128>(ka[3]);
-      if constexpr (DROP == 0) {
+      if constexpr (!HALF) {
+        kl1[0] = lds_read_b128_asm<SB + TB + 32 * 128>(ka[0]);
+        kl1[1] = lds_read_b128_asm<SB + TB + 32 * 128>(ka[1]);
+        kl1[2] = lds_read_b128_asm<SB + TB + 32 * 128>(ka[2]);
+        kl1[3] = lds_read_b128_asm<SB + TB + 32 * 128>(ka[3]);
+        kh1[0] = lds_read_b128_asm<SB + 32 * 128>(ka[0]);
+        kh1[1] = lds_read_b128_asm<SB + 32 * 128>(ka[1]);
+        kh1[2] = lds_read_b128_asm<SB + 32 * 128>(ka[2]);
+        kh1[3] = lds_read_b128_asm<SB + 32 * 128>(ka[3]);
+      }
+      if constexpr (DROP == 0 && HALF) {
+        WCA_LGKM_WAIT4(4, kl0[0], kl0[1], kl0[2], kl0[3]);
+        st[0] = __builtin_amdgcn_mfma_f32_32x32x16_f16(kl0[0], qh[0], cinit, 0, 0, 0);
+#pragma unroll
+        for (int ks = 1; ks < 4; ++ks) st[0] = __builtin_amdgcn_mfma_f32_32x32x16_f16(kl0[ks], qh[ks], st[0], 0, 0, 0);
+        WCA_LGKM_WAIT4(0, kh0[0], kh0[1], kh0[2], kh0[3]);
+#pragma unroll
+        for (int ks = 0; ks < 4; ++ks) st[0] = __builtin_amdgcn_mfma_f32_32x32x16_f16(kh0[ks], ql[ks], st[0], 0, 0, 0);
+#pragma unroll
+        for (int ks = 0; ks < 4; ++ks) st[0] = __builtin_amdgcn_mfma_f32_32x32x16_f16(kh0[ks], qh[ks], st[0], 0, 0, 0);
+      } else if constexpr (DROP == 0) {
       WCA_LGKM_WAIT4(12, kl0[0], kl0[1], kl0[2], kl0[3]);
       st[0] = __builtin_amdgcn_mfma_f32_32x32x16_f16(kl0[0], qh[0], cinit, 0, 0, 0);
 #pragma unroll
@@ -505,7 +520,7 @@
     WCA_ISSUE_V32(v0, 0);
     if (kt * KT + KT > a.nk) {
 #pragma unroll
-      for (int kb = 0; kb < 2; ++kb)
+      for (int kb = 0; kb < NKB; ++kb)
 #pragma unroll
         for (int r = 0; r < 16; ++r) {
           const int key = kt * KT + kb * 32 + (r & 3) + 8 * (r >> 2) + 4 * hh;
@@ -518,14 +533,16 @@
       float m2 = max3f(st[0][6], st[0][7], st[0][8]), m3 = max3f(st[0][9], st[0][10], st[0][11]);
       m0 = max3f(m0, st[0][12], st[0][13]);
       m1 = max3f(m1, st[0][14], st[0][15]);
-      m2 = max3f(m2, st[1][0], st[1][1]);
-      m3 = max3f(m3, st[1][2], st[1][3]);
-      m0 = max3f(m0, st[1][4], st[1][5]);
-      m1 = max3f(m1, st[1][6], st[1][7]);
-      m2 = max3f(m2, st[1][8], st[1][9]);
-      m3 = max3f(m3, st[1][10], st[1][11]);
-      m0 = max3f(m0, st[1][12], st[1][13]);
-      m1 = max3f(m1, st[1][14], st[1][15]);
+      if constexpr (!HALF) {
+        m2 = max3f(m2, st[1][0], st[1][1]);
+        m3 = max3f(m3, st[1][2], st[1][3]);
+        m0 = max3f(m0, st[1][4], st[1][5]);
+        m1 = max3f(m1, st[1][6], st[1][7]);
+        m2 = max3f(m2, st[1][8], st[1][9]);
+        m3 = max3f(m3, st[1][10], st[1][11]);
+        m0 = max3f(m0, st[1][12], st[1][13]);
+        m1 = max3f(m1, st[1][14], st[1][15]);
+      }
       mx = fmaxf(max3f(m0, m1, m2), m3);
       mx = xor32_max(mx);
     }
@@ -540,7 +557,7 @@
 #pragma unroll
         for (int r = 0; r < 16; ++r) ot[d][r] *= alpha;
 #pragma unroll
-      for (int kb = 0; kb < 2; ++kb)
+      for (int kb = 0; kb < NKB; ++kb)
 #pragma unroll
         for (int r = 0; r < 16; ++r) st[kb][r] -= delta;
       m_run = m_new;
@@ -552,7 +569,7 @@
     {
       f32x2 psum = f32x2{0.f, 0.f};
 #pragma unroll
-      for (int s4 = 0; s4 < 4; ++s4) {
+      for (int s4 = 0; s4 < 2 * NKB; ++s4) {
         half2_ hq[4], lq[4];
 #pragma unroll
         for (int u = 0; u < 4; ++u) {
@@ -575,7 +592,7 @@
     WCA_S_PIN8(v0la[0], v0lb[0], v0la[1], v0lb[1], v0la[2], v0lb[2], v0la[3], v0lb[3]);
     WCA_ISSUE_V32(v1, 1);
 #pragma unroll
-    for (int s4 = 0; s4 < 4; ++s4) {
+    for (int s4 = 0; s4 < 2 * NKB; ++s4) {
       const half8 wh = __builtin_shufflevector(v0ha[s4], v0hb[s4], 0, 1, 2, 3, 4, 5, 6, 7);
       const half8 wl = __builtin_shufflevector(v0la[s4], v0lb[s4], 0, 1, 2, 3, 4, 5, 6, 7);
       if (!(DROP & 4)) ot[0] = __builtin_amdgcn_mfma_f32_32x32x16_f16(wl, ph[s4], ot[0], 0, 0, 0);
@@ -585,7 +602,7 @@
     WCA_LGKM_WAIT8(0, v1ha[0], v1hb[0], v1ha[1], v1hb[1], v1ha[2], v1hb[2], v1ha[3], v1hb[3]);
     WCA_S_PIN8(v1la[0], v1lb[0], v1la[1], v1lb[1], v1la[2], v1lb[2], v1la[3], v1lb[3]);
 #pragma unroll
-    for (int s4 = 0; s4 < 4; ++s4) {
+    for (int s4 = 0; s4 < 2 * NKB; ++s4) {
       const half8 wh = __builtin_shufflevector(v1ha[s4], v1hb[s4], 0, 1, 2, 3, 4, 5, 6, 7);
       const half8 wl = __builtin_shufflevector(v1la[s4], v1lb[s4], 0, 1, 2, 3, 4, 5, 6, 7);
       if (!(DROP & 4)) ot[1] = __builtin_amdgcn_mfma_f32_32x32x16_f16(wl, ph[s4], ot[1], 0, 0, 0);
@@ -594,9 +611,18 @@
     }
 #undef WCA_ISSUE_V32
   };
-  for (int kt = 0; kt < nkt; kt += 2) {
-    tile(IntC<0>{}, kt);
-    if (kt + 1 < nkt) tile(IntC<1>{}, kt + 1);
+  const int n_full = (DROP == 0 && a.tail_half) ? nkt - 1 : nkt;
+  for (int kt = 0; kt < n_full; kt += 2) {
+    tile(IntC<0>{}, IntC<0>{}, kt);
+    if (kt + 1 < n_full) tile(IntC<1>{}, IntC<0>{}, kt + 1);
+  }
+  if constexpr (DROP == 0) {
+    if (n_full < nkt) {
+      if (n_full & 1)
+        tile(IntC<1>{}, IntC<1>{}, n_full);
+      else
+        tile(IntC<0>{}, IntC<1>{}, n_full);
+    }
   }
 
   const float inv = 1.0f / xor32_sum(l_run);
@@ -642,7 +668,9 @@
   const dim3 grid(((a.nq + 127) / 128) * a.H * a.B), block(256);
   const int variant = a.variant ? a.variant : debug_switch(DBG_ATTN_SPLIT_VARIANT);
   if (!a.causal && !cap && a.nq >= 64 && variant != 1 && (a.o_rs % 8) == 0 && (a.o_lo % 8) == 0) {
-    auto launch32 = [&](auto drop_c) { return launch_lds<attn_split32_kernel<decltype(drop_c)::value>, LDS>(grid, block, LDS, s, a); };
+    AttnArgs a32 = a;
+    a32.tail_half = (a.nk - 1) % KT < KT / 2 && !debug_switch(DBG_PAD_SKIP);
+    auto launch32 = [&](auto drop_c) { return launch_lds<attn_split32_kernel<decltype(drop_c)::value>, LDS>(grid, block, LDS, s, a32); };
     switch (debug_switch(DBG_ATTN_SPLIT_DROP)) {
       case 0: return launch32(IntC<0>{});
       case 1: return launch32(IntC<1>{});
diff --git a/whisper-char-alignment_amd/csrc/debug_switch.cpp b/whisper-char-alignment_amd/csrc/debug_switch.cpp
--- a/whisper-char-alignment_amd/csrc/debug_switch.cpp
+++ b/whisper-char-alignment_amd/csrc/debug_switch.cpp
@@ -16,6 +16,7 @@
     {"fail_precision_alloc", {0}},
     {"attn_split_drop", {0}},
     {"gemm_ring", {0}},
+    {"pad_skip", {0}},
 };
 }
 
diff --git a/whisper-char-alignment_amd/csrc/elementwise.hip b/whisper-char-alignment_amd/csrc/elementwise.hip
--- a/whisper-char-alignment_amd/csrc/elementwise.hip
+++ b/whisper-char-alignment_amd/csrc/elementwise.hip
@@ -202,6 +202,36 @@
   size_t i = (size_t)blockIdx.x * blockDim.x + threadIdx.x;
   const size_t st = (size_t)gridDim.x * blockDim.x;
   for (; i < n; i += st) out[i] = (half_t)in[i];
+}
+
+struct PadDst {
+  int t[3];
+};
+__global__ __launch_bounds__(256) void pad_fill_h1_kernel(half_t* __restrict__ h1pad, int row_w, int B, int src, PadDst dst, const float* __restrict__ pos,
+                                                          int last_row, int d, float* __restrict__ pos_tail) {
+  const int b = blockIdx.y;
+  if (b == B) {
+    if (blockIdx.x != 0) return;
+    for (int j = threadIdx.x; j < d; j += 256) {
+      pos_tail[j] = -0.0f;
+      pos_tail[d + j] = pos[(long)last_row * d + j];
+    }
+    return;
+  }
+  half_t* base = h1pad + (long)b * (3002L * row_w);
+  const half8* sp = reinterpret_cast<const half8*>(base + (long)(src + 1) * row_w);
+  half8* dp = reinterpret_cast<half8*>(base + (long)(dst.t[blockIdx.x] + 1) * row_w);
+  for (int j = threadIdx.x; j < row_w / 8; j += 256) dp[j] = sp[j];
+}
+
+constexpr int PAD_FILL_ROWS = 4;
+__global__ __launch_bounds__(256) void pad_fill_x_kernel(float* __restrict__ x, int rows, int d, int c_row, const float* __restrict__ pos, int t0, int t1) {
+  float* xb = x + (long)blockIdx.y * rows * d;
+  const int ta = t0 + blockIdx.x * PAD_FILL_ROWS, tb = ta + PAD_FILL_ROWS < t1 ? ta + PAD_FILL_ROWS : t1;
+  for (int j = threadIdx.x; j < d / 4; j += 256) {
+    const f32x4 c = reinterpret_cast<const f32x4*>(xb + (long)c_row * d)[j];
+    for (int t = ta; t < tb; ++t) reinterpret_cast<f32x4*>(xb + (long)t * d)[j] = c + reinterpret_cast<const f32x4*>(pos + (long)t * d)[j];
+  }
 }
 
 }
@@ -254,6 +284,25 @@
   return hipGetLastError();
 }
 
+hipError_t launch_pad_fill_h1(half_t* h1pad, int row_w, int B, int src, const int* dst, int n_dst, const float* pos, int last_row, int d, float* pos_tail,
+                              hipStream_t s) {
+  if (B <= 0 || n_dst < 1 || n_dst > 3 || (row_w & 7) || src < 0 || last_row < 0) return hipErrorInvalidValue;
+  PadDst pd{};
+  for (int i = 0; i < n_dst; ++i) {
+    if (dst[i] < 0 || dst[i] >= 3000) return hipErrorInvalidValue;
+    pd.t[i] = dst[i];
+  }
+  hipLaunchKernelGGL(pad_fill_h1_kernel, dim3(n_dst, B + 1), dim3(256), 0, s, h1pad, row_w, B, src, pd, pos, last_row, d, pos_tail);
+  return hipGetLastError();
+}
+
+hipError_t launch_pad_fill_x(float* x, int rows, int d, int B, int c_row, const float* pos, int t0, int t1, hipStream_t s) {
+  if (B <= 0 || t1 <= t0) return hipSuccess;
+  if ((d & 3) || t0 < 0 || t1 > rows || c_row < 0 || c_row >= rows || (c_row >= t0 && c_row < t1 && t1 - t0 != 1)) return hipErrorInvalidValue;
+  hipLaunchKernelGGL(pad_fill_x_kernel, dim3((t1 - t0 + PAD_FILL_ROWS - 1) / PAD_FILL_ROWS, B), dim3(256), 0, s, x, rows, d, c_row, pos, t0, t1);
+  return hipGetLastError();
+}
+
 hipError_t launch_f32_to_f16(const float* in, half_t* out, size_t n, hipStream_t s) {
   if (n == 0) return hipSuccess;
   const int blocks = (int)((n + 255) / 256 < 2048 ? (n + 255) / 256 : 2048);
diff --git a/whisper-char-alignment_amd/csrc/engine.hip b/whisper-char-alignment_amd/csrc/engine.hip
--- a/whisper-char-alignment_amd/csrc/engine.hip
+++ b/whisper-char-alignment_amd/csrc/engine.hip
@@ -207,6 +207,7 @@
   if (e->wslab) (void)hipFree(e->wslab);
   if (e->wslab2) (void)hipFree(e->wslab2);
   if (e->wslab_lo) (void)hipFree(e->wslab_lo);
+  e->pad_pos.release();
   e->wlo_tmp[0].release();
   e->wlo_tmp[1].release();
   if (e->aslab) (void)hipFree(e->aslab);
diff --git a/whisper-char-alignment_amd/csrc/engine_align.hip b/whisper-char-alignment_amd/csrc/engine_align.hip
--- a/whisper-char-alignment_amd/csrc/engine_align.hip
+++ b/whisper-char-alignment_amd/csrc/engine_align.hip
@@ -603,7 +603,7 @@
   } else {
     WCA_TRY(kv_slot_or_fail(e, &bs));
     e->slot_busy[bs] = true;
-    if (int rc = run_phase1(e, nullptr, pcm_dev, pcm_stride, rows[0], batch, bs, !want_lp)) {
+    if (int rc = run_phase1(e, nullptr, pcm_dev, pcm_stride, rows[0], n_samples_host, batch, bs, !want_lp)) {
       e->slot_busy[bs] = false;
       return rc;
     }
@@ -660,7 +660,7 @@
   int* rows[4] = {nullptr, nullptr, nullptr, nullptr};
   if (pcm_dev) WCA_TRY(stage_meta(e, batch, n_samples_host, nullptr, nullptr, nullptr, rows));
   e->slot_busy[slot] = true;
-  if (int rc = run_phase1(e, mel_dev, pcm_dev, pcm_stride, rows[0], batch, slot)) {
+  if (int rc = run_phase1(e, mel_dev, pcm_dev, pcm_stride, rows[0], n_samples_host, batch, slot)) {
     e->slot_busy[slot] = false;
     return rc;
   }
diff --git a/whisper-char-alignment_amd/csrc/engine_audio.hip b/whisper-char-alignment_amd/csrc/engine_audio.hip
--- a/whisper-char-alignment_amd/csrc/engine_audio.hip
+++ b/whisper-char-alignment_amd/csrc/engine_audio.hip
@@ -56,8 +56,20 @@
   return WCA_OK;
 }
 
-int run_logmel(wca_engine* e, const float* pcm_dev, int64_t pcm_stride, const int* n_samples_dev, int B, float* mel_out, bool want_tm) {
+PadBounds pad_bounds(int n) {
+  PadBounds p;
+  p.frames = n >= 480000 ? N_FRAMES : std::min(N_FRAMES, (n + 200 + 159) / 160);
+  p.mel = n <= 0 ? 0 : p.frames;
+  p.conv1 = p.frames + 1 < N_FRAMES - 1 ? p.frames + 1 : N_FRAMES;
+  const int s = (p.frames + 3) / 2;
+  p.conv2 = s < N_CTX - 1 ? s : N_CTX;
+  return p;
+}
+
+int run_logmel(wca_engine* e, const float* pcm_dev, int64_t pcm_stride, const int* n_samples_dev, const int32_t* n_samples_host, int B, float* mel_out,
+               bool want_tm) {
   LogMelArgs a{};
+  for (int b = 0; n_samples_host && !debug_switch(DBG_PAD_SKIP) && b < B; ++b) a.frames = std::max(a.frames, pad_bounds(n_samples_host[b]).frames);
   WCA_TRY(logmel_tables(e, &a));
   a.pcm = pcm_dev;
   a.pcm_stride = pcm_stride;
@@ -84,7 +96,7 @@
   WCA_TRY(enter(e));
   int* rows[4];
   WCA_TRY(stage_meta(e, batch, n_samples_host, nullptr, nullptr, nullptr, rows));
-  return run_logmel(e, pcm_dev, pcm_stride, rows[0], batch, mel_out_dev, false);
+  return run_logmel(e, pcm_dev, pcm_stride, rows[0], n_samples_host, batch, mel_out_dev, false);
 }
 
 int wca_log_mel_long(wca_engine* e, const float* pcm_dev, int64_t n_samples, float* mel_out_dev, int64_t ld, int64_t* n_frames_out) {
@@ -147,6 +159,17 @@
   memcpy(cuts_host + 1, out.data(), sizeof(int32_t) * (size_t)n);
   cuts_host[n_pieces] = (int32_t)content_frames;
   if (level_host) memcpy(level_host, out.data() + n, sizeof(int32_t) * (size_t)n);
+  return WCA_OK;
+}
+
+int wca_test_pad_bounds(int n_samples, int32_t* out) {
+  if (!out) return fail(WCA_ERR_INVALID, "null argument");
+  if (n_samples < 0) return fail(WCA_ERR_INVALID, "n_samples %d < 0", n_samples);
+  const PadBounds p = pad_bounds(n_samples);
+  out[0] = p.mel;
+  out[1] = p.conv1;
+  out[2] = p.conv2;
+  out[3] = p.frames;
   return WCA_OK;
 }
 
diff --git a/whisper-char-alignment_amd/csrc/engine_forward.hip b/whisper-char-alignment_amd/csrc/engine_forward.hip
--- a/whisper-char-alignment_amd/csrc/engine_forward.hip
+++ b/whisper-char-alignment_amd/csrc/engine_forward.hip
@@ -19,6 +19,7 @@
     x.a_batch_stride = g.a_batch_stride;
     x.cu_limit = g_gemm_cu_limit;
     x.site = g.site;
+    x.force_tile = g.force_tile;
     x.out_mode = 2;
     if (g.out_mode != 2) {
       GrowBuf& tmp = e->wlo_tmp[s == e->stream ? 0 : 1];
@@ -116,19 +117,20 @@
 
 }
 
-int run_encoder(wca_engine* e, int B) {
+int run_encoder(wca_engine* e, int B, int pad_row) {
   const wca_model_dims& D = e->dims;
   const int d = D.n_audio_state, H = D.n_audio_head;
   const bool sp = e->split;
   const int om = sp ? 2 : 1;
   hipStream_t s = e->stream;
-  {
-    const int k1 = sp ? e->sw.k1pad : e->k1pad;
-    Gemm g = flat(e->mel_tm, om * D.n_mels, sp ? e->sw.conv1_w : e->conv1_w, k1, e->h1pad + om * d, om * d, B * N_FRAMES, d, k1);
-    g.a_rows_per_batch = N_FRAMES;
+  const int k1 = sp ? e->sw.k1pad : e->k1pad;
+  auto conv1 = [&](int t0, int n) {
+    Gemm g = flat(e->mel_tm + (size_t)t0 * om * D.n_mels, om * D.n_mels, sp ? e->sw.conv1_w : e->conv1_w, k1, e->h1pad + (size_t)(t0 + 1) * om * d, om * d,
+                  B * n, d, k1);
+    g.a_rows_per_batch = n;
     g.a_batch_stride = (long)(N_FRAMES + 2) * om * D.n_mels;
     g.bias = e->conv1_b;
-    g.c_rows_per_batch = N_FRAMES;
+    g.c_rows_per_batch = n;
     g.c_batch_stride = (long)(N_FRAMES + 2) * om * d;
     g.c_lo = sp ? d : 0;
     g.gelu = 1;
@@ -138,15 +140,19 @@
       g.k_plain = k1;
       g.w_lo = e->sw.conv1_wlo;
     }
-    HIPCHK(gemm(e, s, g));
-  }
-  {
-    Gemm g = flat(e->h1pad, 2 * om * d, sp ? e->sw.conv2_w : e->conv2_w, 3 * om * d, e->x, d, B * N_CTX, d, 3 * om * d);
-    g.a_rows_per_batch = N_CTX;
+    return g;
+  };
+  auto conv2 = [&](int s0, int n) {
+    Gemm g = flat(e->h1pad + (size_t)s0 * 2 * om * d, 2 * om * d, sp ? e->sw.conv2_w : e->conv2_w, 3 * om * d, e->x + (size_t)s0 * d, d, B * n, d, 3 * om * d);
+    g.a_rows_per_batch = n;
     g.a_batch_stride = (long)(N_FRAMES + 2) * om * d;
+    if (n != N_CTX) {
+      g.c_rows_per_batch = n;
+      g.c_batch_stride = (long)N_CTX * d;
+    }
     g.bias = e->conv2_b;
-    g.pos = e->enc_pos;
-    g.pos_period = N_CTX;
+    g.pos = e->enc_pos + (size_t)s0 * d;
+    g.pos_period = n;
     g.gelu = 1;
     g.out_mode = 1;
     g.site = 3;
@@ -155,7 +161,40 @@
       g.k_plain = 3 * om * d;
       g.w_lo = e->sw.conv2_wlo;
     }
+    return g;
+  };
+  auto tile_of = [&](Gemm g) {
+    g.cu_limit = g_gemm_cu_limit;
+    if (g.c_lo > 0) g.out_mode = 4;
+    const GemmKernel k = plan_gemm(g, e->n_cu).kernel;
+    return k == GemmKernel::Tile256 ? (int)GEMM_TILE_256 : k == GemmKernel::Tile128 ? (int)GEMM_TILE_128 : 0;
+  };
+  const int S = pad_row;
+  const int tile1 = tile_of(conv1(0, N_FRAMES)), tile2 = tile_of(conv2(0, N_CTX));
+  if (S >= 1 && S < N_CTX - 1 && tile1 && tile2 && !debug_switch(DBG_PAD_SKIP)) {
+    HIPCHK(e->pad_pos.ensure(sizeof(float) * 2 * (size_t)d));
+    Gemm g = conv1(0, 2 * S);
+    g.force_tile = tile1;
     HIPCHK(gemm(e, s, g));
+    g = conv1(N_FRAMES - 2, 2);
+    g.force_tile = tile1;
+    HIPCHK(gemm(e, s, g));
+    const int dst[3] = {2 * S, 2 * S + 1, N_FRAMES - 3};
+    HIPCHK(launch_pad_fill_h1(e->h1pad, om * d, B, 2 * S - 1, dst, 2 * S + 1 < N_FRAMES - 3 ? 3 : 2, e->enc_pos, N_CTX - 1, d, (float*)e->pad_pos.p, s));
+    g = conv2(0, S);
+    g.force_tile = tile2;
+    HIPCHK(gemm(e, s, g));
+    g = conv2(S, 2);
+    g.lda = (N_CTX - 1 - S) * 2 * om * d;
+    g.C = e->x + (size_t)(N_CTX - 2) * d;
+    g.pos = (const float*)e->pad_pos.p;
+    g.force_tile = tile2;
+    HIPCHK(gemm(e, s, g));
+    HIPCHK(launch_pad_fill_x(e->x, N_CTX, d, B, N_CTX - 2, e->enc_pos, S, N_CTX - 2, s));
+    HIPCHK(launch_pad_fill_x(e->x, N_CTX, d, B, N_CTX - 2, e->enc_pos, N_CTX - 2, N_CTX - 1, s));
+  } else {
+    HIPCHK(gemm(e, s, conv1(0, N_FRAMES)));
+    HIPCHK(gemm(e, s, conv2(0, N_CTX)));
   }
   const int M = B * N_CTX;
   const float scale = 1.0f / std::sqrt((float)(d / H));
@@ -500,13 +539,16 @@
   return WCA_OK;
 }
 
-int run_phase1(wca_engine* e, const float* mel_dev, const float* pcm_dev, int64_t pcm_stride, const int* n_samples_dev, int batch, int slot,
-               bool skip_last_v) {
+int run_phase1(wca_engine* e, const float* mel_dev, const float* pcm_dev, int64_t pcm_stride, const int* n_samples_dev, const int32_t* n_samples_host,
+               int batch, int slot, bool skip_last_v) {
   half_t* kvbuf = slot ? e->kv_alt : e->kv;
   record(e, 0);
+  int pad_row = N_CTX;
   if (pcm_dev) {
-    int rc = run_logmel(e, pcm_dev, pcm_stride, n_samples_dev, batch, nullptr, true);
+    int rc = run_logmel(e, pcm_dev, pcm_stride, n_samples_dev, n_samples_host, batch, nullptr, true);
     if (rc) return rc;
+    pad_row = 0;
+    for (int b = 0; b < batch; ++b) pad_row = std::max(pad_row, pad_bounds(n_samples_host[b]).conv2);
   } else {
     if (int mr = mel_to_tm(e, mel_dev, batch)) return mr;
   }
@@ -514,7 +556,7 @@
   e->ln_err = e->err_dev + 1 + slot;
   HIPCHK(hipMemsetAsync(e->ln_err, 0, sizeof(int), e->stream));
   g_gemm_cu_limit = e->part_cus > 0 ? e->n_cu - e->part_cus : 0;
-  int rc = run_encoder(e, batch);
+  int rc = run_encoder(e, batch, pad_row);
   e->ln_err = e->err_dev;
   if (!rc) {
     record(e, 2);
diff --git a/whisper-char-alignment_amd/csrc/engine_internal.h b/whisper-char-alignment_amd/csrc/engine_internal.h
--- a/whisper-char-alignment_amd/csrc/engine_internal.h
+++ b/whisper-char-alignment_amd/csrc/engine_internal.h
@@ -105,6 +105,7 @@
   bool allow_rounded = false;
   char* wslab_lo = nullptr;
   std::set<const void*> wlo_bases;
+  wca::GrowBuf pad_pos;
   wca::GrowBuf wlo_tmp[2];
 
   char* wslab = nullptr;
@@ -265,7 +266,7 @@
   return g;
 }
 hipError_t gemm(wca_engine* e, hipStream_t s, Gemm g);
-int run_encoder(wca_engine* e, int B);
+int run_encoder(wca_engine* e, int B, int pad_row = N_CTX);
 int run_cross_kv(wca_engine* e, int B, half_t* kvbuf = nullptr, bool skip_last_v = false);
 int run_decoder(wca_engine* e, const int64_t* tokens_dev, int B, int n, float* cap, int Fpad, int Fcap, float* logits_out, hipStream_t s = nullptr,
                 const half_t* kvbuf = nullptr, bool finish_last = false);
@@ -273,10 +274,15 @@
                     int T_max, bool want_logits, int phase = -2);
 int run_decode_prefill(wca_engine* e, hipStream_t s, const half_t* kvbuf, const int* tokens, int B, int n, int T_max, StepPos last, StepPos sot);
 int mel_to_tm(wca_engine* e, const float* mel_dev, int batch);
-int run_phase1(wca_engine* e, const float* mel_dev, const float* pcm_dev, int64_t pcm_stride, const int* n_samples_dev, int batch, int slot,
-               bool skip_last_v = false);
+int run_phase1(wca_engine* e, const float* mel_dev, const float* pcm_dev, int64_t pcm_stride, const int* n_samples_dev, const int32_t* n_samples_host,
+               int batch, int slot, bool skip_last_v = false);
 
 int check_pcm_lengths(const int32_t* n_samples_host, int batch, int64_t pcm_stride);
-int run_logmel(wca_engine* e, const float* pcm_dev, int64_t pcm_stride, const int* n_samples_dev, int B, float* mel_out, bool want_tm);
-
-}
+int run_logmel(wca_engine* e, const float* pcm_dev, int64_t pcm_stride, const int* n_samples_dev, const int32_t* n_samples_host, int B, float* mel_out,
+               bool want_tm);
+struct PadBounds {
+  int frames, mel, conv1, conv2;
+};
+PadBounds pad_bounds(int n_samples);
+
+}
diff --git a/whisper-char-alignment_amd/csrc/kernels.h b/whisper-char-alignment_amd/csrc/kernels.h
--- a/whisper-char-alignment_amd/csrc/kernels.h
+++ b/whisper-char-alignment_amd/csrc/kernels.h
@@ -6,7 +6,7 @@
 
 typedef _Float16 half_t;
 
-enum { DBG_ATTN_SPLIT_VARIANT = 0, DBG_HEAD_STATS_GENERAL, DBG_FAIL_PRECISION_ALLOC, DBG_ATTN_SPLIT_DROP, DBG_GEMM_RING, DBG_SWITCH_COUNT };
+enum { DBG_ATTN_SPLIT_VARIANT = 0, DBG_HEAD_STATS_GENERAL, DBG_FAIL_PRECISION_ALLOC, DBG_ATTN_SPLIT_DROP, DBG_GEMM_RING, DBG_PAD_SKIP, DBG_SWITCH_COUNT };
 int debug_switch(int id);
 int set_debug_switch(const char* name, int value);
 
@@ -106,6 +106,7 @@
   int split;
   long q_lo, k_lo, v_lo, o_lo;
   const int* nk_rows;
+  int tail_half;
 };
 hipError_t launch_attention(const AttnArgs& a, hipStream_t s);
 hipError_t launch_attention_split(const AttnArgs& a, hipStream_t s);
@@ -115,6 +116,9 @@
 hipError_t launch_embed(const int64_t* tokens, const half_t* tok_emb, const float* pos_emb, float* x,
                         int B, int n, int d, int n_vocab, int* err, hipStream_t s, const half_t* tok_emb_lo = nullptr);
 hipError_t launch_fill_f16(half_t* p, size_t n, float v, hipStream_t s);
+hipError_t launch_pad_fill_h1(half_t* h1pad, int row_w, int B, int src, const int* dst, int n_dst, const float* pos, int last_row, int d, float* pos_tail,
+                              hipStream_t s);
+hipError_t launch_pad_fill_x(float* x, int rows, int d, int B, int c_row, const float* pos, int t0, int t1, hipStream_t s);
 
 struct StepPos {
   int t;
@@ -173,6 +177,7 @@
   float* scratch;
   unsigned* gmax;
   int B;
+  int frames;
 };
 hipError_t launch_logmel(const LogMelArgs& a, hipStream_t s);
 
diff --git a/whisper-char-alignment_amd/csrc/logmel.hip b/whisper-char-alignment_amd/csrc/logmel.hip
--- a/whisper-char-alignment_amd/csrc/logmel.hip
+++ b/whisper-char-alignment_amd/csrc/logmel.hip
@@ -192,7 +192,8 @@
   if (a.B <= 0) return hipSuccess;
   if (a.n_mels > 256) return hipErrorInvalidValue;
   hipLaunchKernelGGL(logmel_init_kernel, dim3((a.B + 63) / 64), dim3(64), 0, s, a.gmax, a.B);
-  hipLaunchKernelGGL(logmel_power_kernel, dim3(NFRAMES, a.B), dim3(256), 0, s, a);
+  const int frames = a.frames > 0 && a.frames < NFRAMES ? a.frames : NFRAMES;
+  hipLaunchKernelGGL(logmel_power_kernel, dim3(frames, a.B), dim3(256), 0, s, a);
   hipLaunchKernelGGL(logmel_finalize_kernel, dim3((NFRAMES + 63) / 64, a.B), dim3(256), 0, s, a);
   return hipGetLastError();
 }
```

New measurement: 353.6, median of 6. No clear change (+0.7%).
